# mikestir/webradio

Hardware: AMD Instinct MI355X
Metric: complex Msamples/sec (node), 256-ch DDC+NFM demod (higher is better)
Workload: dtype f32

## Files before the change

include/webradio_amd.h:

```cpp
#ifndef WEBRADIO_AMD_H_
#define WEBRADIO_AMD_H_

#include <stddef.h>
#include <stdint.h>

#ifdef __cplusplus
extern "C" {
#endif

#define WR_ABI_VERSION   6
#define WR_FIR_LENGTH    64
#define WR_TABLE_SIZE    65536

enum wr_status {
	WR_OK = 0,
	WR_ERR_ARG = 1,
	WR_ERR_HIP = 2,
	WR_ERR_STATE = 3,
	WR_ERR_NOMEM = 4,
	WR_ERR_NODEV = 5,
	WR_ERR_RATE = 6
};

enum wr_mode { WR_AM = 0, WR_FM = 1, WR_USB = 2, WR_LSB = 3 };

enum wr_stage {
	WR_STAGE_CHAN_IQ = 1,
	WR_STAGE_DEMOD   = 2,
	WR_STAGE_AUDIO   = 3
};

enum wr_nco {
	WR_NCO_SPLIT = 0,
	WR_NCO_EXACT = 1,
	WR_NCO_ROTATE = 2
};

enum wr_where { WR_HOST = 0, WR_DEVICE = 1 };

typedef struct wr_dev      wr_dev;
typedef struct wr_tuner    wr_tuner;
typedef struct wr_spectrum wr_spectrum;
typedef struct wr_ring     wr_ring;

int         wr_abi_version(void);
const char *wr_last_error(void);
int         wr_device_count(int *count);
enum wr_tunable {
	WR_TUNE_DDC_NG2_MIN_PASSES = 1
};
int         wr_tune(int key, long value, long *previous);

int wr_phase_step(int if_hz, unsigned int input_rate, int *phase_step);
int wr_sin_table(float *table_host);
int wr_lowpass_design(unsigned int passband, unsigned int input_rate,
                      float *coeff_host , unsigned int *maxbin_out);
#define WR_FIR_MAX 1024
#define WR_FIR_FUSED_MAX 256
int wr_lowpass_design_n(unsigned int fir_length, unsigned int passband, unsigned int input_rate,
                        float *coeff_host , unsigned int *maxbin_out);
int wr_spectrum_window(unsigned int fft_size, float *window_host);

int wr_dev_open(wr_dev **dev, int device_index, void *hip_stream);
int wr_dev_close(wr_dev *dev);
int wr_dev_sync(wr_dev *dev);
void *wr_dev_stream(wr_dev *dev);
int wr_dev_malloc(wr_dev *dev, size_t bytes, void **ptr_dev);
int wr_dev_free(wr_dev *dev, void *ptr_dev);
int wr_dev_upload(wr_dev *dev, void *dst_dev, const void *src_host, size_t bytes);
int wr_dev_download(wr_dev *dev, void *dst_host, const void *src_dev, size_t bytes);
int wr_dev_host_register(wr_dev *dev, void *host, size_t bytes);
int wr_dev_host_unregister(wr_dev *dev, void *host);
int wr_dev_upload_async(wr_dev *dev, void *dst_dev, const void *src_host, size_t bytes);
int wr_dev_wait_uploads(wr_dev *dev);
int wr_dev_wait_uploads_but(wr_dev *dev, unsigned int newest);
int wr_dev_upload_ahead(wr_dev *dev, void *dst_dev, const void *src_host, size_t bytes);

int wr_mix(wr_dev *dev, const float *in_dev, float *out_dev, size_t nframes,
           unsigned int *phase_io, int phase_step);

int wr_fir_decimate(wr_dev *dev, const float *in_dev, size_t nframes, unsigned int channels,
                    unsigned int decimation, const float *coeff_host ,
                    float *history_dev, float *out_dev);
int wr_fir_decimate_n(wr_dev *dev, const float *in_dev, size_t nframes, unsigned int channels,
                      unsigned int decimation, unsigned int fir_length, const float *coeff_host ,
                      float *history_dev, float *out_dev);
unsigned long long wr_block_kernel_calls(void);

int wr_demod(wr_dev *dev, int mode, const float *in_dev, size_t nframes,
             float *prev_io , float *out_dev);

int wr_u8_to_f32(wr_dev *dev, const uint8_t *in_dev, float *out_dev, size_t count);
int wr_u8_to_f32_from_host(wr_dev *dev, const uint8_t *in_host_registered, float *out_dev, size_t count);
int wr_stage_windows_from_host(wr_dev *dev, const void *in_host_registered, int is_u8, float *out_dev, size_t nframes,
                               unsigned int period, unsigned int length, size_t tail_frames);

#define WR_MAX_CHANNELS 4096
int wr_tuner_create(wr_tuner **tuner, wr_dev *dev, unsigned int input_rate,
                    unsigned int max_channels, size_t max_block_frames, int nco_mode);
int wr_tuner_destroy(wr_tuner *tuner);

int wr_chan_add(wr_tuner *tuner, int *chan);
int wr_chan_remove(wr_tuner *tuner, int chan);
int wr_chan_count(wr_tuner *tuner, int *count);

int wr_chan_set_if(wr_tuner *tuner, int chan, int if_hz);
int wr_chan_set_filter(wr_tuner *tuner, int chan, int stage, unsigned int passband,
                       unsigned int out_rate);
int wr_chan_set_taps(wr_tuner *tuner, int chan, int stage, const float *coeff_host ,
                     unsigned int decimation);
int wr_chan_set_filter_n(wr_tuner *tuner, int chan, int stage, unsigned int fir_length,
                         unsigned int passband, unsigned int out_rate);
int wr_chan_set_taps_n(wr_tuner *tuner, int chan, int stage, const float *coeff_host ,
                       unsigned int fir_length, unsigned int decimation);
#define WR_FILTER_CHANNEL  0
#define WR_FILTER_AUDIO    1
#define WR_FILTER_CHANNEL2 2
int wr_chan_set_af_gain(wr_tuner *tuner, int chan, float gain_db);
int wr_chan_set_squelch(wr_tuner *tuner, int chan, float threshold_dbfs, int enable);
int wr_chan_set_mode(wr_tuner *tuner, int chan, int mode);
int wr_tuner_keep_stages(wr_tuner *tuner, unsigned int stage_mask);

int wr_chan_get_state(wr_tuner *tuner, int chan, unsigned int *phase, float *prev_iq );
int wr_chan_set_state(wr_tuner *tuner, int chan, unsigned int phase, const float *prev_iq);

int wr_tuner_last_staging(wr_tuner *tuner, int *how);
int wr_tuner_submit(wr_tuner *tuner, const float *iq, size_t nframes, int where);
int wr_tuner_submit_u8(wr_tuner *tuner, const uint8_t *iq_u8, size_t nframes, int where);

int wr_tuner_flush(wr_tuner *tuner);

int wr_chan_fetch(wr_tuner *tuner, int chan, int stage, float *out_host, size_t out_capacity,
                  size_t *count);
int wr_tuner_audio_dev(wr_tuner *tuner, const float **audio_dev, size_t *chan_stride,
                       size_t *frames);
int wr_chan_slot(wr_tuner *tuner, int chan, int *slot);
int wr_tuner_fetch_audio_all(wr_tuner *tuner, float *out_host, size_t out_capacity,
                             size_t *chan_stride, size_t *frames, unsigned int *slots_used);
int wr_tuner_audio_ring(wr_tuner *tuner, unsigned int depth);
int wr_tuner_audio_ring_acquire(wr_tuner *tuner, const float **audio_host, size_t *chan_stride,
                                size_t *frames, unsigned int *slots_used, unsigned long long *seq);
int wr_tuner_audio_ring_release(wr_tuner *tuner);
int wr_tuner_audio_ring_ready(wr_tuner *tuner, int *ready);
int wr_tuner_audio_ring_stats(wr_tuner *tuner, unsigned int *queued, unsigned long long *overruns);
int wr_tuner_submit_count(wr_tuner *tuner, unsigned long long *submits);
int wr_chan_reset_history(wr_tuner *tuner, int chan);
int wr_tuner_seek(wr_tuner *tuner, unsigned long long frame);
int wr_ring_id_bytes(void);
int wr_ring_version(int *version);
int wr_ring_make_id(void *id_host, size_t nbytes);
int wr_ring_create(wr_ring **ring, wr_dev *dev, const void *id_host, size_t nbytes, int rank, int world);
int wr_ring_exchange(wr_ring *ring, const float *send_dev, float *recv_dev, size_t nfloats);
int wr_tuner_mark_launches(wr_tuner *tuner, int enable);
int wr_ring_exchange_after(wr_ring *ring, wr_tuner *tuner, const float *send_dev, float *recv_dev, size_t nfloats);
int wr_ring_wait(wr_ring *ring);
int wr_ring_info(wr_ring *ring, int *rank, int *world, unsigned long long *exchanges);
int wr_ring_destroy(wr_ring *ring);
int wr_tuner_set_audio_scale(wr_tuner *tuner, float scale);

int wr_tuner_set_blocks_per_launch(wr_tuner *tuner, unsigned int nblocks);

#define WR_STREAM_MAX_BLOCKS 512u
int wr_tuner_set_streaming(wr_tuner *tuner, int enable);
int wr_tuner_stream_info(wr_tuner *tuner, int *live, unsigned long long *launches, unsigned long long *blocks);
int wr_tuner_stream_host_blocks(wr_tuner *tuner, unsigned long long *blocks);
int wr_tuner_stream_long_blocks(wr_tuner *tuner, unsigned long long *blocks);

int wr_tuner_profile(wr_tuner *tuner, int enable);
int wr_tuner_profile_read(wr_tuner *tuner, unsigned int *launches, double *mean_ms);

int wr_spectrum_create(wr_spectrum **spec, wr_dev *dev, unsigned int fft_size, unsigned int hop);
int wr_spectrum_destroy(wr_spectrum *spec);
int wr_spectrum_push(wr_spectrum *spec, const float *iq, size_t nframes, int where);
int wr_spectrum_lazy_info(wr_spectrum *spec, unsigned long long *deferred_pushes, unsigned long long *resolves);
int wr_spectrum_get_db(wr_spectrum *spec, float *magnitudes_host );
int wr_spectrum_get_bins(wr_spectrum *spec, float *bins_host );
int wr_spectrum_frames_done(wr_spectrum *spec, unsigned long *frames);
int wr_spectrum_get_waterfall_row(wr_spectrum *spec, unsigned int width, int hold,
                                  float *db_row_host, uint8_t *palette_host);
int wr_spectrum_batch_db(wr_spectrum *spec, const float *iq_dev, size_t nframes_fft,
                         float *db_dev);

#ifdef __cplusplus
}
#endif
#endif
```

webradio_amd/capi.py:

```python
import ctypes as C
import os

_HERE = os.path.dirname(os.path.abspath(__file__))
LIB_PATH = os.path.join(_HERE, "lib", "libwebradio_amd.so")

WR_OK, WR_ERR_ARG, WR_ERR_HIP, WR_ERR_STATE, WR_ERR_NOMEM, WR_ERR_NODEV, WR_ERR_RATE = range(7)
WR_AM, WR_FM, WR_USB, WR_LSB = range(4)
WR_STAGE_CHAN_IQ, WR_STAGE_DEMOD, WR_STAGE_AUDIO = 1, 2, 3
WR_NCO_SPLIT, WR_NCO_EXACT, WR_NCO_ROTATE = 0, 1, 2
WR_HOST, WR_DEVICE = 0, 1
WR_ABI_VERSION = 6
WR_STREAM_MAX_BLOCKS = 512
WR_FIR_LENGTH = 64
WR_TABLE_SIZE = 65536

_fp = C.POINTER(C.c_float)
_vp = C.c_void_p
_u32 = C.c_uint
_sz = C.c_size_t

SIGNATURES = {
    "wr_abi_version": (C.c_int, []),
    "wr_last_error": (C.c_char_p, []),
    "wr_device_count": (C.c_int, [C.POINTER(C.c_int)]),
    "wr_tune": (C.c_int, [C.c_int, C.c_long, C.POINTER(C.c_long)]),
    "wr_phase_step": (C.c_int, [C.c_int, _u32, C.POINTER(C.c_int)]),
    "wr_sin_table": (C.c_int, [_vp]),
    "wr_lowpass_design": (C.c_int, [_u32, _u32, _vp, C.POINTER(_u32)]),
    "wr_lowpass_design_n": (C.c_int, [_u32, _u32, _u32, _vp, C.POINTER(_u32)]),
    "wr_spectrum_window": (C.c_int, [_u32, _vp]),
    "wr_dev_open": (C.c_int, [C.POINTER(_vp), C.c_int, _vp]),
    "wr_dev_close": (C.c_int, [_vp]),
    "wr_dev_sync": (C.c_int, [_vp]),
    "wr_dev_stream": (_vp, [_vp]),
    "wr_dev_malloc": (C.c_int, [_vp, _sz, C.POINTER(_vp)]),
    "wr_dev_free": (C.c_int, [_vp, _vp]),
    "wr_dev_upload": (C.c_int, [_vp, _vp, _vp, _sz]),
    "wr_dev_download": (C.c_int, [_vp, _vp, _vp, _sz]),
    "wr_dev_host_register": (C.c_int, [_vp, _vp, _sz]),
    "wr_dev_host_unregister": (C.c_int, [_vp, _vp]),
    "wr_dev_upload_async": (C.c_int, [_vp, _vp, _vp, _sz]),
    "wr_dev_wait_uploads": (C.c_int, [_vp]),
    "wr_dev_wait_uploads_but": (C.c_int, [_vp, C.c_uint]),
    "wr_dev_upload_ahead": (C.c_int, [_vp, _vp, _vp, _sz]),
    "wr_mix": (C.c_int, [_vp, _vp, _vp, _sz, C.POINTER(_u32), C.c_int]),
    "wr_fir_decimate": (C.c_int, [_vp, _vp, _sz, _u32, _u32, _vp, _vp, _vp]),
    "wr_fir_decimate_n": (C.c_int, [_vp, _vp, _sz, _u32, _u32, _u32, _vp, _vp, _vp]),
    "wr_demod": (C.c_int, [_vp, C.c_int, _vp, _sz, _vp, _vp]),
    "wr_u8_to_f32": (C.c_int, [_vp, _vp, _vp, _sz]),
    "wr_stage_windows_from_host": (C.c_int, [_vp, _vp, C.c_int, _vp, _sz, _u32, _u32, _sz]),
    "wr_u8_to_f32_from_host": (C.c_int, [_vp, _vp, _vp, _sz]),
    "wr_tuner_create": (C.c_int, [C.POINTER(_vp), _vp, _u32, _u32, _sz, C.c_int]),
    "wr_tuner_destroy": (C.c_int, [_vp]),
    "wr_chan_add": (C.c_int, [_vp, C.POINTER(C.c_int)]),
    "wr_chan_remove": (C.c_int, [_vp, C.c_int]),
    "wr_chan_count": (C.c_int, [_vp, C.POINTER(C.c_int)]),
    "wr_chan_set_if": (C.c_int, [_vp, C.c_int, C.c_int]),
    "wr_chan_set_filter": (C.c_int, [_vp, C.c_int, C.c_int, _u32, _u32]),
    "wr_chan_set_taps": (C.c_int, [_vp, C.c_int, C.c_int, _vp, _u32]),
    "wr_chan_set_filter_n": (C.c_int, [_vp, C.c_int, C.c_int, _u32, _u32, _u32]),
    "wr_chan_set_taps_n": (C.c_int, [_vp, C.c_int, C.c_int, _vp, _u32, _u32]),
    "wr_chan_set_mode": (C.c_int, [_vp, C.c_int, C.c_int]),
    "wr_chan_set_af_gain": (C.c_int, [_vp, C.c_int, C.c_float]),
    "wr_chan_set_squelch": (C.c_int, [_vp, C.c_int, C.c_float, C.c_int]),
    "wr_tuner_keep_stages": (C.c_int, [_vp, _u32]),
    "wr_tuner_flush": (C.c_int, [_vp]),
    "wr_tuner_set_blocks_per_launch": (C.c_int, [_vp, _u32]),
    "wr_tuner_set_streaming": (C.c_int, [_vp, C.c_int]),
    "wr_tuner_stream_info": (C.c_int, [_vp, C.POINTER(C.c_int), C.POINTER(C.c_ulonglong), C.POINTER(C.c_ulonglong)]),
    "wr_tuner_stream_host_blocks": (C.c_int, [_vp, C.POINTER(C.c_ulonglong)]),
    "wr_tuner_stream_long_blocks": (C.c_int, [_vp, C.POINTER(C.c_ulonglong)]),
    "wr_tuner_seek": (C.c_int, [_vp, C.c_ulonglong]),
    "wr_tuner_audio_ring": (C.c_int, [_vp, _u32]),
    "wr_tuner_audio_ring_acquire": (C.c_int, [_vp, C.POINTER(C.POINTER(C.c_float)), C.POINTER(C.c_size_t),
                                              C.POINTER(C.c_size_t), C.POINTER(_u32), C.POINTER(C.c_ulonglong)]),
    "wr_tuner_audio_ring_release": (C.c_int, [_vp]),
    "wr_tuner_audio_ring_ready": (C.c_int, [_vp, C.POINTER(C.c_int)]),
    "wr_tuner_audio_ring_stats": (C.c_int, [_vp, C.POINTER(_u32), C.POINTER(C.c_ulonglong)]),
    "wr_tuner_submit_count": (C.c_int, [_vp, C.POINTER(C.c_ulonglong)]),
    "wr_chan_get_state": (C.c_int, [_vp, C.c_int, C.POINTER(_u32), _vp]),
    "wr_chan_set_state": (C.c_int, [_vp, C.c_int, _u32, _vp]),
    "wr_tuner_submit": (C.c_int, [_vp, _vp, _sz, C.c_int]),
    "wr_tuner_last_staging": (C.c_int, [_vp, C.POINTER(C.c_int)]),
    "wr_block_kernel_calls": (C.c_ulonglong, []),
    "wr_tuner_submit_u8": (C.c_int, [_vp, _vp, _sz, C.c_int]),
    "wr_chan_fetch": (C.c_int, [_vp, C.c_int, C.c_int, _vp, _sz, C.POINTER(_sz)]),
    "wr_tuner_audio_dev": (C.c_int, [_vp, C.POINTER(_vp), C.POINTER(_sz), C.POINTER(_sz)]),
    "wr_chan_slot": (C.c_int, [_vp, C.c_int, C.POINTER(C.c_int)]),
    "wr_tuner_fetch_audio_all": (C.c_int, [_vp, _vp, _sz, C.POINTER(_sz), C.POINTER(_sz), C.POINTER(_u32)]),
    "wr_chan_reset_history": (C.c_int, [_vp, C.c_int]),
    "wr_ring_id_bytes": (C.c_int, []),
    "wr_ring_version": (C.c_int, [C.POINTER(C.c_int)]),
    "wr_ring_make_id": (C.c_int, [_vp, _sz]),
    "wr_ring_create": (C.c_int, [C.POINTER(_vp), _vp, _vp, _sz, C.c_int, C.c_int]),
    "wr_ring_exchange": (C.c_int, [_vp, _vp, _vp, _sz]),
    "wr_ring_exchange_after": (C.c_int, [_vp, _vp, _vp, _vp, _sz]),
    "wr_tuner_mark_launches": (C.c_int, [_vp, C.c_int]),
    "wr_ring_wait": (C.c_int, [_vp]),
    "wr_ring_info": (C.c_int, [_vp, C.POINTER(C.c_int), C.POINTER(C.c_int), C.POINTER(C.c_ulonglong)]),
    "wr_ring_destroy": (C.c_int, [_vp]),
    "wr_tuner_set_audio_scale": (C.c_int, [_vp, C.c_float]),
    "wr_spectrum_get_waterfall_row": (C.c_int, [_vp, _u32, C.c_int, _vp, _vp]),
    "wr_tuner_profile": (C.c_int, [_vp, C.c_int]),
    "wr_tuner_profile_read": (C.c_int, [_vp, C.POINTER(_u32), C.POINTER(C.c_double)]),
    "wr_spectrum_create": (C.c_int, [C.POINTER(_vp), _vp, _u32, _u32]),
    "wr_spectrum_destroy": (C.c_int, [_vp]),
    "wr_spectrum_push": (C.c_int, [_vp, _vp, _sz, C.c_int]),
    "wr_spectrum_lazy_info": (C.c_int, [_vp, C.POINTER(C.c_ulonglong), C.POINTER(C.c_ulonglong)]),
    "wr_spectrum_get_db": (C.c_int, [_vp, _vp]),
    "wr_spectrum_get_bins": (C.c_int, [_vp, _vp]),
    "wr_spectrum_frames_done": (C.c_int, [_vp, C.POINTER(C.c_ulong)]),
    "wr_spectrum_batch_db": (C.c_int, [_vp, _vp, _sz, _vp]),
}


class WrError(RuntimeError):
    def __init__(self, code, msg):
        super().__init__("webradio_amd error %d: %s" % (code, msg))
        self.code = code


_lib = None


def load():
    global _lib
    if _lib is not None:
        return _lib
    if not os.path.exists(LIB_PATH):
        raise RuntimeError(
            "%s is missing: build it with `python -c 'import __graft_entry__ as g; g.build()'` "
            "(there is no CPU fallback)" % LIB_PATH)
    try:
        import torch
    except Exception:
        pass
    lib = C.CDLL(LIB_PATH, mode=C.RTLD_GLOBAL)
    for name, (res, args) in SIGNATURES.items():
        fn = getattr(lib, name)
        fn.restype = res
        fn.argtypes = args
    _lib = lib
    return lib


def check(rc):
    if rc != WR_OK:
        raise WrError(rc, load().wr_last_error().decode(errors="replace"))
    return rc


def ptr(x):
    if x is None:
        return None
    if isinstance(x, int):
        return C.c_void_p(x)
    if hasattr(x, "data_ptr"):
        return C.c_void_p(x.data_ptr())
    return C.c_void_p(x.ctypes.data)
```

webradio_amd/csrc/wr_capi_internal.h:

```cpp
#ifndef WR_CAPI_INTERNAL_H
#define WR_CAPI_INTERNAL_H

#include "wr_internal.h"

#include <cstdarg>
#include <cstdio>
#include <cstdlib>
#include <cstring>
#include <new>
#include <atomic>
#include <chrono>
#include <map>
#include <mutex>
#include <vector>

#define HIP_TRY(expr)                                                                    \
	do {                                                                                 \
		hipError_t e_ = (expr);                                                          \
		if (e_ != hipSuccess)                                                            \
			return wrc_fail(WR_ERR_HIP, "%s: %s (%s:%d)", #expr, hipGetErrorString(e_),  \
			                __FILE__, __LINE__);                                         \
	} while (0)


#define WR_UPLOAD_RING 4

struct wr_dev {
	int device;
	hipStream_t stream;
	bool own_stream;
	int num_cus;
	float *table;
	float *table_turn;
	float *turn_host;
	float *hi_cs, *lo_cs;
	float *scratch;
	size_t scratch_floats;
	float *coeff;
	std::mutex *scratch_lock;
	hipEvent_t upload_ev[WR_UPLOAD_RING];
	std::atomic<unsigned long long> uploads_issued, uploads_done;
	std::mutex *upload_lock;
	hipStream_t up_stream;
	hipStream_t lazy_stream = nullptr;
	hipEvent_t up_tail[WR_UPLOAD_RING], up_done;
	void *up_out[WR_UPLOAD_RING];
	unsigned long long up_calls;
	uint8_t *up_raw[2];
	size_t up_raw_cap[2];
	std::map<void *, size_t> *registered;
	wr_tuner *streaming = nullptr;
	unsigned long long reg_gen = 1;
};
#define SCRATCH_GUARD(d) std::lock_guard<std::mutex> scratch_guard_(*(d)->scratch_lock)

struct Chan {
	bool in_use;
	int if_hz;
	unsigned int stepL;
	unsigned int phaseL;
	int mode;
	bool have[3];
	float taps[3][WR_FIR_LENGTH];
	unsigned int len1;
	float taps_long[WR_FIR_FUSED_MAX];
	unsigned int len2, len1b;
	float taps_long2[WR_FIR_FUSED_MAX], taps_long1b[WR_FIR_FUSED_MAX];
	unsigned int decim[3];
	float gain;
	float squelch;
	bool cs_hist_reset;
	int group;
	int slot;
	float prev_iq[2];
	bool prev_dirty;
	bool phase_dirty;
	bool dem_hist_reset;
};

struct Group {
	unsigned int d1, d2;
	unsigned int d1b = 0;
	unsigned int l1 = WR_FIR_LENGTH;
	unsigned int l2 = WR_FIR_LENGTH;
	unsigned int l1b = WR_FIR_LENGTH;
	int p2 = 0;
	bool use_gain = false, use_squelch = false;
	unsigned int slots;
	size_t k1max, k2max;
	WrGroupDev dev;
	int audio_cur = 0;
	int parity;
	int last_parity;
	bool last_demod_kept = false;
	bool post_pending = false;
	WrPostArgs post_args;
	bool seek_pending = false;
	unsigned long long seek_frame = 0;
	float *z_hist = nullptr, *z_prev = nullptr, *z_dem = nullptr;
	bool pend_direct = false;
	unsigned long long pend_seq = 0;
	size_t pend_k2 = 0;
	unsigned int pend_slots = 0;
	int sp;
	int cb;
	int last_cb;
	std::vector<int> owner;
	bool dirty;
	bool uniform_taps;
	unsigned long long uniform_mask = 0;
	unsigned long long uniform2_mask = 0;
	unsigned long long fewsets_mask = 0;
	unsigned char nsets[64] = {0};
	bool one_filter = false;
	bool long_uniform = false;
	bool long_one = false;
	size_t last_k1, last_k2;
	int active;
};

struct wr_tuner {
	wr_dev *dev;
	unsigned int input_rate;
	unsigned int max_channels;
	size_t max_block_frames;
	int nco_mode;
	unsigned int keep_mask;
	std::vector<Chan> chans;
	std::vector<Group *> groups;
	float *in_stage;
	int last_staging = 0;
	const void *probe_ptr = nullptr;
	unsigned long long probe_gen = 0;
	unsigned int probe_left = 0;
	float *in_hist[2];
	int in_par;
	bool submitted;
	float audio_scale;
	bool profiling;
	unsigned int prof_stride;
	unsigned int prof_tick;
	std::vector<unsigned int> ev_span;
	bool mark_launches = false;
	hipEvent_t launch_ev[4] = {nullptr, nullptr, nullptr, nullptr};
	unsigned long long launches_marked = 0;
	std::vector<hipEvent_t> ev;
	size_t ev_used;
	double prof_ms;
	unsigned int prof_n;
	struct RingSlot {
		float *host = nullptr;
		size_t cap = 0;
		hipEvent_t done = nullptr;
		size_t stride = 0, frames = 0;
		unsigned int slots = 0;
		unsigned long long seq = 0;
		unsigned int stream_wait = 0;
		unsigned long long stream_gen = 0;
	};
	std::vector<RingSlot> ring;
	unsigned int ring_head = 0, ring_count = 0;
	bool ring_held = false;
	unsigned long long ring_overruns = 0;
	unsigned long long submit_seq = 0;
	bool defer_post = true;
	unsigned int coalesce = 1;
	const float *held_base = nullptr;
	size_t held_frames = 0, held_each = 0;
	unsigned int held_count = 0;
	std::mutex ring_lock;
	struct Stream {
		bool enabled = false;
		bool host_bytes = false;
		bool live = false;
		bool unchecked = false;
		WrStreamCtl *ctl = nullptr;
		WrStreamDesc *desc = nullptr;
		WrStreamDev *sdev = nullptr;
		float *ring = nullptr;
		size_t ring_floats = 0;
		Group *g = nullptr;
		unsigned int count = 0;
		size_t nframes = 0;
		bool u8 = false;
		int parity0 = 0;
		size_t k1 = 0, k2 = 0;
		unsigned long long gen = 0;
		unsigned long long blocks = 0;
		std::chrono::steady_clock::time_point last_bell;
		const float *last_iq = nullptr;
		uint8_t *raw[4] = {nullptr, nullptr, nullptr, nullptr};
		size_t raw_cap = 0;
		unsigned long long raw_next = 0;
		unsigned long long raw_gen[4] = {0, 0, 0, 0};
		unsigned int raw_idx[4] = {0, 0, 0, 0};
		hipEvent_t raw_ev = nullptr;
		bool ext = false;
		bool up_pending = false;
		unsigned long long host_blocks = 0;
		unsigned long long long_blocks = 0;
	} stream;
};

struct wr_spectrum {
	wr_dev *dev;
	unsigned int n, hop;
	WrFftPlan plan;
	float *stage;
	size_t stage_cap;
	size_t pending;
	float *bins;
	unsigned long frames_done;
	bool deferred = false;
	float *keep_host = nullptr;
	size_t keep_cap = 0;
	size_t def_off = 0, def_keep = 0;
	size_t def_rest = 0;
	hipEvent_t def_ev = nullptr;
	unsigned long long deferred_pushes = 0, resolves = 0;
};


int        wrc_dev_bind(wr_dev *d);
int        wrc_dev_settle_stream(wr_dev *d);
hipError_t wrc_dev_stream_sync(wr_dev *d);
int        wrc_dev_scratch(wr_dev *d, size_t floats);
void      *wrc_host_mapped(const void *host, hipError_t *why = nullptr);
int        wrc_upload_mark_locked(wr_dev *d, hipStream_t st);
int        wrc_upload_mark(wr_dev *d, hipStream_t st);
int        wrc_dev_up_stream(wr_dev *d);

unsigned int  wrc_group_slots_used(const Group *g);
WrTunerLaunch wrc_group_launch(const wr_tuner *t, const Group *g, const float *cur, const uint8_t *cur_u8, size_t nframes);
Group        *wrc_single_group(wr_tuner *t, bool *several = nullptr);
int           wrc_group_upload(wr_tuner *t, Group *g);
int           wrc_settle_held(wr_tuner *t);
int           wrc_tuner_launch_held(wr_tuner *t);
int           wrc_tuner_flush(wr_tuner *t);
int           wrc_tuner_quiesce(wr_tuner *t);
int           wrc_tuner_submit_now(wr_tuner *t, const void *iq, size_t nframes, int where, bool u8);
void          wrc_advance_phases(wr_tuner *t, unsigned long long frames);
int           wrc_prof_pair_begin(wr_tuner *t, void **ev_start, void **ev_stop);
void          wrc_prof_pair_stamped(wr_tuner *t);

int  wrc_stream_close(wr_tuner *t);
int  wrc_stream_check(wr_tuner *t);
void wrc_stream_free(wr_tuner *t);
bool wrc_stream_follows(const wr_tuner *t, size_t nframes, int where, bool u8);
int  wrc_stream_bell(wr_tuner *t, const void *iq, bool behind_upload);
int  wrc_stream_open(wr_tuner *t, const void *iq, size_t nframes, bool u8, bool *took);
int  wrc_stream_host_u8(wr_tuner *t, const uint8_t *bytes, size_t nframes, bool *took);

float *wrc_ring_reserve(wr_tuner *t, Group *g, size_t k2, unsigned int used);
int    wrc_ring_push(wr_tuner *t, Group *g, unsigned long long seq, size_t k2, unsigned int used, bool direct);
float *wrc_stream_ring_entry(wr_tuner *t, Group *g, unsigned long long seq, size_t k2, unsigned int used, unsigned int idx);

#define DEV_SETTLE(d_) do { if (int rc_ = wrc_dev_settle_stream(d_)) return rc_; } while (0)
#define TUNER_SYNC_CHECKED(t_) do { HIP_TRY(wrc_dev_stream_sync((t_)->dev)); if (int rc_ = wrc_stream_check(t_)) return rc_; } while (0)

#define WR_STREAM_IDLE_MS   500
#define WR_STREAM_STALE_MS  100
#define WR_STREAM_WAIT_MS  2000
#define WR_STREAM_HOST_MIN_BYTES (16u << 10)

#endif
```

webradio_amd/csrc/wr_internal.h:

```cpp
#ifndef WR_INTERNAL_H_
#define WR_INTERNAL_H_

#include <hip/hip_runtime.h>
#include <stddef.h>
#include <stdint.h>

#include "webradio_amd.h"

#define WR_HIST      (WR_FIR_LENGTH - 1)
#define WR_LANES     64
#define WR_SPLIT_N   256
#define WR_MAX_DEVICES 64
#define WR_TAPSETS   4

int         wrc_fail(int code, const char *fmt, ...) __attribute__((format(printf, 2, 3)));
int         wrc_dev_index(const wr_dev *dev);
hipStream_t wrc_dev_stream(const wr_dev *dev);
int         wrc_tuner_launch_mark(wr_tuner *t, hipEvent_t *ev);

void     wrd_sin_table(float *table);
void     wrd_sin_table_rounded(float *table);
int      wrd_phase_step(int if_hz, unsigned int input_rate);
unsigned wrd_lowpass_maxbin(unsigned int fir_length, unsigned int passband, unsigned int input_rate);
void     wrd_lowpass_design(unsigned int fir_length, unsigned int passband, unsigned int input_rate, float *coeff);
void     wrd_spectrum_window(unsigned int n, float *window);
void     wrd_split_tables(float *hi_cs , float *lo_cs );
void     wrd_twiddles(unsigned int n, float *tw );

struct WrGroupDev {
	unsigned int *phase[2];
	unsigned int *step;
	float        *hist_cs[2];
	float        *hist_lo[2];
	int          *flags;
	int          *mode;
	float        *taps1;
	float        *taps2;
	float        *taps2u;
	float        *rot;
	float        *taps1u;
	int          *tapsel;
	float        *taps1b;
	float        *iq2_hist[2];
	float        *chan_iq2[2];
	float        *taps1L;
	float        *mixhist[2];
	float        *gain;
	float        *squelch;
	float        *prev_iq[2];
	float        *chan_iq[2];
	float        *dem[2];
	float        *audio;
	float        *audio_set[4];
	unsigned int  l2 = 64, l1b = 64;
};

struct WrTunerLaunch {
	const float *cur;
	const uint8_t *cur_u8;
	const float *hist;
	float       *hist_next;
	int          parity;
	int          sp;
	int          cb;
	size_t       nframes;
	unsigned int d1, d2;
	unsigned int slots;
	unsigned int slots_used;
	size_t       k1, k2;
	size_t       k2max;
	int          nco_mode;
	float        audio_scale;
	int          use_gain, use_squelch;
	unsigned long long uniform_mask;
	unsigned long long uniform2_mask;
	unsigned long long fewsets_mask;
	unsigned char nsets[64];
	int          one_filter;
	void        *ev_start, *ev_stop;
	bool         seeking = false;
	unsigned int seek_lo = 0;
};

hipError_t wrk_mix(hipStream_t st, const float *in, float *out, size_t nframes,
                   unsigned int phase, int step, const float *table_dev);
hipError_t wrk_fir(hipStream_t st, const float *in, size_t nframes, unsigned int channels,
                   unsigned int decim, unsigned int fir_length, const float *coeff_dev, const float *hist_dev,
                   float *out);
hipError_t wrk_hist_update(hipStream_t st, const float *in, size_t nframes, unsigned int channels,
                           unsigned int fir_length, float *hist_dev, float *scratch_dev);
hipError_t wrk_demod(hipStream_t st, int mode, const float *in, size_t nframes, float prev_i,
                     float prev_q, float *out);
hipError_t wrk_u8_to_f32(hipStream_t st, const uint8_t *in, float *out, size_t count);
hipError_t wrk_stage_windows(hipStream_t st, const void *src_mapped, bool u8, float *dst, size_t nframes, unsigned int period,
                             unsigned int len, size_t tail_frames);

struct WrPostArgs {
	const float *chan_iq;
	unsigned int k1, slots;
	const int   *mode;
	const float *prev_iq;
	float       *prev_next;
	const float *dem_hist;
	float       *dem_hist_next;
	size_t       k2;
	unsigned int tiles;
	unsigned int run;
	unsigned int ntiles;
	const float *taps2;
	const float *taps2u;
	unsigned long long uni2;
	float       *audio;
	size_t       k2max;
	float        scale;
	unsigned int d2;
	unsigned int groups;
	const float *gain;
	const float *squelch;
	float       *audio_host;
	size_t       host_stride;
	unsigned int nseg = 1;
	const float *chan_prev = nullptr;
};
long wrk_tune_ng2_min_passes(long value, bool set);
hipError_t wrk_tuner_ddc(hipStream_t st, const WrTunerLaunch &L, const WrGroupDev &G,
                         const float *table_dev, const float *hi_dev, const float *lo_dev,
                         int num_cus, const WrPostArgs *post = nullptr, bool *post_taken = nullptr);
hipError_t wrk_tuner_ddc_long(hipStream_t st, const WrTunerLaunch &L, const WrGroupDev &G, unsigned int len,
                              const float *table_dev, int num_cus, bool rotate, bool rotate_one_filter, const float *hi_dev,
                              const float *lo_dev, const WrPostArgs *post = nullptr, bool *post_taken = nullptr);
hipError_t wrk_tuner_demod(hipStream_t st, const WrTunerLaunch &L, const WrGroupDev &G);
hipError_t wrk_tuner_iq2(hipStream_t st, const WrGroupDev &G, unsigned int slots, unsigned int slots_used,
                         size_t k1a, unsigned int d1b, int cb, int p2);
hipError_t wrk_tuner_audio(hipStream_t st, const WrTunerLaunch &L, const WrGroupDev &G);
WrPostArgs wrk_post_args(const WrTunerLaunch &L, const WrGroupDev &G);
hipError_t wrk_tuner_post(hipStream_t st, const WrTunerLaunch &L, const WrGroupDev &G);
hipError_t wrk_tuner_post_args(hipStream_t st, const WrPostArgs &A);
bool wrk_tuner_post_supported(unsigned int d2);
hipError_t wrk_input_hist(hipStream_t st, const float *cur, const uint8_t *cur_u8, size_t nframes,
                          const float *hist, float *hist_next);
hipError_t wrk_seek(hipStream_t st, const WrGroupDev &G, unsigned int slots, int sp, int parity, int p2,
                    unsigned long long frame);
hipError_t wrk_gather_rows(hipStream_t st, const float *src, size_t rows, size_t row_stride_floats,
                           size_t col_offset_floats, unsigned int width_floats, float *dst);

#define WR_STREAM_MAXJ   WR_STREAM_MAX_BLOCKS
#define WR_STREAM_RING   6u
struct WrStreamDesc {
	unsigned long long cur;
	unsigned long long audio_host;
	unsigned int count;
	unsigned int pad;
};
struct WrStreamCtl {
	volatile unsigned int ready;
	volatile unsigned int stop;
	volatile unsigned int pad0[14];
	volatile unsigned int done;
	volatile unsigned int final_blocks;
	volatile unsigned int err;
	volatile unsigned int self_closed;
	volatile unsigned int long_blocks;
	volatile unsigned int pad1[11];
};
#define WR_STREAM_SHARDS 16u
struct WrStreamDev {
	unsigned int ready, stop;
	unsigned long long beat;
	unsigned int ready_up;
	unsigned int pad0[27];
	unsigned long long progress;
	unsigned int drain_from;
	unsigned int pad1[29];
	unsigned int post_done[WR_STREAM_MAXJ];
	unsigned int post_fine[WR_STREAM_MAXJ];
	unsigned int post_ticket[WR_STREAM_MAXJ];
	unsigned int ddc_done[WR_STREAM_MAXJ][WR_STREAM_SHARDS][32];
	WrStreamDesc desc[WR_STREAM_MAXJ];
	unsigned long long cur[WR_STREAM_MAXJ + 1u];
};
struct WrStreamArgs {
	WrStreamCtl        *ctl;
	const WrStreamDesc *desc_host;
	WrStreamDev        *sdev;
	unsigned long long  idle_ticks;
	unsigned long long  wait_ticks;
	unsigned int        n_ddc, n_post;
	unsigned long long *tl;
	unsigned long long  cur0, audio0;
	unsigned long long  nframes;
	unsigned int        k1, d1, is_u8;
	unsigned int        ext;
	unsigned int        slots, groups;
	unsigned long long  gmap0, gmap1;
	unsigned int        kslow;
	unsigned int        kmax;
	const float        *hist;
	float              *hist_next;
	const unsigned int *phase, *step;
	unsigned int       *phase_next;
	const float        *hist_cs, *hist_lo;
	float              *hist_cs_next, *hist_lo_next;
	const int          *flags;
	const float        *taps1, *rot, *taps1u;
	const int          *tapsel;
	const float        *table, *hi_cs, *lo_cs;
	float              *ring;
	float              *audio_bufs[4];
	WrPostArgs          post;
	unsigned int        drain_run, drain_ntiles;
	const float        *prev_iq[2];
	float              *dem[2];
	int                 parity0;
	unsigned int        one_filter;
};
#define WR_STREAM_ERR_WAIT   1u
hipError_t wrk_stream_geometry(unsigned int d2, unsigned int groups, unsigned int kmax, bool one_filter, int num_cus,
                               unsigned int *n_ddc, unsigned int *n_post);
hipError_t wrk_tuner_stream(hipStream_t st, const WrStreamArgs &A, void *ev_start, void *ev_stop);

struct WrFftPlan {
	unsigned int n;
	unsigned int n1, n2;
	float *tw_n;
	float *tw_sub;
	float *window;
	float *window_p1;
	float *work;
	size_t work_frames;
};
hipError_t wrk_fft_frames(hipStream_t st, const WrFftPlan &P, const float *iq, size_t hop,
                          size_t nframes_fft, float *bins_out , float *db_out );

hipError_t wrk_bins_to_db(hipStream_t st, const float *bins, unsigned int n, float *db);
hipError_t wrk_waterfall_row(hipStream_t st, const float *bins, unsigned int n, unsigned int width, int hold,
                             float *db_row, uint8_t *palette);

#endif
```

webradio_amd/csrc/wr_kernels.hip:

```cpp
#include "wr_internal.h"

#include <atomic>
#include <cstdlib>
#include <type_traits>

#include <hip/hip_ext.h>

typedef float v2f __attribute__((ext_vector_type(2)));
typedef __attribute__((address_space(3))) v2f lds_v2f;
typedef float v4f __attribute__((ext_vector_type(4)));
typedef __attribute__((address_space(3))) v4f lds_v4f;

#define PHASE_FLAG_ACTIVE   1

#define WR_CONSTANT __attribute__((address_space(4)))

#ifdef DDC_TIMELINE
#define TL_SLOTS 12
__device__ unsigned long long g_ddc_tl[16384 * TL_SLOTS];
extern "C" int wr_debug_timeline(unsigned long long *out, size_t n)
{
	return (int)hipMemcpyFromSymbol(out, HIP_SYMBOL(g_ddc_tl), n * sizeof(unsigned long long));
}
__device__ unsigned long long g_ddc_rt[16384 * 2];
// ... 49 lines not shown
		out[n] = y;
	}
}

__global__ void __launch_bounds__(256)
k_fir(const float *__restrict__ in, size_t outfloats, unsigned int channels, unsigned int decim,
      unsigned int L, const float *__restrict__ coeff, const float *__restrict__ hist, float *__restrict__ out)
{
	__shared__ float taps[WR_FIR_MAX];
	for (unsigned int j = threadIdx.x; j < L; j += blockDim.x)
		taps[j] = coeff[j];
	__syncthreads();
	const unsigned int nh = L - 1u;
	size_t stride = (size_t)gridDim.x * blockDim.x;
	for (size_t o = (size_t)blockIdx.x * blockDim.x + threadIdx.x; o < outfloats; o += stride) {
		size_t k = o / channels;
		unsigned int c = (unsigned int)(o - k * channels);
		size_t first = k * decim;
		float acc = 0.0f;
		for (unsigned int j = 0; j < L; ++j) {
			size_t f = first + j;
			float x = (f < nh) ? hist[f * channels + c] : in[(f - nh) * channels + c];
			acc = acc + taps[L - 1u - j] * x;
		}
		out[o] = acc;
	}
}

__global__ void k_hist_build(const float *__restrict__ in, size_t nframes, unsigned int channels, unsigned int nh,
                             const float *__restrict__ hist, float *__restrict__ scratch)
{
	unsigned int total = nh * channels;
	for (unsigned int e = blockIdx.x * blockDim.x + threadIdx.x; e < total; e += gridDim.x * blockDim.x) {
		size_t f = nframes + e / channels;
		unsigned int c = e % channels;
		scratch[e] = (f < nh) ? hist[f * channels + c] : in[(f - nh) * channels + c];
	}
}

__global__ void k_copy_f32(const float *__restrict__ src, float *__restrict__ dst, size_t n)
{
	size_t stride = (size_t)gridDim.x * blockDim.x;
	for (size_t i = (size_t)blockIdx.x * blockDim.x + threadIdx.x; i < n; i += stride)
		dst[i] = src[i];
}

__device__ __forceinline__ float fm_angle_cycles(float y, float x)
{
	const float ax = __builtin_fabsf(x), ay = __builtin_fabsf(y);
	const float mx = __builtin_fmaxf(ax, ay), mn = __builtin_fminf(ax, ay);
	const float sc = (mx < 0x1p-100f) ? 0x1p100f : 1.0f;
	const float r = (mx == 0.0f) ? 0.0f : (mn * sc) * __builtin_amdgcn_rcpf(mx * sc);
	const float t = r * r;
	float p = 0.002456712769344449f;
	p = __builtin_fmaf(p, t, -0.014401308260858059f);
	p = __builtin_fmaf(p, t, 0.03978113830089569f);
	p = __builtin_fmaf(p, t, -0.07234849780797958f);
	p = __builtin_fmaf(p, t, 0.1049894168972969f);
	p = __builtin_fmaf(p, t, -0.14161227643489838f);
	p = __builtin_fmaf(p, t, 0.19985906779766083f);
	p = __builtin_fmaf(p, t, -0.33332598209381104f);
	p = __builtin_fmaf(p, t, 0.9999998807907104f);
	float c = (p * r) * 0.15915494309189533577f;
	if (ay > ax)
		c = 0.25f - c;
	if (__builtin_signbitf(x))
		c = 0.5f - c;
	return __builtin_copysignf(c, y);
}

__device__ __forceinline__ float demod_one(int mode, float i, float q, float pi_, float pq_)
{
	switch (mode) {
	case WR_AM:
		return (float)sqrt((double)(i * i + q * q));
	case WR_FM: {
		float ii = i * pi_ + q * pq_;
		float qq = q * pi_ - i * pq_;
		return fm_angle_cycles(ii, qq);
	}
	case WR_USB:
		return i + q;
	default:
		return i - q;
	}
}

__global__ void __launch_bounds__(256)
k_demod(int mode, const float2 *__restrict__ in, size_t nframes, float prev_i, float prev_q,
        float *__restrict__ out)
{
	size_t stride = (size_t)gridDim.x * blockDim.x;
	for (size_t n = (size_t)blockIdx.x * blockDim.x + threadIdx.x; n < nframes; n += stride) {
		float2 z = in[n];
		float2 p = n ? in[n - 1] : make_float2(prev_i, prev_q);
		out[n] = demod_one(mode, z.x, z.y, p.x, p.y);
	}
}

__global__ void k_u8_to_f32(const uint8_t *__restrict__ in, float *__restrict__ out, size_t n)
{
	size_t stride = (size_t)gridDim.x * blockDim.x;
	for (size_t i = (size_t)blockIdx.x * blockDim.x + threadIdx.x; i < n; i += stride)
		out[i] = ((float)in[i] - 128.0f) / 128.0f;
}

#define U8_X16_WGS 128u
__global__ void __launch_bounds__(256) k_u8_to_f32_x16(const uint4 *__restrict__ in, float4 *__restrict__ out, size_t n16)
{
	const size_t stride = (size_t)gridDim.x * blockDim.x;
	for (size_t i0 = (size_t)blockIdx.x * blockDim.x + threadIdx.x; i0 < n16; i0 += 4 * stride) {
		uint4 v[4];
#pragma unroll
		for (int u = 0; u < 4; ++u)
			if (i0 + u * stride < n16)
				v[u] = in[i0 + u * stride];
#pragma unroll
		for (int u = 0; u < 4; ++u) {
			const size_t i = i0 + u * stride;
			if (i >= n16)
				break;
			const unsigned int w[4] = {v[u].x, v[u].y, v[u].z, v[u].w};
#pragma unroll
			for (int q = 0; q < 4; ++q) {
				float4 o;
				o.x = ((float)(w[q] & 255u) - 128.0f) / 128.0f;
				o.y = ((float)((w[q] >> 8) & 255u) - 128.0f) / 128.0f;
				o.z = ((float)((w[q] >> 16) & 255u) - 128.0f) / 128.0f;
				o.w = ((float)(w[q] >> 24) - 128.0f) / 128.0f;
				out[4 * i + q] = o;
			}
		}
	}
}


template <int NCO>
__device__ __forceinline__ v2f nco(unsigned int P, const float *__restrict__ table,
                                   const v2f *hi_l, const v2f *lo_l)
{
	if (NCO == WR_NCO_EXACT) {
		v2f cs;
		cs.y = table[P >> 16];
		cs.x = table[(P + 0x40000000u) >> 16];
		return cs;
	} else {
		constexpr unsigned int SH = (NCO == WR_NCO_SPLIT) ? 5u : 0u;
		const v2f a = hi_l[(P >> 24) << SH];
		const v2f b = lo_l[((P >> 16) & 255u) << SH];
		const v2f rot = {-a.y, a.x};
		return __builtin_elementwise_fma(rot, b.yy, a * b.xx);
	}
}

template <int NCO>
__device__ __forceinline__ void mac(v2f xs, v2f cs, float hj, v2f &acc)
{
	if (NCO == WR_NCO_EXACT) {
		const float mi = xs.x * cs.x + xs.y * cs.y;
		const float mq = xs.y * cs.x - xs.x * cs.y;
		float ti, tq;
		asm("v_mul_f32 %0, %1, %2" : "=v"(ti) : "v"(hj), "v"(mi));
		asm("v_mul_f32 %0, %1, %2" : "=v"(tq) : "v"(hj), "v"(mq));
		acc.x = acc.x + ti;
		acc.y = acc.y + tq;
	} else {
		const v2f xr = {xs.y, -xs.x};
		const v2f m = __builtin_elementwise_fma(xr, cs.yy, xs * cs.xx);
		asm("v_fmac_f32 %0, %1, %2" : "+v"(acc.x) : "v"(hj), "v"(m.x));
		asm("v_fmac_f32 %0, %1, %2" : "+v"(acc.y) : "v"(hj), "v"(m.y));
	}
}

__device__ __forceinline__ unsigned int rot_index(unsigned int p0, unsigned int st, unsigned int m)
{
	const unsigned int P = p0 + m * st;
	return (st >> 16) + (((P & 0xFFFFu) < (st & 0xFFFFu)) ? 1u : 0u);
}

__device__ __forceinline__ v2f rot_into(unsigned int p0, unsigned int st, unsigned int m,
                                        const float *__restrict__ table)
{
	const unsigned int idx = rot_index(p0, st, m);
	v2f r;
	r.y = table[idx & 0xFFFFu];
	r.x = table[(idx + 16384u) & 0xFFFFu];
	return r;
}

__device__ __forceinline__ void horner_step(v2f &A, float rc, float rs, v2f u)
{
	const float tr = __builtin_fmaf(-A.y, rs, u.x);
	const float ti = __builtin_fmaf(A.x, rs, u.y);
	const float ar = __builtin_fmaf(A.x, rc, tr);
	const float ai = __builtin_fmaf(A.y, rc, ti);
	A.x = ar;
	A.y = ai;
}

__device__ __forceinline__ void horner_close(v2f &y, v2f A, v2f cs)
{
	const float yr = __builtin_fmaf(A.y, cs.y, __builtin_fmaf(A.x, cs.x, y.x));
	const float yi = __builtin_fmaf(-A.x, cs.y, __builtin_fmaf(A.y, cs.x, y.y));
	y.x = yr;
	y.y = yi;
}

__device__ __forceinline__ void wave_prio(unsigned int level)
{
	if (level >= 3u)
		__builtin_amdgcn_s_setprio(3);
	else if (level == 2u)
		__builtin_amdgcn_s_setprio(2);
	else if (level == 1u)
		__builtin_amdgcn_s_setprio(1);
	else
		__builtin_amdgcn_s_setprio(0);
}

__device__ __forceinline__ void rot_tables_to_lds(v2f *lds, const float2 *hi_cs, const float2 *lo_cs)
{
	for (unsigned int e = threadIdx.x; e < WR_SPLIT_N; e += blockDim.x) {
		const float2 hv = hi_cs[e], lv = lo_cs[e];
		lds[e] = (v2f){hv.x, hv.y};
		lds[WR_SPLIT_N + e] = (v2f){lv.x, lv.y};
	}
	__syncthreads();
}

#define ROT_SEG 64
#define ROT_Q   (WR_FIR_LENGTH / ROT_SEG)
#define SLOW_CH 4

__device__ __forceinline__ void gather_split(unsigned int P, unsigned int &ah, unsigned int &al,
                                             v2f &a, v2f &b)
{
	asm("v_mov_b32_sdwa %0, %1 dst_sel:BYTE_1 dst_unused:UNUSED_PRESERVE src0_sel:BYTE_3"
	    : "+v"(ah) : "v"(P));
	asm("v_mov_b32_sdwa %0, %1 dst_sel:BYTE_1 dst_unused:UNUSED_PRESERVE src0_sel:BYTE_2"
	    : "+v"(al) : "v"(P));
	a = *(const lds_v2f *)(uintptr_t)ah;
	b = *(const lds_v2f *)(uintptr_t)al;
}

__device__ __forceinline__ float2 input_frame(const float2 *__restrict__ cur, const uchar2 *__restrict__ cur_u8,
                                              size_t n)
{
	if (cur_u8) {
		const uchar2 b = cur_u8[n];
		return make_float2(((float)b.x - 128.0f) / 128.0f, ((float)b.y - 128.0f) / 128.0f);
	}
	return cur[n];
}

#define POST_TK 16u
#define POST_B 4u
#define POST_LB 5u
#define POST_THREADS 512u
__device__ __forceinline__ float audio_out(float v, const float *__restrict__ gain, const float *__restrict__ squelch,
                                           const float2 *__restrict__ chan_iq, unsigned int slots, unsigned int so,
                                           size_t k, unsigned int d2, float scale)
{
	if (squelch) {
		const float thr = squelch[so];
		if (thr > 0.0f) {
			float p = 0.0f;
			for (unsigned int i = 0; i < d2; ++i) {
				const float2 z = chan_iq[(k * d2 + i) * slots + so];
				p = p + (z.x * z.x + z.y * z.y);
			}
			if (p / (float)d2 < thr)
				v = 0.0f;
		}
	}
	if (gain) {
		const float gn = gain[so];
		if (gn != 1.0f)
			v = v * gn;
	}
	return (scale == 1.0f) ? v : v * scale;
}

__device__ __forceinline__ float post_row(const float2 *__restrict__ chan_iq, unsigned int k1, unsigned int slots,
                                          unsigned int s, int m, const float2 *__restrict__ prev_iq,
                                          const float *__restrict__ dem_hist, size_t rr,
                                          const float2 *__restrict__ chan_prev = nullptr, unsigned int hist = WR_HIST)
{
	if (rr < hist) {
		if (!chan_prev)
			return dem_hist[rr * slots + s];
		const size_t kp = (size_t)k1 - hist + rr;
		const float2 z = chan_prev[kp * slots + s];
		const float2 zp = chan_prev[(kp - 1u) * slots + s];
		return demod_one(m, z.x, z.y, zp.x, zp.y);
	}
	const size_t kk = rr - hist;
	if (kk >= k1)
		return 0.0f;
	const float2 z = chan_iq[kk * slots + s];
	const float2 zp = kk ? chan_iq[(kk - 1u) * slots + s] : chan_prev ? chan_prev[((size_t)k1 - 1u) * slots + s] : prev_iq[s];
	return demod_one(m, z.x, z.y, zp.x, zp.y);
}

template <unsigned int D2, bool HREGS, unsigned int NSEG = 1u>
__device__ __forceinline__ void post_role(const WrPostArgs &A, unsigned int bx, unsigned int g,
                                          float *stage, float *tile, int *modes)
{
	constexpr unsigned int HIST = WR_FIR_LENGTH * NSEG - 1u;
	constexpr unsigned int NEED = (POST_TK - 1u) * D2 + WR_FIR_LENGTH * NSEG;
	constexpr unsigned int NROW = POST_THREADS / 64u;
	static_assert(NSEG == 1u || !HREGS, "the segmented filter reads its taps when their turn comes (measured at C2, 128 / 256 taps: "
	                                    "61 / 83 us per block; a segment's 64 taps fetched into registers first: 64 / 94)");
	const float2 *__restrict__ chan_iq = (const float2 *)A.chan_iq;
	const float2 *__restrict__ prev_iq = (const float2 *)A.prev_iq;
	const float2 *__restrict__ chan_prev = (const float2 *)A.chan_prev;
	const float *__restrict__ dem_hist = A.dem_hist;
	const float *__restrict__ taps2 = A.taps2;
	const unsigned int k1 = A.k1, slots = A.slots;
	const unsigned int lane = threadIdx.x & 63u;
	const unsigned int row = threadIdx.x >> 6;
	const unsigned int s = g * 64u + lane;
	const int m = A.mode[s];

	if (bx == A.ntiles) {
		if (m < 0)
			return;
		const size_t first = k1;
#pragma unroll
		for (unsigned int r = row; r < HIST; r += NROW)
			A.dem_hist_next[(size_t)r * slots + s] = post_row(chan_iq, k1, slots, s, m, prev_iq, dem_hist, first + r, chan_prev, HIST);
		if (row == 0)
			((float2 *)A.prev_next)[s] = k1 ? chan_iq[(size_t)(k1 - 1u) * slots + s] : prev_iq[s];
		return;
	}

	TLP(0);
	float h[HREGS ? WR_FIR_LENGTH : 1];
	if (HREGS && row < POST_TK / POST_B) {
#pragma unroll
		for (int j = 0; j < (HREGS ? WR_FIR_LENGTH : 1); ++j)
			h[j] = taps2[(size_t)j * slots + s];
	}
	if (row == 0)
		modes[lane] = m;
	constexpr unsigned int FRESH = POST_TK * D2;
	constexpr unsigned int CARRY = NEED - FRESH;
	constexpr unsigned int CARRY_PER = (CARRY * 64u + POST_THREADS - 1u) / POST_THREADS;
	for (unsigned int tt = 0; tt < A.run; ++tt) {
		const unsigned int tl = bx * A.run + tt;
		if (tl >= A.tiles)
			break;
		const size_t kbase = (size_t)tl * POST_TK;
		const size_t r0 = kbase * D2;
		unsigned int first = 0;
		if (tt) {
			float keep[CARRY_PER];
#pragma unroll
			for (unsigned int i = 0; i < CARRY_PER; ++i) {
				const unsigned int e = threadIdx.x + i * POST_THREADS;
				keep[i] = (e < CARRY * 64u) ? stage[FRESH * 64u + e] : 0.0f;
			}
			__syncthreads();
#pragma unroll
			for (unsigned int i = 0; i < CARRY_PER; ++i) {
				const unsigned int e = threadIdx.x + i * POST_THREADS;
				if (e < CARRY * 64u)
					stage[e] = keep[i];
			}
			first = CARRY;
		}
		{
			const unsigned int per = (NEED - first + NROW - 1u) / NROW;
			const unsigned int beg = first + row * per;
			const unsigned int end = (beg + per < NEED) ? beg + per : NEED;
			if (r0 > HIST && r0 + NEED <= (size_t)k1 + HIST) {
				const float2 *__restrict__ src = chan_iq + (r0 - HIST) * slots + s;
				for (unsigned int r = beg; r < end; r += POST_LB) {
					float2 z[POST_LB + 1u];
					z[0] = src[((size_t)r - 1u) * slots];
#pragma unroll
					for (unsigned int i = 0; i < POST_LB; ++i) {
						const unsigned int ri = (r + i < end) ? r + i : end - 1u;
						z[i + 1u] = src[(size_t)ri * slots];
					}
#pragma unroll
					for (unsigned int i = 0; i < POST_LB; ++i)
						if (r + i < end)
							stage[(r + i) * 64u + lane] = (m >= 0) ? demod_one(m, z[i + 1u].x, z[i + 1u].y, z[i].x, z[i].y) : 0.0f;
				}
			} else {
				float2 zp = make_float2(0.0f, 0.0f);
				if (m >= 0 && beg < end) {
					const size_t rr = r0 + beg;
					if (rr == HIST)
						zp = chan_prev ? chan_prev[((size_t)k1 - 1u) * slots + s] : prev_iq[s];
					else if (rr > HIST && rr - HIST - 1u < k1)
						zp = chan_iq[(rr - HIST - 1u) * slots + s];
					else if (rr < HIST && chan_prev)
						zp = chan_prev[((size_t)k1 - HIST - 1u + rr) * slots + s];
				}
#pragma unroll 6
				for (unsigned int r = beg; r < end; ++r) {
					const size_t rr = r0 + r;
					float v = 0.0f;
					if (m >= 0) {
						if (rr < HIST && chan_prev) {
							const float2 z = chan_prev[((size_t)k1 - HIST + rr) * slots + s];
							v = demod_one(m, z.x, z.y, zp.x, zp.y);
							zp = z;
						} else if (rr < HIST) {
							v = dem_hist[rr * slots + s];
							if (rr + 1u == HIST)
								zp = prev_iq[s];
						} else if (rr - HIST < k1) {
							const float2 z = chan_iq[(rr - HIST) * slots + s];
							v = demod_one(m, z.x, z.y, zp.x, zp.y);
							zp = z;
						}
					}
					stage[r * 64u + lane] = v;
				}
			}
		}
		__syncthreads();
		TLP(1);
		if (row < POST_TK / POST_B) {
			float acc[POST_B];
#pragma unroll
			for (unsigned int o = 0; o < POST_B; ++o)
				acc[o] = 0.0f;
			if (HREGS) {
				const float *x = stage + (row * POST_B * D2) * 64u + lane;
#pragma unroll
				for (unsigned int r = 0; r < (POST_B - 1u) * D2 + WR_FIR_LENGTH; ++r) {
					const float xv = x[r * 64u];
#pragma unroll
					for (unsigned int o = 0; o < POST_B; ++o) {
						if (r >= o * D2 && r - o * D2 < WR_FIR_LENGTH)
							acc[o] = acc[o] + h[HREGS ? WR_FIR_LENGTH - 1u - (r - o * D2) : 0] * xv;
					}
				}
			} else {
#pragma unroll 1
			for (unsigned int seg = 0; seg < NSEG; ++seg) {
				const float *x = stage + (row * POST_B * D2 + seg * WR_FIR_LENGTH) * 64u + lane;
				const unsigned int tap0 = (NSEG - 1u - seg) * WR_FIR_LENGTH;
				if (g < 64u && ((A.uni2 >> g) & 1ull)) {
					const WR_CONSTANT float *tu = (const WR_CONSTANT float *)(A.taps2u + (size_t)g * (WR_FIR_LENGTH * NSEG) + tap0);
#pragma unroll
					for (int j = WR_FIR_LENGTH - 1; j >= 0; --j) {
						const float hj = tu[j];
#pragma unroll
						for (unsigned int o = 0; o < POST_B; ++o)
							acc[o] = acc[o] + hj * x[(o * D2 + (WR_FIR_LENGTH - 1u - (unsigned int)j)) * 64u];
					}
				} else {
#pragma unroll 16
					for (int j = WR_FIR_LENGTH - 1; j >= 0; --j) {
						const float hj = taps2[((size_t)tap0 + j) * slots + s];
#pragma unroll
						for (unsigned int o = 0; o < POST_B; ++o)
							acc[o] = acc[o] + hj * x[(o * D2 + (WR_FIR_LENGTH - 1u - (unsigned int)j)) * 64u];
					}
				}
			}
			}
#pragma unroll
			for (unsigned int o = 0; o < POST_B; ++o)
				tile[(row * POST_B + o) * 65u + lane] = acc[o];
		}
		__syncthreads();
		TLP(2);
		for (unsigned int e = threadIdx.x; e < 64u * POST_TK; e += POST_THREADS) {
			const unsigned int sl = e / POST_TK, kk = e - sl * POST_TK;
			const unsigned int so = g * 64u + sl;
			const size_t k = kbase + kk;
			if (k < A.k2 && modes[sl] >= 0) {
				const float v = audio_out(tile[kk * 65u + sl], A.gain, A.squelch, chan_iq, slots, so, k, D2, A.scale);
				A.audio[(size_t)so * A.k2max + k] = v;
				if (A.audio_host)
					A.audio_host[(size_t)so * A.host_stride + k] = v;
			} else if (k < A.k2 && A.audio_host) {
				A.audio_host[(size_t)so * A.host_stride + k] = 0.0f;
			}
		}
		TLP(3);
	}
}

template <unsigned int D2, unsigned int NSEG = 1u>
__global__ void __launch_bounds__(POST_THREADS)
k_tuner_post(WrPostArgs A)
{
	constexpr unsigned int NEED = (POST_TK - 1u) * D2 + WR_FIR_LENGTH * NSEG;
	if constexpr (NSEG == 1u) {
		__shared__ float stage[NEED * 64u];
		__shared__ float tile[POST_TK * 65u];
		__shared__ int modes[64];
		post_role<D2, NSEG == 1u, NSEG>(A, blockIdx.x, blockIdx.y, stage, tile, modes);
	} else {
		extern __shared__ float post_lds[];
		float *stage = post_lds;
		float *tile = stage + NEED * 64u;
		int *modes = (int *)(tile + POST_TK * 65u);
		post_role<D2, NSEG == 1u, NSEG>(A, blockIdx.x, blockIdx.y, stage, tile, modes);
	}
}

#define DDC_TABLE_BYTES   (2u * WR_SPLIT_N * 32u * 8u)
#define DDC_WAVES         16u
#define DDC_ROTATE_WAVES      8u
#define DDC_ROTATE_WGS_PER_CU 4u
#define DDC_LDS_BYTES     (DDC_TABLE_BYTES + DDC_WAVES * 2u * 512u)
#define DDC_DEAL_WAYS 2u

#define DDC_PARAMS \
	const float2 *__restrict__ cur, const uchar2 *__restrict__ cur_u8, const float2 *__restrict__ hist, \
	float2 *__restrict__ hist_next, size_t nframes, size_t k1, unsigned int d1, unsigned int slots, unsigned int groups, \
	const unsigned int *__restrict__ phase, const unsigned int *__restrict__ step, \
	const float2 *__restrict__ hist_cs, const int *__restrict__ flags, \
	unsigned int *__restrict__ phase_next, float2 *__restrict__ hist_cs_next, \
	const float2 *__restrict__ hist_lo, float2 *__restrict__ hist_lo_next, \
	const float *__restrict__ taps1, const float4 *__restrict__ rot, const float *__restrict__ taps1u, \
	const int *__restrict__ tapsel, unsigned int kmax, float2 *__restrict__ chan_iq, \
	const float *__restrict__ table, const float2 *__restrict__ hi_cs, const float2 *__restrict__ lo_cs, \
	unsigned int n_ddc, const WrPostArgs &post, unsigned long long gmap0, unsigned long long gmap1, int whole, \
	unsigned int kslow, unsigned int n_bnd, unsigned int seek_on, unsigned int seek_lo
#define DDC_PASS \
	cur, cur_u8, hist, hist_next, nframes, k1, d1, slots, groups, phase, step, hist_cs, flags, phase_next, hist_cs_next, \
	hist_lo, hist_lo_next, taps1, rot, taps1u, tapsel, kmax, chan_iq, table, hi_cs, lo_cs, n_ddc, post, gmap0, gmap1, \
	whole, kslow, n_bnd, seek_on, seek_lo
#define DDC_PHASE(s_) (seek_on ? step[s_] * seek_lo : phase[s_])
#define DDC_ROLE_ALL      0
#define DDC_ROLE_BOUNDARY 1
#define DDC_ROLE_ROLL     2

template <int NCO, bool UTAPS, unsigned int PD2>
__device__ __forceinline__ void
ddc_body(DDC_PARAMS, v2f *lds, const int role)
{
	if (PD2 != 0u && role != DDC_ROLE_ROLL && blockIdx.x >= n_ddc + n_bnd) {
		wave_prio(3u);
		constexpr unsigned int NEED = (POST_TK - 1u) * (PD2 ? PD2 : 1u) + WR_FIR_LENGTH;
		const unsigned int idx = blockIdx.x - n_ddc - n_bnd;
		if (threadIdx.x >= POST_THREADS)
			return;
		float *stage = (float *)lds;
		post_role<(PD2 ? PD2 : 1u), false>(post, idx % (post.ntiles + 1u), idx / (post.ntiles + 1u), stage,
		                                    stage + NEED * 64u, (int *)(stage + NEED * 64u + POST_TK * 65u));
		return;
	}
	const unsigned int lane = threadIdx.x & 63u;
	const unsigned int wave = __builtin_amdgcn_readfirstlane(threadIdx.x >> 6);
	const unsigned int waves_per_wg = blockDim.x >> 6;
	const unsigned int wid = blockIdx.x * waves_per_wg + wave;
	TL(0);
	wave_prio(3u);

	if (NCO == WR_NCO_SPLIT) {
		for (unsigned int e = threadIdx.x; e < WR_SPLIT_N * 32u; e += blockDim.x) {
			const float2 hv = hi_cs[e >> 5], lv = lo_cs[e >> 5];
			lds[e] = (v2f){hv.x, hv.y};
			lds[WR_SPLIT_N * 32u + e] = (v2f){lv.x, lv.y};
		}
		__syncthreads();
	} else if (NCO == WR_NCO_ROTATE) {
		rot_tables_to_lds(lds, hi_cs, lo_cs);
	}
	const v2f *hi_l = (NCO == WR_NCO_ROTATE) ? lds : lds + (lane & 31u);
	const v2f *lo_l = (NCO == WR_NCO_ROTATE) ? lds + WR_SPLIT_N : lds + WR_SPLIT_N * 32u + (lane & 31u);
	const unsigned int a_hi = (unsigned int)(uintptr_t)hi_l;
	const unsigned int a_lo = (unsigned int)(uintptr_t)lo_l;
	const unsigned int nset = UTAPS ? kmax : 1u;
	v2f *win = lds + (NCO == WR_NCO_SPLIT ? DDC_TABLE_BYTES / 8u : NCO == WR_NCO_ROTATE ? 2u * WR_SPLIT_N : 0u)
	           + wave * (128u * nset);

	if (whole && role != DDC_ROLE_ROLL && blockIdx.x == 0 && wave == 0 && lane < WR_HIST) {
		const size_t f = nframes + lane;
		hist_next[lane] = (f < WR_HIST) ? hist[f] : input_frame(cur, cur_u8, f - WR_HIST);
	}

	const unsigned int k1u = (unsigned int)k1;
	const unsigned int nwaves = n_ddc * waves_per_wg;
	TL(1);
	constexpr bool LTAPS = (NCO == WR_NCO_ROTATE) && !UTAPS;
	unsigned int wpg = LTAPS ? (n_ddc / groups) * waves_per_wg : nwaves / groups;
	const bool bnd = role == DDC_ROLE_BOUNDARY;
	const unsigned int ub = bnd ? (blockIdx.x - n_ddc) * waves_per_wg + wave : 0u;
	const unsigned int gl = bnd ? ub % groups : LTAPS ? blockIdx.x % groups : wid % groups;
	const unsigned int g = (unsigned int)(((gl < 8u ? gmap0 : gmap1) >> ((gl & 7u) * 8u)) & 255u);
	unsigned int k = bnd ? ub / groups : LTAPS ? (blockIdx.x / groups) * waves_per_wg + wave : wid / groups;
	if (role == DDC_ROLE_ROLL) {
		k = k1u;
	} else if (bnd) {
		if (k >= kslow)
			k = k1u;
		wpg = k1u;
	} else if (k >= wpg) {
		k = k1u;
	} else if (!LTAPS) {
		const unsigned int r = k % DDC_DEAL_WAYS, q = k / DDC_DEAL_WAYS;
		const unsigned int fl_ = wpg / DDC_DEAL_WAYS, rem = wpg % DDC_DEAL_WAYS;
		k = r * fl_ + (r < rem ? r : rem) + q;
	}
	const float *ltaps = (const float *)(lds + (NCO == WR_NCO_ROTATE ? 2u * WR_SPLIT_N : 0u) + waves_per_wg * 128u * nset);
	if (LTAPS) {
		float *lt = (float *)(lds + 2u * WR_SPLIT_N + waves_per_wg * 128u * nset);
		for (unsigned int e = threadIdx.x; e < WR_FIR_LENGTH * 64u; e += blockDim.x)
			lt[e] = taps1[(size_t)(e >> 6) * slots + g * 64u + (e & 63u)];
		__syncthreads();
	}

	float h[(UTAPS || LTAPS) ? 1 : WR_FIR_LENGTH];
	float hlane[UTAPS ? WR_TAPSETS : 1];
	unsigned int mysel = 0;
#pragma unroll
	for (int q = 0; q < (UTAPS ? WR_TAPSETS : 1); ++q)
		hlane[q] = 0.0f;
	unsigned int p0 = 0, st = 0;
	int fl = 0;
	unsigned int buf = 0;
	v2f rot0 = {1.0f, 0.0f}, rot1 = {1.0f, 0.0f};

	auto window_sample = [&](unsigned int kk) -> float2 {
		const long long n = (long long)kk * d1 - WR_HIST + lane;
		return (n >= 0) ? input_frame(cur, cur_u8, (size_t)n) : hist[WR_HIST + n];
	};
	float2 xnext = make_float2(0.0f, 0.0f);
	float2 xnext2 = make_float2(0.0f, 0.0f);
	const unsigned int s = g * 64u + lane;
	if (k < k1u) {
		{
			p0 = DDC_PHASE(s);
			st = step[s];
			fl = flags[s];
			if (NCO == WR_NCO_ROTATE) {
				const float4 r = rot[s];
				rot0 = (v2f){r.x, r.y};
				rot1 = (v2f){r.z, r.w};
			}
			if (UTAPS) {
				mysel = (unsigned int)tapsel[s];
#pragma unroll
				for (int q = 0; q < (UTAPS ? WR_TAPSETS : 1); ++q)
					if ((unsigned int)q < nset)
						hlane[q] = taps1u[((size_t)g * WR_TAPSETS + q) * 64u + lane];
			} else {
#pragma unroll
				for (int j = 0; j < ((UTAPS || LTAPS) ? 1 : WR_FIR_LENGTH); ++j)
					h[j] = taps1[(size_t)j * slots + s];
			}
		}
		xnext = window_sample(k);
		if (k + wpg < k1u)
			xnext2 = window_sample(k + wpg);
	}

	TL(2);
	unsigned int tl_unit = 0;
	const unsigned int my_units = (k < k1u) ? (k1u - k + wpg - 1u) / wpg : 0u;
	for (; k < k1u; buf ^= 1u) {
		const unsigned int kn = k + wpg;
		{
			const unsigned int q = (4u * tl_unit) / (my_units ? my_units : 1u);
			wave_prio(q >= 3u ? 0u : 2u - q + 0u);
		}

		const long long n0 = (long long)k * d1 - WR_HIST;
		{
			const float2 xf = xnext;
			if (UTAPS) {
#pragma unroll
				for (int q = 0; q < (UTAPS ? WR_TAPSETS : 1); ++q)
					if ((unsigned int)q < nset)
						win[(buf * nset + q) * 64u + lane] = (v2f){hlane[q] * xf.x, hlane[q] * xf.y};
			} else {
				win[buf * 64u + lane] = (v2f){xf.x, xf.y};
			}
// ... 1634 lines not shown
```

webradio_amd/csrc/wr_stream_kernel.inc:

```

__device__ __forceinline__ unsigned int st_rfl(unsigned int v) { return __builtin_amdgcn_readfirstlane(v); }
__device__ __forceinline__ unsigned int st_ld(const unsigned int *p)
{
	return st_rfl(__hip_atomic_load(p, __ATOMIC_RELAXED, __HIP_MEMORY_SCOPE_AGENT));
}
__device__ __forceinline__ unsigned long long st_ld64(const unsigned long long *p)
{
	const unsigned long long v = __hip_atomic_load(p, __ATOMIC_RELAXED, __HIP_MEMORY_SCOPE_AGENT);
	return ((unsigned long long)st_rfl((unsigned int)(v >> 32)) << 32) | st_rfl((unsigned int)v);
}
__device__ __forceinline__ unsigned int st_ld_sys(const volatile unsigned int *p)
{
	return st_rfl(__hip_atomic_load((const unsigned int *)p, __ATOMIC_RELAXED, __HIP_MEMORY_SCOPE_SYSTEM));
}
__device__ __forceinline__ void st_st_sys(volatile unsigned int *p, unsigned int v)
{
	__hip_atomic_store((unsigned int *)p, v, __ATOMIC_RELAXED, __HIP_MEMORY_SCOPE_SYSTEM);
}

__device__ __forceinline__ unsigned int st_ddc_ready(const WrStreamArgs &S)
{
	return st_rfl((unsigned int)__hip_atomic_load(&S.sdev->progress, __ATOMIC_RELAXED, __HIP_MEMORY_SCOPE_AGENT));
}
__device__ __forceinline__ unsigned int st_post_ready(const WrStreamArgs &S)
{
	return st_rfl((unsigned int)(__hip_atomic_load(&S.sdev->progress, __ATOMIC_RELAXED, __HIP_MEMORY_SCOPE_AGENT) >> 32));
}

__device__ __forceinline__ void stream_fail(const WrStreamArgs &S)
{
	st_st_sys(&S.ctl->err, WR_STREAM_ERR_WAIT);
	__hip_atomic_store(&S.sdev->stop, 1u, __ATOMIC_RELAXED, __HIP_MEMORY_SCOPE_AGENT);
}

__device__ __forceinline__ bool stream_wait_ready(const WrStreamArgs &S, unsigned int need, unsigned int &known, bool &closed)
{
	if (need < known)
		return true;
	if (closed)
		return false;
	const unsigned long long t0 = __builtin_amdgcn_s_memrealtime();
	unsigned int spins = 0;
	for (;;) {
		const unsigned int r = st_ld(&S.sdev->ready);
		if (r > need) {
			known = r;
			return true;
		}
		if (st_ld(&S.sdev->stop)) {
			const unsigned int f = st_ld(&S.sdev->ready);
			if (f > known)
				known = f;
			closed = true;
			return known > need;
		}
		if ((++spins & 63u) == 0u) {
			const unsigned long long now = __builtin_amdgcn_s_memrealtime();
			const unsigned long long beat = __hip_atomic_load(&S.sdev->beat, __ATOMIC_RELAXED, __HIP_MEMORY_SCOPE_AGENT);
			if (now - t0 > S.wait_ticks && now >= beat && now - beat > S.wait_ticks) {
				stream_fail(S);
				if (r > known)
					known = r;
				closed = true;
				return false;
			}
		}
		__builtin_amdgcn_s_sleep(20);
	}
}

__device__ __forceinline__ bool stream_wait_count(const WrStreamArgs &S, const unsigned int *p, unsigned int target)
{
	if (st_ld(p) >= target)
		return true;
	const unsigned long long t0 = __builtin_amdgcn_s_memrealtime();
	unsigned int spins = 0;
	for (;;) {
		__builtin_amdgcn_s_sleep(20);
		if (st_ld(p) >= target)
			return true;
		if ((++spins & 63u) == 0u) {
			if (__builtin_amdgcn_s_memrealtime() - t0 > S.wait_ticks) {
				stream_fail(S);
				return false;
			}
			if (st_ld_sys(&S.ctl->err))
				return false;
		}
	}
}

#define STREAM_DRAIN_BLOCKS 2u
__device__ __forceinline__ void stream_watch(const WrStreamArgs &S)
{
	const unsigned int lane = threadIdx.x & 63u;
	__builtin_amdgcn_s_setprio(3);
	const unsigned int units = S.k1 * S.groups;
	unsigned int known = 1, jd = 0, jp = 0;
	unsigned int df = 0;
	unsigned int nlong = 0;
	bool closed = false;
	unsigned long long t_last = __builtin_amdgcn_s_memrealtime();
#ifdef STREAM_TL
	if ((threadIdx.x & 63u) == 0 && S.tl)
		S.tl[6999u * 8u + 0u] = t_last;
#endif
	for (;;) {
		bool moved = false;
		auto look = [&]() __attribute__((always_inline)) {
			const unsigned int r = st_ld(&S.sdev->ready);
			if (r > known)
				known = r;
			if (st_ld(&S.sdev->stop)) {
				const unsigned int f = st_ld(&S.sdev->ready);
				if (f > known)
					known = f;
				closed = true;
				const unsigned int from = known >= STREAM_DRAIN_BLOCKS ? known - STREAM_DRAIN_BLOCKS : 0u;
				df = (jd > from ? jd : from) + 1u;
				__hip_atomic_store(&S.sdev->drain_from, df, __ATOMIC_RELAXED, __HIP_MEMORY_SCOPE_AGENT);
				__builtin_amdgcn_fence(__ATOMIC_RELEASE, "agent");
			}
		};
		if (!closed && (jd >= known || jp >= known))
			look();
		if (jd < known && jd < WR_STREAM_MAXJ) {
			unsigned int v = 0;
			if (lane < WR_STREAM_SHARDS)
				v = __hip_atomic_load(&S.sdev->ddc_done[jd][lane][0], __ATOMIC_RELAXED, __HIP_MEMORY_SCOPE_AGENT);
#pragma unroll
			for (int o = 8; o >= 1; o >>= 1)
				v += __shfl_xor(v, o, 64);
			if (st_rfl(v) >= units) {
				{
					unsigned int fine = 1u;
					if (S.drain_run != S.post.run) {
						if (!closed)
							look();
						fine = (df && jd + 1u >= df) ? 1u : known >= jd + 3u ? 0u : 1u;
					}
					__hip_atomic_store(&S.sdev->post_fine[jd], fine, __ATOMIC_RELAXED, __HIP_MEMORY_SCOPE_AGENT);
					if (!fine && lane == 0)
						st_st_sys(&S.ctl->long_blocks, ++nlong);
					asm volatile("s_waitcnt vmcnt(0)" ::: "memory");
				}
				++jd;
				__hip_atomic_store(&S.sdev->progress, ((unsigned long long)jp << 32) | jd, __ATOMIC_RELAXED, __HIP_MEMORY_SCOPE_AGENT);
				moved = true;
#ifdef STREAM_TL
				if (lane == 0 && S.tl && jd <= 256u)
					S.tl[(7000u + jd - 1u) * 8u + 0u] = __builtin_amdgcn_s_memrealtime();
#endif
			}
		}
		if (jp < jd && st_ld(&S.sdev->post_done[jp]) >= (st_ld(&S.sdev->post_fine[jp]) ? S.drain_ntiles : S.post.ntiles) * S.post.groups) {
			++jp;
			__hip_atomic_store(&S.sdev->progress, ((unsigned long long)jp << 32) | jd, __ATOMIC_RELAXED, __HIP_MEMORY_SCOPE_AGENT);
			if (lane == 0)
				st_st_sys(&S.ctl->done, jp);
			moved = true;
#ifdef STREAM_TL
			if (lane == 0 && S.tl && jp <= 256u)
				S.tl[(7000u + jp - 1u) * 8u + 1u] = __builtin_amdgcn_s_memrealtime();
#endif
		}
		if (closed && jp >= known)
			return;
		const unsigned long long now = __builtin_amdgcn_s_memrealtime();
		if (moved) {
			t_last = now;
		} else {
			if ((jd < known || jp < jd) && now - t_last > S.wait_ticks) {
				stream_fail(S);
				return;
			}
			if (closed && st_ld_sys(&S.ctl->err))
				return;
			__builtin_amdgcn_s_sleep(4);
		}
	}
}

__device__ __forceinline__ void stream_bell(const WrStreamArgs &S)
{
	if (threadIdx.x >= 64u && threadIdx.x < 128u) {
		stream_watch(S);
		return;
	}
	if (threadIdx.x != 0)
		return;
	__builtin_amdgcn_s_setprio(3);
	unsigned int seen = 1;
	__hip_atomic_store(&S.sdev->desc[0].cur, S.cur0, __ATOMIC_RELAXED, __HIP_MEMORY_SCOPE_AGENT);
	__hip_atomic_store(&S.sdev->desc[0].audio_host, S.audio0, __ATOMIC_RELAXED, __HIP_MEMORY_SCOPE_AGENT);
	__hip_atomic_store(&S.sdev->cur[1], S.cur0, __ATOMIC_RELAXED, __HIP_MEMORY_SCOPE_AGENT);
	asm volatile("s_waitcnt vmcnt(0)" ::: "memory");
	unsigned long long t_last = __builtin_amdgcn_s_memrealtime();
	for (;;) {
		__hip_atomic_store(&S.sdev->beat, (unsigned long long)__builtin_amdgcn_s_memrealtime(), __ATOMIC_RELAXED,
		                   __HIP_MEMORY_SCOPE_AGENT);
		const unsigned int s = st_ld_sys(&S.ctl->stop);
		unsigned int r = st_ld_sys(&S.ctl->ready);
		{
			const unsigned int ru = st_ld(&S.sdev->ready_up);
			if (ru > r)
				r = ru;
		}
		if (r > WR_STREAM_MAXJ)
			r = WR_STREAM_MAXJ;
		if (r > seen) {
			for (unsigned int j = seen; j < r; ++j) {
				const unsigned long long c = __hip_atomic_load(&S.desc_host[j].cur, __ATOMIC_RELAXED, __HIP_MEMORY_SCOPE_SYSTEM);
				const unsigned long long a = __hip_atomic_load(&S.desc_host[j].audio_host, __ATOMIC_RELAXED, __HIP_MEMORY_SCOPE_SYSTEM);
				__hip_atomic_store(&S.sdev->desc[j].cur, c, __ATOMIC_RELAXED, __HIP_MEMORY_SCOPE_AGENT);
				__hip_atomic_store(&S.sdev->cur[j + 1u], c, __ATOMIC_RELAXED, __HIP_MEMORY_SCOPE_AGENT);
				__hip_atomic_store(&S.sdev->desc[j].audio_host, a, __ATOMIC_RELAXED, __HIP_MEMORY_SCOPE_AGENT);
			}
			asm volatile("s_waitcnt vmcnt(0)" ::: "memory");
			__hip_atomic_store(&S.sdev->ready, r, __ATOMIC_RELAXED, __HIP_MEMORY_SCOPE_AGENT);
			seen = r;
			t_last = __builtin_amdgcn_s_memrealtime();
		}
		if (s || st_ld(&S.sdev->stop)) {
			asm volatile("s_waitcnt vmcnt(0)" ::: "memory");
			__hip_atomic_store(&S.sdev->stop, 1u, __ATOMIC_RELAXED, __HIP_MEMORY_SCOPE_AGENT);
			return;
		}
		if (seen >= WR_STREAM_MAXJ || __builtin_amdgcn_s_memrealtime() - t_last > S.idle_ticks) {
			if (seen < WR_STREAM_MAXJ)
				st_st_sys(&S.ctl->self_closed, 1u);
			asm volatile("s_waitcnt vmcnt(0)" ::: "memory");
			__hip_atomic_store(&S.sdev->stop, 1u, __ATOMIC_RELAXED, __HIP_MEMORY_SCOPE_AGENT);
			return;
		}
		__builtin_amdgcn_s_sleep(40);
	}
}

template <unsigned int PD2, unsigned int TS>
__device__ __forceinline__ void stream_post(const WrStreamArgs &S, const unsigned int p, v2f *lds, const bool helper)
{
	constexpr unsigned int D2 = PD2 ? PD2 : 1u;
	constexpr unsigned int NEED = (POST_TK - 1u) * D2 + WR_FIR_LENGTH;
	wave_prio(3u);
	if (threadIdx.x >= POST_THREADS)
		return;
	const unsigned int wave = st_rfl(threadIdx.x >> 6);
	const unsigned int waves_per_wg = POST_THREADS / 64u;
#ifdef STREAM_TL
	if (threadIdx.x == 0 && S.tl && !helper)
		S.tl[(6000u + p) * 8u + 7u] = 12345ull;
#endif

	const unsigned int n_bnd = (S.kslow * S.groups + waves_per_wg - 1u) / waves_per_wg;
	if (!helper && p < n_bnd) {
		const unsigned long long c0 = S.cur0;
		ddc_body<WR_NCO_ROTATE, true, PD2>(S.is_u8 ? nullptr : (const float2 *)c0, S.is_u8 ? (const uchar2 *)c0 : nullptr,
		                                   (const float2 *)S.hist, (float2 *)S.hist_next, (size_t)S.nframes, (size_t)S.k1, S.d1,
		                                   S.slots, S.groups, S.phase, S.step, (const float2 *)S.hist_cs, S.flags, S.phase_next,
		                                   (float2 *)S.hist_cs_next, (const float2 *)S.hist_lo, (float2 *)S.hist_lo_next, S.taps1,
		                                   (const float4 *)S.rot, S.taps1u, S.tapsel, TS == 1u ? 1u : S.kmax, (float2 *)S.ring, S.table,
		                                   (const float2 *)S.hi_cs, (const float2 *)S.lo_cs, S.n_ddc, S.post, S.gmap0, S.gmap1, 0,
		                                   S.kslow, 0x40000000u, 0u, 0u, lds, DDC_ROLE_BOUNDARY);
		const unsigned int ub = p * waves_per_wg + wave;
		asm volatile("s_waitcnt vmcnt(0)" ::: "memory");
		if (ub / S.groups < S.kslow && (threadIdx.x & 63u) == 0u)
			__hip_atomic_fetch_add(&S.sdev->ddc_done[0][ub % WR_STREAM_SHARDS][0], 1u, __ATOMIC_RELAXED, __HIP_MEMORY_SCOPE_AGENT);
		wave_prio(3u);
		__syncthreads();
	}

	float *stage = (float *)lds;
	float *tile = stage + NEED * 64u;
	int *modes = (int *)(tile + POST_TK * 65u);
	unsigned int *sh = (unsigned int *)(modes + 64);
	const unsigned int tasks = S.post.ntiles * S.post.groups;
	unsigned int known = 1;
	bool closed = false;
	unsigned int j = 0;
	if (helper) {
		if (threadIdx.x == 0)
			sh[6] = st_ld(&S.sdev->drain_from);
		__syncthreads();
		const unsigned int df = sh[6];
		if (!df)
			return;
		j = df - 1u;
	}
#ifdef STREAM_TL
	unsigned long long pt_wait = 0, pt_work = 0, pt_sync = 0, pt_n = 0;
#endif
	for (;; ++j) {
#ifdef STREAM_TL
		const unsigned long long pt0 = __builtin_amdgcn_s_memtime();
#endif
		if (threadIdx.x == 0) {
			bool ok = j < WR_STREAM_MAXJ && stream_wait_ready(S, j, known, closed);
			if (ok) {
				const unsigned int need_hi = j >= 4u ? j - 3u : 0u;
				const unsigned long long t0 = __builtin_amdgcn_s_memrealtime();
				unsigned int spins = 0;
				for (;;) {
					const unsigned long long pg = st_ld64(&S.sdev->progress);
					if ((unsigned int)pg >= j + 1u && (unsigned int)(pg >> 32) >= need_hi)
						break;
					if ((++spins & 63u) == 0u) {
						if (__builtin_amdgcn_s_memrealtime() - t0 > S.wait_ticks) {
							stream_fail(S);
							ok = false;
							break;
						}
						if (st_ld_sys(&S.ctl->err)) {
							ok = false;
							break;
						}
					}
					__builtin_amdgcn_s_sleep(20);
				}
			}
			unsigned long long ah = 0;
			unsigned int drain = helper ? 1u : 0u;
			if (ok) {
				ah = j ? st_ld64(&S.sdev->desc[j].audio_host) : S.audio0;
				__builtin_amdgcn_fence(__ATOMIC_ACQUIRE, "agent");
				if (!helper) {
					const unsigned int df = st_ld(&S.sdev->drain_from);
					drain = (df && j + 1u >= df) ? 1u : 0u;
				}
				sh[7] = (helper || drain) ? 1u : st_ld(&S.sdev->post_fine[j]);
			}
			sh[5] = drain;
			sh[0] = ok ? 1u : 0u;
			sh[1] = (unsigned int)ah;
			sh[2] = (unsigned int)(ah >> 32);
			sh[3] = known;
		}
		__syncthreads();
		const bool go = sh[0] != 0u;
		const unsigned long long ah = ((unsigned long long)sh[2] << 32) | sh[1];
		known = sh[3];
		if (!go)
			break;
		WrPostArgs A = S.post;
		A.chan_iq = S.ring + (size_t)(j % WR_STREAM_RING) * S.k1 * S.slots * 2u;
		A.chan_prev = j ? S.ring + (size_t)((j - 1u) % WR_STREAM_RING) * S.k1 * S.slots * 2u : nullptr;
		A.prev_iq = S.prev_iq[S.parity0];
		A.dem_hist = S.dem[S.parity0];
		A.audio_host = (float *)ah;
		A.audio = S.audio_bufs[j & 3u];
#ifdef STREAM_TL
		const unsigned long long pt1 = __builtin_amdgcn_s_memtime();
		if (threadIdx.x == 0 && S.tl && !helper && p < 4u && j < 256u)
			S.tl[(7300u + j) * 8u + p * 2u] = __builtin_amdgcn_s_memrealtime();
#endif
		const bool drain = sh[5] != 0u;
		if (sh[7] != 0u) {
			A.run = S.drain_run;
			A.ntiles = S.drain_ntiles;
		}
		const unsigned int tasks_j = A.ntiles * A.groups;
		unsigned int mine = 0;
		const unsigned int rot = (unsigned int)(((unsigned long long)j * tasks) % S.n_post);
		for (unsigned int t = p >= rot ? p - rot : p + S.n_post - rot;; t += S.n_post) {
			if (drain) {
				if (threadIdx.x == 0)
					sh[4] = __hip_atomic_fetch_add(&S.sdev->post_ticket[j], 1u, __ATOMIC_RELAXED, __HIP_MEMORY_SCOPE_AGENT);
				__syncthreads();
				t = sh[4];
			}
			if (t >= tasks_j)
				break;
			post_role<D2, false>(A, t % A.ntiles, t / A.ntiles, stage, tile, modes);
			__syncthreads();
			++mine;
		}
		if (threadIdx.x == 0 && mine) {
			if (ah)
				__builtin_amdgcn_fence(__ATOMIC_RELEASE, "");
			else
				__builtin_amdgcn_fence(__ATOMIC_RELEASE, "agent");
			asm volatile("s_waitcnt vmcnt(0)" ::: "memory");
			__hip_atomic_fetch_add(&S.sdev->post_done[j], mine, __ATOMIC_RELAXED, __HIP_MEMORY_SCOPE_AGENT);
		}
#ifdef STREAM_TL
		if (threadIdx.x == 0 && S.tl && !helper && p < 4u && j < 256u)
			S.tl[(7300u + j) * 8u + p * 2u + 1u] = __builtin_amdgcn_s_memrealtime();
		if (threadIdx.x == 0) {
			const unsigned long long pt3 = __builtin_amdgcn_s_memtime();
			pt_wait += pt1 - pt0;
			pt_sync += pt3 - pt1;
			++pt_n;
		}
#endif
	}
#ifdef STREAM_TL
	if (threadIdx.x == 0 && S.tl && !helper) {
		S.tl[(6000u + p) * 8u + 0u] = pt_wait;
		S.tl[(6000u + p) * 8u + 1u] = pt_sync;
		S.tl[(6000u + p) * 8u + 2u] = pt_n;
	}
#endif
	if (!helper && p < S.post.groups && known && known <= WR_STREAM_MAXJ) {
		const unsigned int jl = known - 1u;
		WrPostArgs A = S.post;
		A.chan_iq = S.ring + (size_t)(jl % WR_STREAM_RING) * S.k1 * S.slots * 2u;
		A.chan_prev = jl ? S.ring + (size_t)((jl - 1u) % WR_STREAM_RING) * S.k1 * S.slots * 2u : nullptr;
		A.prev_iq = S.prev_iq[S.parity0];
		A.dem_hist = S.dem[S.parity0];
		A.prev_next = const_cast<float *>(S.prev_iq[S.parity0 ^ 1]);
		A.dem_hist_next = S.dem[S.parity0 ^ 1];
		post_role<D2, false>(A, A.ntiles, p, stage, tile, modes);
	}
}

template <unsigned int NG, unsigned int TS>
__device__ __forceinline__ void stream_ddc(const WrStreamArgs &S, v2f *lds)
{
	static_assert(TS == 1u || (TS == WR_TAPSETS && NG == 1u), "several channel filters: one lane group per wave");
	constexpr int NCO = WR_NCO_ROTATE;
	const unsigned int lane = threadIdx.x & 63u;
	const unsigned int wave = st_rfl(threadIdx.x >> 6);
	const unsigned int waves_per_wg = blockDim.x >> 6;
	const unsigned int wid = blockIdx.x * waves_per_wg + wave;
	wave_prio(3u);
	rot_tables_to_lds(lds, (const float2 *)S.hi_cs, (const float2 *)S.lo_cs);
	const v2f *hi_l = lds, *lo_l = lds + WR_SPLIT_N;
	const unsigned int nset = TS == 1u ? 1u : S.kmax;
	v2f *win = lds + 2u * WR_SPLIT_N + wave * (128u * nset);
	const unsigned int k1s = S.k1, d1 = S.d1;
	const unsigned int nwaves = S.n_ddc * waves_per_wg;
	const unsigned int gsets = S.groups / NG;
	const unsigned int wpg = nwaves / gsets;
	const unsigned int gs = wid % gsets;
	const unsigned int iw = wid / gsets;
	unsigned int known = 1;
	bool closed = false;
	if (iw < wpg) {
		const unsigned long long q0 = (unsigned long long)S.kslow + iw;
		LeanRec<NG> R = lean_rec<NG>([&](unsigned int s) { return S.phase[s]; }, S.step, S.flags, (const float4 *)S.rot,
		                             (float2 *)S.ring, S.gmap0, S.gmap1, gs, lane, (unsigned int)(q0 * d1 - WR_HIST), wpg, d1);
		const LeanWin<TS> W = lean_win<TS>(S.taps1u, S.tapsel, R.g0, lane, nset, win);
		unsigned int j = 0, k = (unsigned int)q0;
		while (k >= k1s) {
			k -= k1s;
			++j;
		}
		unsigned int jf = j, kf = k;
		unsigned int jb = 0xFFFFFFFFu;
		unsigned long long base_cur = 0, base_prev = 0;
		const bool u8 = S.is_u8 != 0u, ext = S.ext != 0u;
		unsigned int ahead = 0;
		bool drain = false;
		auto try_fetch = [&](float2 &dst) __attribute__((always_inline)) {
			if (drain)
				return;
			if (jf >= WR_STREAM_MAXJ) {
				drain = true;
				return;
			}
			if (jf >= known) {
				if (!closed) {
					const unsigned int r = st_ld(&S.sdev->ready);
					if (r > known)
						known = r;
					if (jf >= known && st_ld(&S.sdev->stop)) {
						const unsigned int f = st_ld(&S.sdev->ready);
						if (f > known)
							known = f;
						closed = true;
					}
				}
				if (jf >= known) {
					drain = true;
					return;
				}
			}
			if (jf != jb) {
				if (jf) {
					const unsigned long long a0 = __hip_atomic_load(&S.sdev->cur[jf], __ATOMIC_RELAXED, __HIP_MEMORY_SCOPE_AGENT);
					const unsigned long long a1 = __hip_atomic_load(&S.sdev->cur[jf + 1u], __ATOMIC_RELAXED, __HIP_MEMORY_SCOPE_AGENT);
					base_prev = ((unsigned long long)st_rfl((unsigned int)(a0 >> 32)) << 32) | st_rfl((unsigned int)a0);
					base_cur = ((unsigned long long)st_rfl((unsigned int)(a1 >> 32)) << 32) | st_rfl((unsigned int)a1);
				} else {
					base_prev = 0;
					base_cur = S.cur0;
				}
				jb = jf;
			}
			const long long n = (long long)kf * d1 - WR_HIST + lane;
			const unsigned long long base = (n >= 0) ? base_cur : base_prev;
			const unsigned long long idx = (n >= 0) ? (unsigned long long)n : (unsigned long long)((long long)S.nframes + n);
			if (ext) {
				if (u8) {
					const unsigned short b2 = __hip_atomic_load((const __attribute__((address_space(1))) unsigned short *)base + idx,
					                                            __ATOMIC_RELAXED, __HIP_MEMORY_SCOPE_AGENT);
					dst = make_float2(__builtin_bit_cast(float, (unsigned int)b2), 0.0f);
				} else {
					const unsigned long long x2 = __hip_atomic_load((const __attribute__((address_space(1))) unsigned long long *)base + idx,
					                                                __ATOMIC_RELAXED, __HIP_MEMORY_SCOPE_AGENT);
					dst = make_float2(__builtin_bit_cast(float, (unsigned int)x2), __builtin_bit_cast(float, (unsigned int)(x2 >> 32)));
				}
			} else if (u8) {
				const unsigned short b2 = ((const __attribute__((address_space(1))) unsigned short *)base)[idx];
				dst = make_float2(__builtin_bit_cast(float, (unsigned int)b2), 0.0f);
			} else {
				const v2f x2 = ((const __attribute__((address_space(1))) v2f *)base)[idx];
				dst = make_float2(x2.x, x2.y);
			}
			++ahead;
			kf += wpg;
			while (kf >= k1s) {
				kf -= k1s;
				++jf;
			}
		};
		unsigned int cnt = 0, pend_j = 0, pend_cnt = 0;
		unsigned int jring = 0xFFFFFFFFu;
		auto tell = [&]() __attribute__((always_inline)) {
			if (pend_cnt) {
				asm volatile("s_waitcnt vmcnt(0)" ::: "memory");
				if (lane == 0)
					__hip_atomic_fetch_add(&S.sdev->ddc_done[pend_j][wid % WR_STREAM_SHARDS][0], pend_cnt, __ATOMIC_RELAXED, __HIP_MEMORY_SCOPE_AGENT);
				pend_cnt = 0;
			}
		};
		static_assert(ROT_SEG == WR_FIR_LENGTH, "one recurrence over the whole window");
		float2 xa = make_float2(0.0f, 0.0f), xb = xa;
		unsigned long long tl_taps = 0, tl_rest = 0, tl_wait = 0, tl_units = 0, tl_ring = 0, tl_ringn = 0, tl_epochs = 0;
#ifdef STREAM_TL
		const bool tl_on = S.tl != nullptr;
#else
		constexpr bool tl_on = false;
#endif
		unsigned int lead = 0;
		auto unit = [&](float2 &xo, const int b) __attribute__((always_inline)) {
			const unsigned long long tl0 = tl_on ? __builtin_amdgcn_s_memtime() : 0ull;
			if (j != jring) {
				const unsigned long long pg = __hip_atomic_load(&S.sdev->progress, __ATOMIC_RELAXED, __HIP_MEMORY_SCOPE_AGENT);
				const unsigned int dr = st_rfl((unsigned int)pg), pr = st_rfl((unsigned int)(pg >> 32));
				lead = j > dr ? j - dr : 0u;
				if (j + 1u >= WR_STREAM_RING && pr < j - WR_STREAM_RING + 2u) {
					const unsigned long long tw0 = tl_on ? __builtin_amdgcn_s_memtime() : 0ull;
					tell();
					if (!stream_wait_count(S, (const unsigned int *)&S.sdev->progress + 1, j - WR_STREAM_RING + 2u)) {
						known = j;
						closed = true;
					}
					if (tl_on) {
						tl_ring += __builtin_amdgcn_s_memtime() - tw0;
						++tl_ringn;
#ifdef STREAM_TL
						if (lane == 0 && S.tl && (wid % 1000u) == 0u && j < 256u)
							S.tl[(7600u + j) * 8u + 4u + wid / 1000u] = __builtin_amdgcn_s_memrealtime();
#endif
					}
				}
				jring = j;
			}
			{
				wave_prio(lead <= 1u ? 2u : lead <= 3u ? 1u : 0u);
			}
			const AccN<NG> acc = rotate_unit<NG>(W.w4[b], R, S.table, hi_l, lo_l);
			const unsigned long long tl1 = tl_on ? __builtin_amdgcn_s_memtime() : 0ull;
			if (ahead >= 2u)
				W.to_lds(xo, b ^ 1, u8);
			unsigned long long tl2 = 0;
			if (tl_on) {
				asm volatile("s_waitcnt vmcnt(0) lgkmcnt(0)" ::: "memory");
				tl2 = __builtin_amdgcn_s_memtime();
			}
			tell();
			const size_t row = (size_t)(j % WR_STREAM_RING) * k1s + k;
#pragma unroll
			for (unsigned int c = 0; c < NG; ++c) {
				if (R.fl[c] & PHASE_FLAG_ACTIVE) {
					union { v2f f; unsigned long long u; } cv;
					cv.f = acc.v[c];
					__hip_atomic_store((unsigned long long *)&R.out[c][row * S.slots], cv.u, __ATOMIC_RELAXED,
					                   __HIP_MEMORY_SCOPE_AGENT);
				}
				R.Pk[c] += R.dP[c];
			}
			--ahead;
			cnt += NG;
			k += wpg;
			if (k >= k1s) {
				pend_j = j;
				pend_cnt = cnt;
				cnt = 0;
				do {
					k -= k1s;
					++j;
				} while (k >= k1s);
			}
			try_fetch(xo);
			if (tl_on) {
				const unsigned long long tl3 = __builtin_amdgcn_s_memtime();
				tl_taps += tl1 - tl0;
				tl_wait += tl2 - tl1;
				tl_rest += tl3 - tl2;
				++tl_units;
			}
		};
		for (;;) {
			if (j >= WR_STREAM_MAXJ || !stream_wait_ready(S, j, known, closed))
				break;
			drain = false;
			++tl_epochs;
			try_fetch(xa);
			try_fetch(xb);
			W.to_lds(xa, 0, u8);
			try_fetch(xa);
			wave_prio(2u);
			while (ahead) {
				unit(xb, 0);
				if (!ahead)
					break;
				unit(xa, 1);
			}
			wave_prio(3u);
			tell();
		}
		if (tl_on && lane == 0 && S.tl) {
			S.tl[wid * 8u + 0u] = tl_taps;
			S.tl[wid * 8u + 1u] = tl_wait;
			S.tl[wid * 8u + 2u] = tl_rest;
			S.tl[wid * 8u + 3u] = tl_units;
			S.tl[wid * 8u + 4u] = __builtin_amdgcn_s_getreg((31 << 11) | 4);
			S.tl[wid * 8u + 5u] = __builtin_amdgcn_s_getreg((31 << 11) | 20);
			S.tl[wid * 8u + 6u] = tl_ring;
			S.tl[wid * 8u + 7u] = (tl_ringn << 32) | tl_epochs;
		}
		asm volatile("s_waitcnt vmcnt(0)" ::: "memory");
		if (lane == 0) {
			if (pend_cnt)
				__hip_atomic_fetch_add(&S.sdev->ddc_done[pend_j][wid % WR_STREAM_SHARDS][0], pend_cnt, __ATOMIC_RELAXED, __HIP_MEMORY_SCOPE_AGENT);
			if (cnt && j < WR_STREAM_MAXJ)
				__hip_atomic_fetch_add(&S.sdev->ddc_done[j][wid % WR_STREAM_SHARDS][0], cnt, __ATOMIC_RELAXED, __HIP_MEMORY_SCOPE_AGENT);
		}
	}
	wave_prio(0u);
	(void)stream_wait_ready(S, 0xFFFFFFFEu, known, closed);
	const unsigned long long total = S.nframes * known;
	const unsigned int gtid = wid * 64u + lane, gsz = nwaves * 64u;
	const float *table = S.table;
	for (unsigned int s = gtid; s < S.slots; s += gsz) {
		const bool act = (S.flags[s] & PHASE_FLAG_ACTIVE) != 0;
		S.phase_next[s] = act ? S.phase[s] + (unsigned int)total * S.step[s] : S.phase[s];
	}
	for (unsigned int e = gtid; e < WR_HIST * S.slots; e += gsz) {
		const unsigned int r = e / S.slots, s = e - r * S.slots;
		const unsigned long long f = total + r;
		v2f cs = {0.0f, 0.0f}, lo = {0.0f, 0.0f};
		if (S.flags[s] & PHASE_FLAG_ACTIVE) {
			lo = nco<NCO>(S.phase[s] + (unsigned int)(f - WR_HIST) * S.step[s], table, hi_l, lo_l);
			cs = rot_into(S.phase[s], S.step[s], (unsigned int)(f - (WR_HIST - 1)), table);
		}
		((float2 *)S.hist_lo_next)[e] = make_float2(lo.x, lo.y);
		((float2 *)S.hist_cs_next)[e] = make_float2(cs.x, cs.y);
	}
	if (wid == 0 && known) {
		const unsigned long long c = known > 1u ? st_ld64(&S.sdev->desc[known - 1u].cur) : S.cur0;
		if (lane < WR_HIST) {
			const size_t n = (size_t)(S.nframes - WR_HIST + lane);
			float2 v;
			if (S.ext && S.is_u8) {
				const unsigned int b = __hip_atomic_load((const unsigned short *)c + n, __ATOMIC_RELAXED, __HIP_MEMORY_SCOPE_AGENT);
				v = make_float2(((float)(b & 255u) - 128.0f) / 128.0f, ((float)(b >> 8) - 128.0f) / 128.0f);
			} else if (S.ext) {
				const unsigned long long x = __hip_atomic_load((const unsigned long long *)c + n, __ATOMIC_RELAXED, __HIP_MEMORY_SCOPE_AGENT);
				v = make_float2(__builtin_bit_cast(float, (unsigned int)x), __builtin_bit_cast(float, (unsigned int)(x >> 32)));
			} else {
				v = input_frame(S.is_u8 ? nullptr : (const float2 *)c, S.is_u8 ? (const uchar2 *)c : nullptr, n);
			}
			((float2 *)S.hist_next)[lane] = v;
		}
		if (lane == 0)
			st_st_sys(&S.ctl->final_blocks, known);
	}
}

template <unsigned int PD2, unsigned int NG, unsigned int TS>
__global__ void __launch_bounds__(DDC_ROTATE_WAVES * 64u) __attribute__((amdgpu_waves_per_eu(DDC_NG2_WAVES_PER_EU)))
k_tuner_stream(const WrStreamArgs S)
{
	extern __shared__ v2f lds[];
	if (blockIdx.x >= S.n_ddc + S.n_post) {
		stream_bell(S);
		return;
	}
	const bool ddc = blockIdx.x < S.n_ddc;
	if (ddc) {
		stream_ddc<NG, TS>(S, lds);
		__syncthreads();
	}
	stream_post<PD2, TS>(S, ddc ? blockIdx.x : blockIdx.x - S.n_ddc, lds, ddc);
}

static unsigned int stream_post_run(unsigned int tiles, unsigned int groups, unsigned int max_post)
{
	unsigned int run = 1;
	while (run < tiles && ((tiles + run - 1u) / run) * groups > max_post)
		++run;
	return run;
}

static size_t stream_lds_bytes(unsigned int d2, unsigned int nset)
{
	const size_t post_lds = post_lds_bytes(d2, 1u) + 16u * sizeof(float);
	const size_t ddc_lds = (size_t)DDC_ROTATE_WAVES * 2u * 512u * nset + 2u * WR_SPLIT_N * 8u;
	return post_lds > ddc_lds ? post_lds : ddc_lds;
}

static void stream_shape(unsigned int groups, unsigned int kmax, bool one_filter, unsigned int *ng, unsigned int *ts)
{
	*ng = (one_filter && !(groups & 1u)) ? 2u : 1u;
	*ts = kmax > 1u ? WR_TAPSETS : 1u;
}

template <unsigned int PD2, unsigned int NG, unsigned int TS>
static hipError_t stream_occupancy(size_t lds, int *per_cu)
{
	static bool attr_done[WR_MAX_DEVICES];
	if (lds > 64 * 1024) {
		hipError_t e = allow_lds((const void *)k_tuner_stream<PD2, NG, TS>, lds, attr_done);
		if (e != hipSuccess)
			return e;
	}
	return hipOccupancyMaxActiveBlocksPerMultiprocessor(per_cu, k_tuner_stream<PD2, NG, TS>, (int)(DDC_ROTATE_WAVES * 64u), lds);
}

hipError_t wrk_stream_geometry(unsigned int d2, unsigned int groups, unsigned int kmax, bool one_filter, int num_cus,
                               unsigned int *n_ddc, unsigned int *n_post)
{
	*n_ddc = *n_post = 0;
	if (!wrk_tuner_post_supported(d2) || !groups || groups > 16u || !kmax || kmax > WR_TAPSETS)
		return hipSuccess;
	unsigned int ng, ts;
	stream_shape(groups, kmax, one_filter, &ng, &ts);
	const size_t lds = stream_lds_bytes(d2, ts == 1u ? 1u : kmax);
	int per_cu = 0;
	hipError_t e = with_post_d2(d2, [&](auto D2) {
		constexpr unsigned int PD2 = decltype(D2)::value;
		return ts != 1u ? stream_occupancy<PD2, 1, WR_TAPSETS>(lds, &per_cu)
		       : ng == 1u ? stream_occupancy<PD2, 1, 1>(lds, &per_cu) : stream_occupancy<PD2, 2, 1>(lds, &per_cu);
	});
	if (e != hipSuccess)
		return e;
	if (per_cu > 3)
		per_cu = 3;
	if (per_cu < 2)
		return hipSuccess;
	*n_ddc = (unsigned int)(per_cu - 1) * (unsigned int)num_cus;
	*n_post = (unsigned int)num_cus - 4u;
	return hipSuccess;
}

template <unsigned int PD2, unsigned int NG, unsigned int TS>
static hipError_t launch_stream(hipStream_t st, const WrStreamArgs &A, void *ev_start, void *ev_stop)
{
	const size_t lds = stream_lds_bytes(PD2, TS == 1u ? 1u : A.kmax);
	static bool attr_done[WR_MAX_DEVICES];
	if (lds > 64 * 1024) {
		hipError_t e = allow_lds((const void *)k_tuner_stream<PD2, NG, TS>, lds, attr_done);
		if (e != hipSuccess)
			return e;
	}
	const unsigned int grid = A.n_ddc + A.n_post + 1u;
	if (ev_start || ev_stop) {
		hipExtLaunchKernelGGL((k_tuner_stream<PD2, NG, TS>), dim3(grid), dim3(DDC_ROTATE_WAVES * 64u), (uint32_t)lds, st,
		                      (hipEvent_t)ev_start, (hipEvent_t)ev_stop, 0u, A);
		return hipGetLastError();
	}
	k_tuner_stream<PD2, NG, TS><<<grid, DDC_ROTATE_WAVES * 64u, lds, st>>>(A);
	return hipGetLastError();
}

hipError_t wrk_tuner_stream(hipStream_t st, const WrStreamArgs &A0, void *ev_start, void *ev_stop)
{
	WrStreamArgs A = A0;
	if (!A.n_ddc || !A.n_post || !A.groups || A.groups > 16u || !A.k1)
		return hipErrorInvalidValue;
	const unsigned int min_run = stream_post_run(A.post.tiles, A.post.groups, A.n_post);
	A.post.run = min_run;
	if (min_run >= 2u && A.n_post >= 8u)
		A.post.run = stream_post_run(A.post.tiles, A.post.groups, A.n_post / 2u);
	while (A.post.run < 4u && A.post.run < A.post.tiles &&
	       ((A.post.tiles + A.post.run - 1u) / A.post.run) * A.post.groups > A.n_post / 4u &&
	       ((A.post.tiles + A.post.run - 1u) / A.post.run) * A.post.groups <= A.n_post / 2u)
		++A.post.run;
	A.post.ntiles = (A.post.tiles + A.post.run - 1u) / A.post.run;
	A.drain_run = min_run < A.post.run ? min_run : A.post.run;
	A.drain_ntiles = (A.post.tiles + A.drain_run - 1u) / A.drain_run;
	const unsigned int tasks = A.post.ntiles * A.post.groups;
	(void)tasks;
	if (!A.kmax || A.kmax > WR_TAPSETS)
		return hipErrorInvalidValue;
	unsigned int ng, ts;
	stream_shape(A.groups, A.kmax, A.one_filter != 0u, &ng, &ts);
	if ((size_t)A.n_ddc * DDC_ROTATE_WAVES < A.groups / ng)
		return hipErrorInvalidValue;
	return with_post_d2(A.post.d2, [&](auto D2) {
		constexpr unsigned int PD2 = decltype(D2)::value;
		return ts != 1u ? launch_stream<PD2, 1, WR_TAPSETS>(st, A, ev_start, ev_stop)
		       : ng == 2u ? launch_stream<PD2, 2, 1>(st, A, ev_start, ev_stop)
		                  : launch_stream<PD2, 1, 1>(st, A, ev_start, ev_stop);
	});
}
```

webradio_amd/csrc/wr_tuner.hip:

```cpp
#include "wr_capi_internal.h"

static int dev_alloc_zero(void **p, size_t count, size_t elem)
{
	HIP_TRY(hipMalloc(p, (count ? count : 1) * elem));
	HIP_TRY(hipMemset(*p, 0, (count ? count : 1) * elem));
	HIP_TRY(hipStreamSynchronize(nullptr));
	return WR_OK;
}


unsigned int wrc_group_slots_used(const Group *g)
{
	unsigned int hi = 0;
	for (unsigned int s = 0; s < g->slots; ++s)
		if (g->owner[s] >= 0)
			hi = s + 1;
	return ((hi + WR_LANES - 1) / WR_LANES) * WR_LANES;
}

WrTunerLaunch wrc_group_launch(const wr_tuner *t, const Group *g, const float *cur, const uint8_t *cur_u8,
                               size_t nframes)
{
	WrTunerLaunch L;
	L.cur = cur;
// ... 445 lines not shown
	unsigned int *lens[3] = {&c->len1, &c->len2, &c->len1b};
	float *longs[3] = {c->taps_long, c->taps_long2, c->taps_long1b};
	*lens[stage] = len;
	if (len > WR_FIR_LENGTH)
		memcpy(longs[stage], coeff, sizeof(float) * len);
	if (len <= WR_FIR_LENGTH)
		memcpy(c->taps[stage], coeff, sizeof(float) * WR_FIR_LENGTH);
	c->decim[stage] = decim;
	c->have[stage] = true;
	return chan_seat(t, chan);
}

static bool fused_fir_length_ok(unsigned int n)
{
	return n >= 2 && n <= (unsigned int)WR_FIR_FUSED_MAX && (n & (n - 1)) == 0;
}

extern "C" int wr_chan_set_taps_n(wr_tuner *t, int chan, int stage, const float *coeff_host,
                                  unsigned int fir_length, unsigned int decimation)
{
	if (!t || !coeff_host)
		return wrc_fail(WR_ERR_ARG, "wr_chan_set_taps: bad argument");
	if (!fused_fir_length_ok(fir_length))
		return wrc_fail(WR_ERR_ARG, "wr_chan_set_taps_n: fir_length %u is not a power of two in [2, %d] (longer filters run "
		                        "block by block: wr_fir_decimate_n)", fir_length, WR_FIR_FUSED_MAX);
	float coeff[WR_FIR_FUSED_MAX] = {0.0f};
	memcpy(coeff, coeff_host, sizeof(float) * fir_length);
	return set_taps_common(t, chan, stage, coeff, decimation, fir_length > WR_FIR_LENGTH ? fir_length : (unsigned int)WR_FIR_LENGTH);
}

extern "C" int wr_chan_set_taps(wr_tuner *t, int chan, int stage, const float *coeff_host,
                                unsigned int decimation)
{
	return wr_chan_set_taps_n(t, chan, stage, coeff_host, WR_FIR_LENGTH, decimation);
}

extern "C" int wr_chan_set_filter_n(wr_tuner *t, int chan, int stage, unsigned int fir_length,
                                    unsigned int passband, unsigned int out_rate)
{
	Chan *c = chan_get(t, chan);
	if (!c)
		return g_settle_rc ? g_settle_rc : wrc_fail(WR_ERR_ARG, "wr_chan_set_filter: no channel %d", chan);
	if (stage < 0 || stage > 2)
		return wrc_fail(WR_ERR_ARG, "stage must be 0 (channel), 1 (audio) or 2 (second channel filter)");
	if (!fused_fir_length_ok(fir_length))
		return wrc_fail(WR_ERR_ARG, "wr_chan_set_filter_n: fir_length %u is not a power of two in [2, %d]", fir_length,
		                WR_FIR_FUSED_MAX);
	unsigned int in_rate;
	if (stage == 0) {
		in_rate = t->input_rate;
	} else {
		if (!c->have[0])
			return wrc_fail(WR_ERR_STATE, "set the channel filter (stage 0) before the %s", stage == 1 ? "audio filter"
			                : "second channel filter");
		in_rate = t->input_rate / c->decim[0];
		if (stage == 1 && c->have[2])
			in_rate /= c->decim[2];
	}
	if (!out_rate || out_rate > in_rate)
		return wrc_fail(WR_ERR_RATE, "output rate %u not a decimation of %u", out_rate, in_rate);
	unsigned int decim = in_rate / out_rate;
	if (in_rate / decim != out_rate || in_rate % out_rate)
		return wrc_fail(WR_ERR_RATE, "Sample rates must be integer related (%u -> %u)", in_rate, out_rate);
	float coeff[WR_FIR_FUSED_MAX] = {0.0f};
	wrd_lowpass_design(fir_length, passband, in_rate, coeff);
	return set_taps_common(t, chan, stage, coeff, decim, fir_length > WR_FIR_LENGTH ? fir_length : (unsigned int)WR_FIR_LENGTH);
}

extern "C" int wr_chan_set_filter(wr_tuner *t, int chan, int stage, unsigned int passband,
                                  unsigned int out_rate)
{
	return wr_chan_set_filter_n(t, chan, stage, WR_FIR_LENGTH, passband, out_rate);
}

extern "C" int wr_chan_set_mode(wr_tuner *t, int chan, int mode)
{
	Chan *c = chan_get(t, chan);
	if (!c)
		return g_settle_rc ? g_settle_rc : wrc_fail(WR_ERR_ARG, "wr_chan_set_mode: no channel %d", chan);
	if (mode < WR_AM || mode > WR_LSB)
		return wrc_fail(WR_ERR_ARG, "wr_chan_set_mode: bad mode %d", mode);
	c->mode = mode;
	chan_mark_dirty(t, c);
	return WR_OK;
}

extern "C" int wr_chan_set_af_gain(wr_tuner *t, int chan, float gain_db)
{
	Chan *c = chan_get(t, chan);
	if (!c)
		return g_settle_rc ? g_settle_rc : wrc_fail(WR_ERR_ARG, "wr_chan_set_af_gain: no channel %d", chan);
	if (!(gain_db == gain_db) || gain_db < -200.0f || gain_db > 200.0f)
		return wrc_fail(WR_ERR_ARG, "wr_chan_set_af_gain: %g dB", (double)gain_db);
	c->gain = (float)pow(10.0, (double)gain_db / 20.0);
	chan_mark_dirty(t, c);
	return WR_OK;
}

extern "C" int wr_chan_set_squelch(wr_tuner *t, int chan, float threshold_dbfs, int enable)
{
	Chan *c = chan_get(t, chan);
	if (!c)
		return g_settle_rc ? g_settle_rc : wrc_fail(WR_ERR_ARG, "wr_chan_set_squelch: no channel %d", chan);
	if (enable && (!(threshold_dbfs == threshold_dbfs) || threshold_dbfs < -300.0f || threshold_dbfs > 100.0f))
		return wrc_fail(WR_ERR_ARG, "wr_chan_set_squelch: %g dBFS", (double)threshold_dbfs);
	c->squelch = enable ? (float)pow(10.0, (double)threshold_dbfs / 10.0) : 0.0f;
	chan_mark_dirty(t, c);
	return WR_OK;
}

extern "C" int wr_tuner_keep_stages(wr_tuner *t, unsigned int stage_mask)
{
	if (!t)
		return wrc_fail(WR_ERR_ARG, "tuner is NULL");
	if (int rc = wrc_settle_held(t))
		return rc;
	t->keep_mask = stage_mask;
	return WR_OK;
}

extern "C" int wr_chan_get_state(wr_tuner *t, int chan, unsigned int *phase, float *prev_iq)
{
	Chan *c = chan_get(t, chan);
	if (!c)
		return g_settle_rc ? g_settle_rc : wrc_fail(WR_ERR_ARG, "wr_chan_get_state: no channel %d", chan);
	if (phase)
		*phase = c->phaseL >> 1;
	if (prev_iq) {
		if (c->group >= 0 && !c->prev_dirty) {
			Group *g = t->groups[c->group];
			if (wrc_dev_bind(t->dev))
				return WR_ERR_HIP;
			{
				int rc = wrc_tuner_quiesce(t);
				if (rc)
					return rc;
			}
			HIP_TRY(hipMemcpy(prev_iq, g->dev.prev_iq[g->parity] + 2 * c->slot, 2 * sizeof(float),
			                  hipMemcpyDeviceToHost));
		} else {
			prev_iq[0] = c->prev_iq[0];
			prev_iq[1] = c->prev_iq[1];
		}
	}
	return WR_OK;
}

extern "C" int wr_chan_set_state(wr_tuner *t, int chan, unsigned int phase, const float *prev_iq)
{
	Chan *c = chan_get(t, chan);
	if (!c)
		return g_settle_rc ? g_settle_rc : wrc_fail(WR_ERR_ARG, "wr_chan_set_state: no channel %d", chan);
	c->phaseL = phase << 1;
	c->phase_dirty = true;
	if (prev_iq) {
		c->prev_iq[0] = prev_iq[0];
		c->prev_iq[1] = prev_iq[1];
		c->prev_dirty = true;
	}
	chan_mark_dirty(t, c);
	return WR_OK;
}

extern "C" int wr_chan_slot(wr_tuner *t, int chan, int *slot)
{
	Chan *c = chan_get(t, chan);
	if (!c || !slot)
		return g_settle_rc ? g_settle_rc : wrc_fail(WR_ERR_ARG, "wr_chan_slot: bad argument");
	if (c->group < 0)
		return wrc_fail(WR_ERR_STATE, "channel %d has no filters yet", chan);
	*slot = c->slot;
	return WR_OK;
}

namespace {
struct GroupFilters {
	std::vector<float> taps1u;
	std::vector<float> taps2u;
	std::vector<int> tapsel;
};
}

template <typename Taps>
static int lane_group_rep(const wr_tuner *t, const Group *g, size_t base, Taps taps, unsigned int len, bool *same)
{
	int rep = -1;
	*same = true;
	for (size_t s = base; s < base + WR_LANES && *same; ++s) {
		const int ci = g->owner[s];
		if (ci < 0)
			continue;
		if (rep < 0)
			rep = ci;
		else
			*same = !memcmp(taps(t->chans[ci]), taps(t->chans[rep]), sizeof(float) * len);
	}
	return rep;
}

static void group_classify(const wr_tuner *t, Group *g, GroupFilters &F)
{
	const size_t S = g->slots;
	int first_rep = -1;
	g->uniform_taps = g->one_filter = true;
	g->uniform_mask = g->fewsets_mask = g->uniform2_mask = 0;
	memset(g->nsets, 0, sizeof(g->nsets));
	F.taps1u.assign(S * WR_TAPSETS, 0.0f);
	F.tapsel.assign(S, 0);
	for (size_t base = 0; base < S; base += WR_LANES) {
		const size_t grp = base / WR_LANES;
		int reps[WR_TAPSETS];
		unsigned int nrep = 0;
		bool few = true;
		for (size_t s = base; s < base + WR_LANES; ++s) {
			int ci = g->owner[s];
			if (ci < 0)
				continue;
			unsigned int q = 0;
			for (; q < nrep; ++q)
				if (!memcmp(t->chans[ci].taps[0], t->chans[reps[q]].taps[0], sizeof(float) * WR_FIR_LENGTH))
					break;
			if (q == nrep) {
				if (nrep == WR_TAPSETS) {
					few = false;
					break;
				}
				reps[nrep++] = ci;
			}
			F.tapsel[s] = (int)q;
		}
		if (nrep) {
			if (first_rep < 0)
				first_rep = reps[0];
			if (nrep > 1 || !few ||
			    memcmp(t->chans[reps[0]].taps[0], t->chans[first_rep].taps[0], sizeof(float) * WR_FIR_LENGTH))
				g->one_filter = false;
		}
		if (!few || grp >= 64) {
			for (size_t s = base; s < base + WR_LANES; ++s)
				F.tapsel[s] = 0;
			if (nrep)
				g->uniform_taps = false;
			continue;
		}
		for (unsigned int q = 0; q < nrep; ++q)
			for (size_t j = 0; j < WR_LANES; ++j)
				F.taps1u[(grp * WR_TAPSETS + q) * WR_LANES + j] = t->chans[reps[q]].taps[0][WR_FIR_LENGTH - 1 - j];
		g->nsets[grp] = (unsigned char)(nrep ? nrep : 1);
		g->fewsets_mask |= 1ull << grp;
		if (nrep <= 1)
			g->uniform_mask |= 1ull << grp;
		else
			g->uniform_taps = false;
	}
	g->one_filter = g->one_filter && first_rep >= 0;
	const unsigned int l2 = g->l2;
	const auto audio_taps = [l2](const Chan &c) { return l2 > WR_FIR_LENGTH ? c.taps_long2 : c.taps[1]; };
	F.taps2u.assign(S / WR_LANES * l2, 0.0f);
	for (size_t base = 0; base < S && base / WR_LANES < 64; base += WR_LANES) {
		bool same = true;
		const int rep = lane_group_rep(t, g, base, audio_taps, l2, &same);
		if (!same || rep < 0)
			continue;
		memcpy(&F.taps2u[base / WR_LANES * l2], audio_taps(t->chans[rep]), sizeof(float) * l2);
		g->uniform2_mask |= 1ull << (base / WR_LANES);
	}
	g->long_uniform = g->long_one = false;
	if (g->l1 > WR_FIR_LENGTH) {
		const auto long_taps = [](const Chan &c) { return c.taps_long; };
		g->long_uniform = g->long_one = true;
		int rep_all = -1;
		for (size_t base = 0; base < S && g->long_uniform; base += WR_LANES) {
			const int rep = lane_group_rep(t, g, base, long_taps, g->l1, &g->long_uniform);
			if (rep >= 0) {
				if (rep_all < 0)
					rep_all = rep;
				else if (memcmp(t->chans[rep].taps_long, t->chans[rep_all].taps_long, sizeof(float) * g->l1))
					g->long_one = false;
			}
		}
		g->long_one = g->long_one && g->long_uniform;
	}
	if (g->one_filter)
		for (size_t grp = 0; grp < S / WR_LANES; ++grp)
			for (size_t j = 0; j < WR_LANES; ++j)
				F.taps1u[(grp * WR_TAPSETS) * WR_LANES + j] = t->chans[first_rep].taps[0][WR_FIR_LENGTH - 1 - j];
}

int wrc_group_upload(wr_tuner *t, Group *g)
{
	const size_t S = g->slots;
	hipStream_t st = t->dev->stream;
	{
		int rc = wrc_tuner_quiesce(t);
		if (rc)
			return rc;
	}
	std::vector<unsigned int> step(S, 0);
	std::vector<int> flags(S, 0), mode(S, -1);
	std::vector<float> taps1(S * WR_FIR_LENGTH, 0.0f), taps2(S * g->l2, 0.0f);
	std::vector<float> taps1b(g->d1b ? S * g->l1b : 0, 0.0f), gain(S, 1.0f), squelch(S, 0.0f);
	std::vector<float> taps1L(g->l1 > WR_FIR_LENGTH ? S * g->l1 : 0, 0.0f);
	g->use_gain = g->use_squelch = false;
	for (size_t s = 0; s < S; ++s) {
		int ci = g->owner[s];
		if (ci < 0)
			continue;
		Chan &c = t->chans[ci];
		step[s] = c.stepL;
		mode[s] = c.mode;
		flags[s] = 1;
		for (int j = 0; j < WR_FIR_LENGTH; ++j)
			taps1[(size_t)j * S + s] = c.taps[0][j];
		for (unsigned int j = 0; j < g->l2; ++j)
			taps2[(size_t)j * S + s] = g->l2 > WR_FIR_LENGTH ? c.taps_long2[j] : c.taps[1][j];
		if (g->d1b)
			for (unsigned int j = 0; j < g->l1b; ++j)
				taps1b[(size_t)j * S + s] = g->l1b > WR_FIR_LENGTH ? c.taps_long1b[j] : c.taps[2][j];
		if (g->l1 > WR_FIR_LENGTH)
			for (unsigned int j = 0; j < g->l1; ++j)
				taps1L[(size_t)j * S + s] = c.taps_long[j];
		gain[s] = c.gain;
		squelch[s] = c.squelch;
		g->use_gain = g->use_gain || c.gain != 1.0f;
		g->use_squelch = g->use_squelch || c.squelch > 0.0f;
	}
	GroupFilters F;
	group_classify(t, g, F);
	std::vector<float> rot(S * 4, 0.0f);
	{
		const float *turn = t->dev->turn_host;
		for (size_t s = 0; s < S; ++s) {
			const unsigned int Sx = step[s] >> 16;
			rot[4 * s + 0] = turn[(Sx + 16384u) & 0xFFFFu];
			rot[4 * s + 1] = turn[Sx & 0xFFFFu];
			rot[4 * s + 2] = turn[(Sx + 16385u) & 0xFFFFu];
			rot[4 * s + 3] = turn[(Sx + 1u) & 0xFFFFu];
		}
	}
	HIP_TRY(hipMemcpyAsync(g->dev.step, step.data(), S * sizeof(unsigned int), hipMemcpyHostToDevice, st));
	HIP_TRY(hipMemcpyAsync(g->dev.flags, flags.data(), S * sizeof(int), hipMemcpyHostToDevice, st));
	HIP_TRY(hipMemcpyAsync(g->dev.mode, mode.data(), S * sizeof(int), hipMemcpyHostToDevice, st));
	HIP_TRY(hipMemcpyAsync(g->dev.taps1, taps1.data(), taps1.size() * sizeof(float), hipMemcpyHostToDevice, st));
	if (g->l1 > WR_FIR_LENGTH)
		HIP_TRY(hipMemcpyAsync(g->dev.taps1L, taps1L.data(), taps1L.size() * sizeof(float), hipMemcpyHostToDevice, st));
	HIP_TRY(hipMemcpyAsync(g->dev.taps2, taps2.data(), taps2.size() * sizeof(float), hipMemcpyHostToDevice, st));
	HIP_TRY(hipMemcpyAsync(g->dev.rot, rot.data(), rot.size() * sizeof(float), hipMemcpyHostToDevice, st));
	HIP_TRY(hipMemcpyAsync(g->dev.taps1u, F.taps1u.data(), F.taps1u.size() * sizeof(float), hipMemcpyHostToDevice, st));
	HIP_TRY(hipMemcpyAsync(g->dev.taps2u, F.taps2u.data(), F.taps2u.size() * sizeof(float), hipMemcpyHostToDevice, st));
	HIP_TRY(hipMemcpyAsync(g->dev.tapsel, F.tapsel.data(), F.tapsel.size() * sizeof(int), hipMemcpyHostToDevice, st));
	HIP_TRY(hipMemcpyAsync(g->dev.gain, gain.data(), S * sizeof(float), hipMemcpyHostToDevice, st));
	HIP_TRY(hipMemcpyAsync(g->dev.squelch, squelch.data(), S * sizeof(float), hipMemcpyHostToDevice, st));
	if (g->d1b)
		HIP_TRY(hipMemcpyAsync(g->dev.taps1b, taps1b.data(), taps1b.size() * sizeof(float), hipMemcpyHostToDevice, st));
	for (size_t s = 0; s < S; ++s) {
		int ci = g->owner[s];
		if (ci < 0)
			continue;
		Chan &c = t->chans[ci];
		if (c.phase_dirty) {
			HIP_TRY(hipMemcpyAsync(g->dev.phase[g->sp] + s, &c.phaseL, sizeof(unsigned int), hipMemcpyHostToDevice, st));
			c.phase_dirty = false;
			if (t->nco_mode == WR_NCO_ROTATE)
				c.cs_hist_reset = true;
		}
		if (c.prev_dirty) {
			HIP_TRY(hipMemcpyAsync(g->dev.prev_iq[g->parity] + 2 * s, c.prev_iq, 2 * sizeof(float), hipMemcpyHostToDevice, st));
			c.prev_dirty = false;
		}
		if (c.cs_hist_reset) {
			HIP_TRY(hipMemset2DAsync(g->dev.hist_cs[g->sp] + 2 * s, S * 2 * sizeof(float), 0, 2 * sizeof(float),
			                         WR_HIST, st));
			HIP_TRY(hipMemset2DAsync(g->dev.hist_lo[g->sp] + 2 * s, S * 2 * sizeof(float), 0, 2 * sizeof(float),
			                         WR_HIST, st));
			HIP_TRY(hipMemset2DAsync(g->dev.iq2_hist[g->p2] + 2 * s, S * 2 * sizeof(float), 0, 2 * sizeof(float),
			                         g->l1b - 1, st));
			if (g->l1 > WR_FIR_LENGTH)
				HIP_TRY(hipMemset2DAsync(g->dev.mixhist[g->sp] + 2 * s, S * 2 * sizeof(float), 0, 2 * sizeof(float),
				                         g->l1 - 1, st));
			c.cs_hist_reset = false;
		}
		if (c.dem_hist_reset) {
			HIP_TRY(hipMemset2DAsync(g->dev.dem[g->parity] + s, S * sizeof(float), 0, sizeof(float), g->l2 - 1, st));
			c.dem_hist_reset = false;
		}
	}
	HIP_TRY(hipStreamSynchronize(st));
	g->dirty = false;
	return WR_OK;
}

static int prof_drain(wr_tuner *t, size_t keep)
{
	if (t->ev_used / 2 <= keep)
		return WR_OK;
	HIP_TRY(wrc_dev_stream_sync(t->dev));
	for (size_t i = 0; i + 1 < t->ev_used; i += 2) {
		float ms = 0.0f;
		HIP_TRY(hipEventElapsedTime(&ms, t->ev[i], t->ev[i + 1]));
		const unsigned int span = (i / 2 < t->ev_span.size() && t->ev_span[i / 2]) ? t->ev_span[i / 2] : 1u;
		t->prof_ms += ms;
		t->prof_n += span;
	}
	t->ev_used = 0;
	t->ev_span.clear();
	return WR_OK;
}

static int prof_reserve_pair(wr_tuner *t)
{
	if (int rc = (t->ev_used & 1) ? WR_OK : prof_drain(t, 64))
		return rc;
	while (t->ev.size() < t->ev_used + 2) {
		hipEvent_t e;
		HIP_TRY(hipEventCreate(&e));
		t->ev.push_back(e);
	}
	return WR_OK;
}

int wrc_prof_pair_begin(wr_tuner *t, void **ev_start, void **ev_stop)
{
	if (int rc = prof_reserve_pair(t))
		return rc;
	*ev_start = t->ev[t->ev_used];
	*ev_stop = t->ev[t->ev_used + 1];
	return WR_OK;
}

void wrc_prof_pair_stamped(wr_tuner *t)
{
	t->ev_span.resize(t->ev_used / 2 + 1, 1u);
	t->ev_used += 2;
}

extern "C" int wr_tuner_profile(wr_tuner *t, int enable)
{
	if (!t)
		return wrc_fail(WR_ERR_ARG, "tuner is NULL");
	if (int rc = wrc_settle_held(t))
		return rc;
	if (t->ev_used & 1)
		t->ev_used--;
	t->profiling = enable != 0;
	t->prof_stride = enable > 1 ? (unsigned int)enable : 1u;
	t->prof_tick = 0;
	return WR_OK;
}

extern "C" int wr_tuner_profile_read(wr_tuner *t, unsigned int *launches, double *mean_ms)
{
	if (!t || !launches || !mean_ms)
		return wrc_fail(WR_ERR_ARG, "wr_tuner_profile_read: bad argument");
	if (wrc_dev_bind(t->dev))
		return WR_ERR_HIP;
	if (int rc = wrc_settle_held(t))
		return rc;
	int rc = prof_drain(t, 0);
	if (rc)
		return rc;
	*launches = t->prof_n;
	*mean_ms = t->prof_n ? t->prof_ms / t->prof_n : 0.0;
	t->prof_ms = 0.0;
	t->prof_n = 0;
	return WR_OK;
}

static bool block_can_be_held(const wr_tuner *t, size_t nframes)
{
	for (const Group *g : t->groups) {
		if (g->active <= 0)
			continue;
		const size_t q = (size_t)g->d1 * (g->d1b ? g->d1b : 1u) * g->d2;
		if (!q || nframes % q)
			return false;
	}
	return true;
}

static int submit_precheck(const wr_tuner *t, size_t nframes, int where)
{
	if (nframes > t->max_block_frames)
		return wrc_fail(WR_ERR_ARG, "wr_tuner_submit: %zu frames exceeds max_block_frames %zu", nframes,
		                t->max_block_frames);
	if (where != WR_HOST && where != WR_DEVICE)
		return wrc_fail(WR_ERR_ARG, "wr_tuner_submit: bad `where`");
	for (const Chan &c : t->chans)
		if (c.in_use && c.group < 0)
			return wrc_fail(WR_ERR_STATE, "a channel has no filters (LowPass::init: \"Must specify either "
			                          "decimation or output rate\")");
	return WR_OK;
}

void wrc_advance_phases(wr_tuner *t, unsigned long long frames)
{
	for (Chan &c : t->chans) {
		if (!c.in_use || c.group < 0)
			continue;
		c.phaseL += (unsigned int)frames * c.stepL;
	}
}

struct Submit {
	const float *cur;
	const uint8_t *cur_u8;
	size_t nframes;
	unsigned long long seq;
	bool prof_now, group_first, group_last;
	bool hist_written = false;
	bool marked = false, unmarked = false;
};

static int submit_stage_host(wr_tuner *t, const void *iq, size_t nframes, bool *u8)
{
	wr_dev *d = t->dev;
	hipStream_t st = d->stream;
	if (!t->in_stage)
		HIP_TRY(hipMalloc((void **)&t->in_stage, t->max_block_frames * 2 * sizeof(float)));
	bool sparse = false;
	if (nframes && !(((uintptr_t)iq | (uintptr_t)t->in_stage) & 15u)) {
		unsigned int sd = 0, sl = 0;
		bool same = true;
		for (const Group *g : t->groups) {
			if (g->active <= 0)
				continue;
			if (!sd) {
				sd = g->d1;
				sl = g->l1;
			} else if (g->d1 != sd || g->l1 != sl) {
				same = false;
			}
		}
		void *mapped = nullptr;
		if (same && sd && sd >= 2u * sl && nframes >= 4u * (size_t)sd) {
			if (iq != t->probe_ptr || t->probe_gen != d->reg_gen || !t->probe_left--) {
				mapped = wrc_host_mapped(iq);
				if (!mapped) {
					t->probe_ptr = iq;
					t->probe_gen = d->reg_gen;
					t->probe_left = 64;
				}
			}
		}
		if (mapped) {
			HIP_TRY(wrk_stage_windows(st, mapped, *u8, t->in_stage, nframes, sd, sl, sl - 1u));
			if (int rc = wrc_upload_mark(d, st))
				return rc;
			sparse = true;
		}
	}
	if (nframes && !sparse)
		HIP_TRY(hipMemcpyAsync(t->in_stage, iq, nframes * 2 * (*u8 ? sizeof(uint8_t) : sizeof(float)),
		                       hipMemcpyHostToDevice, st));
	t->last_staging = sparse ? 2 : 1;
	if (sparse)
		*u8 = false;
	return WR_OK;
}

static int submit_post(wr_tuner *t, Group *g, const Submit &S, const WrTunerLaunch &L, const WrTunerLaunch &Lp,
                       const WrGroupDev &Gp, bool two_kernels)
{
	hipStream_t st = t->dev->stream;
	const bool long_rides = g->l1 > WR_FIR_LENGTH && g->long_uniform;
	const bool defer = !two_kernels && (g->l1 <= WR_FIR_LENGTH || long_rides) && Lp.k1 && t->defer_post &&
	                   t->nco_mode == WR_NCO_ROTATE && g->l2 == WR_FIR_LENGTH;
	if (two_kernels) {
		HIP_TRY(wrk_tuner_demod(st, Lp, Gp));
		HIP_TRY(wrk_tuner_audio(st, Lp, Gp));
	} else if (defer) {
		g->post_pending = true;
		g->post_args = wrk_post_args(Lp, Gp);
		g->pend_seq = S.seq;
		g->pend_k2 = Lp.k2;
		g->pend_slots = L.slots_used;
		g->post_args.audio_host = wrc_ring_reserve(t, g, Lp.k2, L.slots_used);
		g->post_args.host_stride = Lp.k2;
		g->pend_direct = g->post_args.audio_host != nullptr;
	} else {
		HIP_TRY(wrk_tuner_post(st, Lp, Gp));
	}
	if (!defer)
		return wrc_ring_push(t, g, S.seq, Lp.k2, L.slots_used, false);
	return WR_OK;
}

static int submit_group(wr_tuner *t, Group *g, Submit &S)
{
	wr_dev *d = t->dev;
	hipStream_t st = d->stream;
	if (g->dirty)
		if (int rc = wrc_group_upload(t, g))
			return rc;
	WrTunerLaunch L = wrc_group_launch(t, g, S.cur, S.cur_u8, S.nframes);
	if (S.group_first)
		if (int rc = prof_reserve_pair(t))
			return rc;
	if (S.prof_now) {
		if (int rc = wrc_prof_pair_begin(t, &L.ev_start, &L.ev_stop))
			return rc;
		if (t->mark_launches)
			S.unmarked = true;
	} else if (t->mark_launches && g->l1 <= WR_FIR_LENGTH) {
		L.ev_start = nullptr;
		L.ev_stop = t->launch_ev[(t->launches_marked + 1) % 4];
		S.marked = true;
	} else if (t->mark_launches) {
		S.unmarked = true;
	}
	if (S.group_first && !(t->ev_used & 1)) {
		HIP_TRY(hipEventRecord(t->ev[t->ev_used], st));
		t->ev_used += 1;
	}
	const bool two_kernels = (t->keep_mask & (1u << WR_STAGE_DEMOD)) != 0 || !wrk_tuner_post_supported(L.d2);
	WrGroupDev Gs = g->dev;
	if (g->seek_pending) {
		if (two_kernels || g->d1b || g->l1 > WR_FIR_LENGTH) {
			if (g->post_pending)
				if (int rc = post_send_pending(t, g, false))
					return rc;
			int rc = seek_materialize(t, g);
			if (rc)
				return rc;
		} else {
			L.seeking = true;
			L.seek_lo = (unsigned int)g->seek_frame;
			Gs.hist_cs[g->sp] = g->z_hist;
			Gs.hist_lo[g->sp] = g->z_hist;
// ... 459 lines not shown
```

webradio_amd/csrc/wr_tuner_stream.hip:

```cpp
#include "wr_capi_internal.h"


static unsigned long long *g_stream_tl = nullptr;
extern "C" int wr_debug_stream_tl(unsigned long long *out, size_t n)
{
	if (!g_stream_tl)
		return 1;
	memcpy(out, g_stream_tl, n * sizeof(unsigned long long));
	return 0;
}

static std::mutex g_stream_mu;
static wr_tuner *g_stream_on[WR_MAX_DEVICES];

static void stream_raw_free(wr_tuner::Stream &s)
{
	for (uint8_t *&r : s.raw) {
		(void)hipFree(r);
		r = nullptr;
	}
	s.raw_cap = 0;
}

void wrc_stream_free(wr_tuner *t)
{
	wr_tuner::Stream &s = t->stream;
	(void)hipHostFree(s.ctl);
	(void)hipHostFree(s.desc);
	(void)hipFree(s.sdev);
	(void)hipFree(s.ring);
	stream_raw_free(s);
	if (s.raw_ev)
		(void)hipEventDestroy(s.raw_ev);
	s.raw_ev = nullptr;
	s.ctl = nullptr;
	s.desc = nullptr;
	s.sdev = nullptr;
	s.ring = nullptr;
	s.ring_floats = 0;
}

int wrc_stream_check(wr_tuner *t)
{
	wr_tuner::Stream &s = t->stream;
	if (!s.unchecked)
		return WR_OK;
	s.unchecked = false;
	s.long_blocks += s.ctl->long_blocks;
	s.ctl->long_blocks = 0;
	if (s.ctl->err)
		return wrc_fail(WR_ERR_HIP, "streaming launch: a wait inside the launch ran into its deadline (code %u)", s.ctl->err);
	if (s.ctl->final_blocks != s.count)
		return wrc_fail(WR_ERR_STATE, "streaming launch: %u blocks rung, %u processed%s", s.count, s.ctl->final_blocks,
		                s.ctl->self_closed ? " (the launch had closed itself: the doorbell was silent too long)" : "");
	return WR_OK;
}

bool wrc_stream_follows(const wr_tuner *t, size_t nframes, int where, bool u8)
{
	const wr_tuner::Stream &s = t->stream;
	if (!s.live || !s.enabled || where != WR_DEVICE || nframes != s.nframes || u8 != s.u8 || s.count >= WR_STREAM_MAXJ)
		return false;
	if (s.g->dirty)
		return false;
	const auto idle = std::chrono::steady_clock::now() - s.last_bell;
	return idle < std::chrono::milliseconds(WR_STREAM_STALE_MS);
}

int wrc_stream_bell(wr_tuner *t, const void *iq, bool behind_upload)
{
	wr_tuner::Stream &s = t->stream;
	const unsigned int j = s.count;
	const unsigned long long seq = t->submit_seq++;
	float *slot = wrc_stream_ring_entry(t, s.g, seq, s.k2, wrc_group_slots_used(s.g), j);
	s.desc[j].cur = (unsigned long long)(uintptr_t)iq;
	s.desc[j].audio_host = (unsigned long long)(uintptr_t)slot;
	s.desc[j].count = j + 1u;
	std::atomic_thread_fence(std::memory_order_release);
	if (behind_upload) {
		HIP_TRY(hipStreamWriteValue32(t->dev->up_stream, &s.sdev->ready_up, j + 1u, 0));
		s.up_pending = true;
	} else {
		if (s.up_pending) {
			HIP_TRY(hipStreamSynchronize(t->dev->up_stream));
			s.up_pending = false;
		}
		s.ctl->ready = j + 1u;
	}
	std::atomic_thread_fence(std::memory_order_seq_cst);
	s.count = j + 1u;
	++s.blocks;
	s.last_bell = std::chrono::steady_clock::now();
	return WR_OK;
}

int wrc_stream_open(wr_tuner *t, const void *iq, size_t nframes, bool u8, bool *took)
{
	*took = false;
	wr_tuner::Stream &s = t->stream;
	wr_dev *d = t->dev;
	if (t->nco_mode != WR_NCO_ROTATE || !t->defer_post || t->mark_launches || (t->keep_mask & (1u << WR_STAGE_DEMOD)))
		return WR_OK;
	Group *g = wrc_single_group(t);
	if (!g || g->l1 != WR_FIR_LENGTH || g->l2 != WR_FIR_LENGTH || g->d1b || g->seek_pending || !wrk_tuner_post_supported(g->d2))
		return WR_OK;
	if (nframes < (size_t)WR_FIR_LENGTH * g->d1 || nframes % ((size_t)g->d1 * g->d2) || nframes / g->d1 > 0x3FFFFFFFu)
		return WR_OK;
	if (wrc_dev_bind(d))
		return WR_ERR_HIP;
	if (int rc = wrc_tuner_launch_held(t))
		return rc;
	if (g->dirty)
		if (int rc = wrc_group_upload(t, g))
			return rc;
	const unsigned int used = wrc_group_slots_used(g), groups = used / 64u;
	if (!groups || groups > 16u)
		return WR_OK;
	const unsigned long long used_mask = (1ull << groups) - 1ull;
	if ((g->fewsets_mask & used_mask) != used_mask)
		return WR_OK;
	unsigned int kmax = 1;
	for (unsigned int gi = 0; gi < groups; ++gi)
		if (g->nsets[gi] > kmax)
			kmax = g->nsets[gi];
	if (int rc = wrc_dev_settle_stream(d))
		return rc;
	{
		std::lock_guard<std::mutex> lk(g_stream_mu);
		if (d->device < 0 || d->device >= WR_MAX_DEVICES || (g_stream_on[d->device] && g_stream_on[d->device] != t))
			return WR_OK;
	}
	if (s.unchecked) {
		HIP_TRY(wrc_dev_stream_sync(d));
		if (int rc = wrc_stream_check(t))
			return rc;
	}
	if (g->post_pending)
		if (int rc = wrc_tuner_flush(t))
			return rc;
	const size_t k1 = nframes / g->d1, k2 = k1 / g->d2;
	unsigned int n_ddc = 0, n_post = 0;
	HIP_TRY(wrk_stream_geometry(g->d2, groups, kmax, g->one_filter, d->num_cus, &n_ddc, &n_post));
	if (!n_ddc || !n_post)
		return WR_OK;
	if (!s.ctl)
		HIP_TRY(hipHostMalloc((void **)&s.ctl, sizeof(WrStreamCtl), hipHostMallocMapped | hipHostMallocCoherent));
	if (!s.desc)
		HIP_TRY(hipHostMalloc((void **)&s.desc, sizeof(WrStreamDesc) * WR_STREAM_MAXJ, hipHostMallocMapped | hipHostMallocCoherent));
	if (!s.sdev)
		HIP_TRY(hipMalloc((void **)&s.sdev, sizeof(WrStreamDev)));
	const size_t ring_floats = (size_t)WR_STREAM_RING * k1 * g->slots * 2u;
	if (ring_floats > s.ring_floats) {
		HIP_TRY(wrc_dev_stream_sync(d));
		(void)hipFree(s.ring);
		s.ring = nullptr;
		s.ring_floats = 0;
		HIP_TRY(hipMalloc((void **)&s.ring, ring_floats * sizeof(float)));
		s.ring_floats = ring_floats;
	}
	void *ctl_dev = nullptr, *desc_dev = nullptr;
	HIP_TRY(hipHostGetDevicePointer(&ctl_dev, s.ctl, 0));
	HIP_TRY(hipHostGetDevicePointer(&desc_dev, s.desc, 0));
	hipStream_t st = d->stream;

	const WrTunerLaunch L = wrc_group_launch(t, g, u8 ? nullptr : (const float *)iq, u8 ? (const uint8_t *)iq : nullptr, nframes);

	WrStreamArgs A;
	memset(&A, 0, sizeof(A));
	A.ctl = (WrStreamCtl *)ctl_dev;
	A.desc_host = (const WrStreamDesc *)desc_dev;
	A.sdev = s.sdev;
	A.idle_ticks = (unsigned long long)WR_STREAM_IDLE_MS * 100000ull;
	A.wait_ticks = (unsigned long long)WR_STREAM_WAIT_MS * 100000ull;
	A.n_ddc = n_ddc;
	A.n_post = n_post;
	if (getenv("WR_STREAM_TL") && atoi(getenv("WR_STREAM_TL"))) {
		static unsigned long long *tlbuf = nullptr;
		if (!tlbuf)
			HIP_TRY(hipHostMalloc((void **)&tlbuf, 8192 * 8 * sizeof(unsigned long long), hipHostMallocMapped | hipHostMallocCoherent));
		memset(tlbuf, 0, 8192 * 8 * sizeof(unsigned long long));
		void *tld = nullptr;
		HIP_TRY(hipHostGetDevicePointer(&tld, tlbuf, 0));
		A.tl = (unsigned long long *)tld;
		g_stream_tl = tlbuf;
	}
	A.nframes = nframes;
	A.k1 = (unsigned int)k1;
	A.d1 = g->d1;
	A.is_u8 = u8 ? 1u : 0u;
	A.ext = s.ext ? 1u : 0u;
	A.slots = g->slots;
	A.groups = groups;
	for (unsigned int gi = 0; gi < groups; ++gi)
		(gi < 8u ? A.gmap0 : A.gmap1) |= (unsigned long long)gi << ((gi & 7u) * 8u);
	A.kslow = (WR_HIST + g->d1 - 1u) / g->d1;
	if (A.kslow > k1)
		A.kslow = (unsigned int)k1;
	A.hist = L.hist;
	A.hist_next = L.hist_next;
	A.phase = g->dev.phase[g->sp];
	A.step = g->dev.step;
	A.phase_next = g->dev.phase[g->sp ^ 1];
	A.hist_cs = g->dev.hist_cs[g->sp];
	A.hist_lo = g->dev.hist_lo[g->sp];
	A.hist_cs_next = g->dev.hist_cs[g->sp ^ 1];
	A.hist_lo_next = g->dev.hist_lo[g->sp ^ 1];
	A.flags = g->dev.flags;
	A.taps1 = g->dev.taps1;
	A.rot = g->dev.rot;
	A.taps1u = g->dev.taps1u;
	A.tapsel = g->dev.tapsel;
	A.table = d->table_turn;
	A.hi_cs = d->hi_cs;
	A.lo_cs = d->lo_cs;
	A.ring = s.ring;
	for (int i = 0; i < 4; ++i)
		A.audio_bufs[i] = g->dev.audio_set[(g->audio_cur + i) & 3];
	A.post = wrk_post_args(L, g->dev);
	A.post.host_stride = k2;
	A.prev_iq[0] = g->dev.prev_iq[0];
	A.prev_iq[1] = g->dev.prev_iq[1];
	A.dem[0] = g->dev.dem[0];
	A.dem[1] = g->dev.dem[1];
	A.parity0 = g->parity;
	A.kmax = kmax;
	A.one_filter = g->one_filter ? 1u : 0u;

	++s.gen;
	s.g = g;
	s.count = 0;
	s.nframes = nframes;
	s.u8 = u8;
	s.parity0 = g->parity;
	s.k1 = k1;
	s.k2 = k2;
	s.last_iq = nullptr;
	const unsigned long long seq = t->submit_seq++;
	float *slot = wrc_stream_ring_entry(t, g, seq, k2, used, 0);
	s.ctl->ready = 1;
	s.ctl->stop = 0;
	s.ctl->done = 0;
	s.ctl->final_blocks = 0;
	s.ctl->long_blocks = 0;
	s.ctl->err = 0;
	s.ctl->self_closed = 0;
	s.desc[0].cur = (unsigned long long)(uintptr_t)iq;
	s.desc[0].audio_host = (unsigned long long)(uintptr_t)slot;
	std::atomic_thread_fence(std::memory_order_seq_cst);
	if (s.ext) {
		HIP_TRY(hipMemsetAsync(s.sdev, 0, offsetof(WrStreamDev, ready_up), st));
		const size_t after = offsetof(WrStreamDev, ready_up) + sizeof(unsigned int);
		HIP_TRY(hipMemsetAsync((char *)s.sdev + after, 0, offsetof(WrStreamDev, desc) - after, st));
	} else {
		HIP_TRY(hipMemsetAsync(s.sdev, 0, offsetof(WrStreamDev, desc), st));
	}
	A.cur0 = s.desc[0].cur;
	A.audio0 = s.desc[0].audio_host;

	void *ev0 = nullptr, *ev1 = nullptr;
	if (t->profiling && !(t->ev_used & 1))
		if (int rc = wrc_prof_pair_begin(t, &ev0, &ev1))
			return rc;
	HIP_TRY(wrk_tuner_stream(st, A, ev0, ev1));
	if (ev0)
		wrc_prof_pair_stamped(t);
	s.live = true;
	s.count = 1;
	++s.blocks;
	s.last_bell = std::chrono::steady_clock::now();
	d->streaming = t;
	{
		std::lock_guard<std::mutex> lk(g_stream_mu);
		g_stream_on[d->device] = t;
	}
	*took = true;
	return WR_OK;
}

int wrc_stream_host_u8(wr_tuner *t, const uint8_t *bytes, size_t nframes, bool *took)
{
	*took = false;
	wr_tuner::Stream &s = t->stream;
	wr_dev *d = t->dev;
	if (wrc_dev_bind(d))
		return WR_ERR_HIP;
	if (!wrc_host_mapped(bytes))
		return WR_OK;
	const size_t need = nframes * 2;
	if (need <= WR_STREAM_HOST_MIN_BYTES)
		return WR_OK;
	const bool follows = s.live && s.ext && wrc_stream_follows(t, nframes, WR_DEVICE, true);
	if (need > s.raw_cap) {
		if (int rc = wrc_stream_close(t))
			return rc;
		HIP_TRY(wrc_dev_stream_sync(d));
		if (d->up_stream)
			HIP_TRY(hipStreamSynchronize(d->up_stream));
		stream_raw_free(s);
		for (uint8_t *&r : s.raw)
			HIP_TRY(hipMalloc((void **)&r, need));
		s.raw_cap = need;
	}
	const unsigned int slot = (unsigned int)(s.raw_next & 3u);
	const unsigned int through = s.raw_idx[slot] + 2u < s.count ? s.raw_idx[slot] + 2u : s.count;
	if ((s.live || s.unchecked) && s.raw_gen[slot] == s.gen && s.ctl->done < through) {
		const auto t0 = std::chrono::steady_clock::now();
		while (s.ctl->done < through && !s.ctl->err)
			if (std::chrono::steady_clock::now() - t0 > std::chrono::milliseconds(4 * WR_STREAM_WAIT_MS))
				return wrc_fail(WR_ERR_HIP, "streaming launch: block %u did not finish", s.raw_idx[slot] + 1u);
	}
	{
		std::lock_guard<std::mutex> up_guard(*d->upload_lock);
		if (int rc = wrc_dev_up_stream(d))
			return rc;
		HIP_TRY(hipMemcpyAsync(s.raw[slot], bytes, need, hipMemcpyHostToDevice, d->up_stream));
		if (int rc = wrc_upload_mark_locked(d, d->up_stream))
			return rc;
	}
	if (follows) {
		s.raw_gen[slot] = s.gen;
		s.raw_idx[slot] = s.count;
		++s.raw_next;
		++s.host_blocks;
		t->last_staging = 3;
		*took = true;
		return wrc_stream_bell(t, s.raw[slot], true);
	}
	if (int rc = wrc_stream_close(t))
		return rc;
	if (!s.raw_ev)
		HIP_TRY(hipEventCreateWithFlags(&s.raw_ev, hipEventDisableTiming));
	if (!s.sdev)
		HIP_TRY(hipMalloc((void **)&s.sdev, sizeof(WrStreamDev)));
	HIP_TRY(hipStreamWriteValue32(d->up_stream, &s.sdev->ready_up, 0u, 0));
	HIP_TRY(hipEventRecord(s.raw_ev, d->up_stream));
	HIP_TRY(hipStreamWaitEvent(d->stream, s.raw_ev, 0));
	s.ext = true;
	bool opened = false;
	if (int rc = wrc_stream_open(t, s.raw[slot], nframes, true, &opened))
		return rc;
	s.raw_gen[slot] = opened ? s.gen : 0;
	s.raw_idx[slot] = 0;
	++s.raw_next;
	*took = true;
	if (opened) {
		++s.host_blocks;
		t->last_staging = 3;
		return WR_OK;
	}
	s.ext = false;
	t->last_staging = 1;
	return wrc_tuner_submit_now(t, s.raw[slot], nframes, WR_DEVICE, true);
}

int wrc_stream_close(wr_tuner *t)
{
	wr_tuner::Stream &s = t->stream;
	if (!s.live)
		return WR_OK;
	if (s.up_pending) {
		HIP_TRY(hipStreamSynchronize(t->dev->up_stream));
		s.ctl->ready = s.count;
		s.up_pending = false;
	}
	std::atomic_thread_fence(std::memory_order_seq_cst);
	s.ctl->stop = 1;
	std::atomic_thread_fence(std::memory_order_seq_cst);
	s.live = false;
	s.unchecked = true;
	if (t->dev->streaming == t)
		t->dev->streaming = nullptr;
	{
		std::lock_guard<std::mutex> lk(g_stream_mu);
		if (g_stream_on[t->dev->device] == t)
			g_stream_on[t->dev->device] = nullptr;
	}
	Group *g = s.g;
	const unsigned int J = s.count;
	for (Group *x : t->groups)
		if (x != g)
			x->last_k1 = x->last_k2 = 0;
	g->sp ^= 1;
	g->last_parity = s.parity0;
	g->parity = s.parity0 ^ 1;
	g->last_k1 = s.k1;
	g->last_k2 = s.k2;
	g->last_demod_kept = false;
	s.last_iq = s.ring + (size_t)((J - 1u) % WR_STREAM_RING) * s.k1 * g->slots * 2u;
	g->audio_cur = (int)((g->audio_cur + (J - 1u)) & 3u);
	g->dev.audio = g->dev.audio_set[g->audio_cur];
	t->in_par ^= 1;
	wrc_advance_phases(t, (unsigned long long)s.nframes * J);
	t->submitted = true;
	return WR_OK;
}

extern "C" int wr_tuner_set_streaming(wr_tuner *t, int enable)
{
	if (!t)
		return wrc_fail(WR_ERR_ARG, "tuner is NULL");
	if (wrc_dev_bind(t->dev))
		return WR_ERR_HIP;
	if (int rc = wrc_tuner_launch_held(t))
		return rc;
	t->stream.enabled = enable != 0;
	t->stream.host_bytes = enable >= 2;
	return WR_OK;
}

extern "C" int wr_tuner_stream_info(wr_tuner *t, int *live, unsigned long long *launches, unsigned long long *blocks)
{
	if (!t)
		return wrc_fail(WR_ERR_ARG, "tuner is NULL");
	if (live)
		*live = t->stream.live ? 1 : 0;
	if (launches)
		*launches = t->stream.gen;
	if (blocks)
		*blocks = t->stream.blocks;
	return WR_OK;
}

extern "C" int wr_tuner_stream_long_blocks(wr_tuner *t, unsigned long long *blocks)
{
	if (!t || !blocks)
		return wrc_fail(WR_ERR_ARG, "wr_tuner_stream_long_blocks: bad argument");
	*blocks = t->stream.long_blocks;
	return WR_OK;
}

extern "C" int wr_tuner_stream_host_blocks(wr_tuner *t, unsigned long long *blocks)
{
	if (!t || !blocks)
		return wrc_fail(WR_ERR_ARG, "wr_tuner_stream_host_blocks: bad argument");
	*blocks = t->stream.host_blocks;
	return WR_OK;
}
```

webradio_amd/device.py:

```python
import ctypes as C

import numpy as np

from . import capi
from .capi import check, ptr


class Device:

    def __init__(self, index=0, stream=None):
        self.lib = capi.load()
        h = C.c_void_p()
        check(self.lib.wr_dev_open(C.byref(h), index, ptr(stream) if stream else None))
        self.h = h
        self.index = index

    def close(self):
        if self.h:
            self.lib.wr_dev_close(self.h)
            self.h = None

    def sync(self):
        check(self.lib.wr_dev_sync(self.h))

    def malloc(self, nbytes):
        p = C.c_void_p()
        check(self.lib.wr_dev_malloc(self.h, nbytes, C.byref(p)))
        return p.value

    def free(self, p):
        check(self.lib.wr_dev_free(self.h, C.c_void_p(p)))

    def upload(self, arr):
        arr = np.ascontiguousarray(arr)
        p = self.malloc(max(arr.nbytes, 4))
        check(self.lib.wr_dev_upload(self.h, C.c_void_p(p), ptr(arr), arr.nbytes))
        return p

    def download(self, p, count, dtype=np.float32):
        out = np.empty(count, dtype=dtype)
        check(self.lib.wr_dev_download(self.h, ptr(out), C.c_void_p(p), out.nbytes))
        return out

    def mix(self, iq, phase, phase_step):
        iq = np.ascontiguousarray(iq, dtype=np.float32)
        n = iq.size // 2
        din = self.upload(iq)
        dout = self.malloc(max(iq.nbytes, 4))
        ph = C.c_uint(phase)
        check(self.lib.wr_mix(self.h, C.c_void_p(din), C.c_void_p(dout), n, C.byref(ph), phase_step))
        out = self.download(dout, 2 * n)
        self.free(din)
        self.free(dout)
        return out, ph.value

    def fir_decimate(self, x, channels, decimation, coeff, history_dev):
        x = np.ascontiguousarray(x, dtype=np.float32)
        nframes = x.size // channels
        nout = (nframes // decimation) * channels
        din = self.upload(x)
        dout = self.malloc(max(nout * 4, 4))
        coeff = np.ascontiguousarray(coeff, dtype=np.float32)
        check(self.lib.wr_fir_decimate_n(self.h, C.c_void_p(din), nframes, channels, decimation, coeff.size,
                                         ptr(coeff), C.c_void_p(history_dev), C.c_void_p(dout)))
        out = self.download(dout, nout)
        self.free(din)
        self.free(dout)
        return out

    def demod(self, mode, iq, prev):
        iq = np.ascontiguousarray(iq, dtype=np.float32)
        n = iq.size // 2
        din = self.upload(iq)
        dout = self.malloc(max(n * 4, 4))
        prev = np.array(prev, dtype=np.float32)
        check(self.lib.wr_demod(self.h, mode, C.c_void_p(din), n, ptr(prev), C.c_void_p(dout)))
        out = self.download(dout, n)
        self.free(din)
        self.free(dout)
        return out, prev


class Tuner:

    def __init__(self, dev, input_rate, max_channels, max_block_frames, nco=capi.WR_NCO_ROTATE):
        self.dev = dev
        self.lib = dev.lib
        h = C.c_void_p()
        check(self.lib.wr_tuner_create(C.byref(h), dev.h, input_rate, max_channels, max_block_frames, nco))
        self.h = h
        self.input_rate = input_rate

    def destroy(self):
        if self.h:
            self.lib.wr_tuner_destroy(self.h)
            self.h = None

    def add_receiver(self, if_hz, chan_passband, chan_rate, mode, audio_passband, audio_rate, fir_lengths=None,
                     stage2=None):
        c = C.c_int()
        check(self.lib.wr_chan_add(self.h, C.byref(c)))
        ch = c.value
        check(self.lib.wr_chan_set_if(self.h, ch, if_hz))
        l1, l2 = fir_lengths if fir_lengths else (capi.WR_FIR_LENGTH, capi.WR_FIR_LENGTH)
        check(self.lib.wr_chan_set_filter_n(self.h, ch, 0, l1, chan_passband, chan_rate))
        if stage2:
            check(self.lib.wr_chan_set_filter_n(self.h, ch, 2, stage2[0], stage2[1], stage2[2]))
        check(self.lib.wr_chan_set_filter_n(self.h, ch, 1, l2, audio_passband, audio_rate))
        check(self.lib.wr_chan_set_mode(self.h, ch, mode))
        return ch

    def keep_stages(self, *stages):
        mask = 0
        for st in stages:
            mask |= 1 << st
        check(self.lib.wr_tuner_keep_stages(self.h, mask))

    def flush(self):
        check(self.lib.wr_tuner_flush(self.h))

    def blocks_per_launch(self, n):
        check(self.lib.wr_tuner_set_blocks_per_launch(self.h, n))

    def streaming(self, enable=True):
        check(self.lib.wr_tuner_set_streaming(self.h, int(enable) if enable is not True else 1))

    def stream_info(self):
        live, launches, blocks = C.c_int(), C.c_ulonglong(), C.c_ulonglong()
        check(self.lib.wr_tuner_stream_info(self.h, C.byref(live), C.byref(launches), C.byref(blocks)))
        return bool(live.value), launches.value, blocks.value

    def stream_host_blocks(self):
        n = C.c_ulonglong()
        check(self.lib.wr_tuner_stream_host_blocks(self.h, C.byref(n)))
        return n.value

    def stream_long_blocks(self):
        n = C.c_ulonglong()
        check(self.lib.wr_tuner_stream_long_blocks(self.h, C.byref(n)))
        return n.value

    def mark_launches(self, enable=True):
        check(self.lib.wr_tuner_mark_launches(self.h, 1 if enable else 0))

    def seek(self, frame):
        check(self.lib.wr_tuner_seek(self.h, C.c_ulonglong(frame)))

    def fetch_audio_all(self):
        stride, frames, slots = C.c_size_t(), C.c_size_t(), C.c_uint()
        self.lib.wr_tuner_fetch_audio_all(self.h, None, 0, C.byref(stride), C.byref(frames), C.byref(slots))
        out = np.empty(max(1, slots.value * frames.value), dtype=np.float32)
        check(self.lib.wr_tuner_fetch_audio_all(self.h, ptr(out), out.size, C.byref(stride), C.byref(frames),
                                                C.byref(slots)))
        return out[: slots.value * frames.value].reshape(slots.value, frames.value)

    def slot(self, ch):
        s = C.c_int()
        check(self.lib.wr_chan_slot(self.h, ch, C.byref(s)))
        return s.value

    def audio_ring(self, depth):
        check(self.lib.wr_tuner_audio_ring(self.h, depth))

    def ring_acquire(self):
        p = C.POINTER(C.c_float)()
        stride, frames, slots, seq = C.c_size_t(), C.c_size_t(), C.c_uint(), C.c_ulonglong()
        check(self.lib.wr_tuner_audio_ring_acquire(self.h, C.byref(p), C.byref(stride), C.byref(frames),
                                                   C.byref(slots), C.byref(seq)))
        n = slots.value * stride.value
        a = np.ctypeslib.as_array(p, shape=(n,)).copy() if n else np.zeros(0, np.float32)
        return a.reshape(slots.value, stride.value)[:, : frames.value], seq.value

    def ring_release(self):
        check(self.lib.wr_tuner_audio_ring_release(self.h))

    def ring_stats(self):
        q, o = C.c_uint(), C.c_ulonglong()
        check(self.lib.wr_tuner_audio_ring_stats(self.h, C.byref(q), C.byref(o)))
        return q.value, o.value

    def submit_count(self):
        n = C.c_ulonglong()
        check(self.lib.wr_tuner_submit_count(self.h, C.byref(n)))
        return n.value

    def remove_receiver(self, ch):
        check(self.lib.wr_chan_remove(self.h, ch))

    def set_if(self, ch, if_hz):
        check(self.lib.wr_chan_set_if(self.h, ch, if_hz))

    def set_af_gain(self, ch, gain_db):
        check(self.lib.wr_chan_set_af_gain(self.h, ch, C.c_float(gain_db)))

    def set_squelch(self, ch, threshold_dbfs, enable=True):
        check(self.lib.wr_chan_set_squelch(self.h, ch, C.c_float(threshold_dbfs), 1 if enable else 0))

    def set_mode(self, ch, mode):
        check(self.lib.wr_chan_set_mode(self.h, ch, mode))

    def set_filter(self, ch, stage, passband, out_rate):
        check(self.lib.wr_chan_set_filter(self.h, ch, stage, passband, out_rate))

    def submit_host(self, iq):
        iq = np.ascontiguousarray(iq, dtype=np.float32)
        check(self.lib.wr_tuner_submit(self.h, ptr(iq), iq.size // 2, capi.WR_HOST))
        self.dev.sync()

    def submit_device(self, dev_ptr, nframes):
        check(self.lib.wr_tuner_submit(self.h, ptr(dev_ptr), nframes, capi.WR_DEVICE))

    def submit_u8_host(self, raw):
        check(self.lib.wr_tuner_submit_u8(self.h, raw.ctypes.data_as(C.c_void_p), raw.size // 2, capi.WR_HOST))

    def last_staging(self):
        how = C.c_int()
        check(self.lib.wr_tuner_last_staging(self.h, C.byref(how)))
        return how.value

    def submit_u8_device(self, dev_ptr, nframes):
        check(self.lib.wr_tuner_submit_u8(self.h, ptr(dev_ptr), nframes, capi.WR_DEVICE))

    def fetch(self, ch, stage, capacity):
        out = np.empty(max(capacity, 1), dtype=np.float32)
        n = C.c_size_t()
        check(self.lib.wr_chan_fetch(self.h, ch, stage, ptr(out), capacity, C.byref(n)))
        return out[: n.value].copy()

    def state(self, ch):
        ph = C.c_uint()
        prev = np.zeros(2, dtype=np.float32)
        check(self.lib.wr_chan_get_state(self.h, ch, C.byref(ph), ptr(prev)))
        return ph.value, prev

    def set_state(self, ch, phase, prev=None):
        p = None if prev is None else np.ascontiguousarray(prev, dtype=np.float32)
        check(self.lib.wr_chan_set_state(self.h, ch, phase, ptr(p)))

    def profile(self, enable):
        check(self.lib.wr_tuner_profile(self.h, int(enable)))

    def profile_read(self):
        n = C.c_uint()
        ms = C.c_double()
        check(self.lib.wr_tuner_profile_read(self.h, C.byref(n), C.byref(ms)))
        return n.value, ms.value

    def audio_dev(self):
        a = C.c_void_p()
        stride = C.c_size_t()
        frames = C.c_size_t()
        check(self.lib.wr_tuner_audio_dev(self.h, C.byref(a), C.byref(stride), C.byref(frames)))
        return a.value, stride.value, frames.value


class Spectrum:

    def __init__(self, dev, fft_size, hop=0):
        self.dev = dev
        self.lib = dev.lib
        self.n = fft_size
        h = C.c_void_p()
        check(self.lib.wr_spectrum_create(C.byref(h), dev.h, fft_size, hop))
        self.h = h

    def destroy(self):
        if self.h:
            self.lib.wr_spectrum_destroy(self.h)
            self.h = None

    def push_host(self, iq):
        iq = np.ascontiguousarray(iq, dtype=np.float32)
        check(self.lib.wr_spectrum_push(self.h, ptr(iq), iq.size // 2, capi.WR_HOST))

    def push_device(self, dev_ptr, nframes):
        check(self.lib.wr_spectrum_push(self.h, ptr(dev_ptr), nframes, capi.WR_DEVICE))

    def get_db(self):
        out = np.empty(self.n, dtype=np.float32)
        check(self.lib.wr_spectrum_get_db(self.h, ptr(out)))
        return out

    def get_bins(self):
        out = np.empty(2 * self.n, dtype=np.float32)
        check(self.lib.wr_spectrum_get_bins(self.h, ptr(out)))
        return out

    def waterfall_row(self, width, hold=0):
        db = np.empty(width, dtype=np.float32)
        pal = np.empty(width, dtype=np.uint8)
        check(self.lib.wr_spectrum_get_waterfall_row(self.h, width, hold, ptr(db), ptr(pal)))
        return db, pal

    def frames_done(self):
        n = C.c_ulong()
        check(self.lib.wr_spectrum_frames_done(self.h, C.byref(n)))
        return n.value

    def lazy_info(self):
        a, b = C.c_ulonglong(), C.c_ulonglong()
        check(self.lib.wr_spectrum_lazy_info(self.h, C.byref(a), C.byref(b)))
        return a.value, b.value

    def batch_db(self, iq_dev, nframes_fft, db_dev):
        check(self.lib.wr_spectrum_batch_db(self.h, ptr(iq_dev), nframes_fft, ptr(db_dev)))


class Ring:

    @staticmethod
    def make_id():
        lib = capi.load()
        buf = (C.c_ubyte * lib.wr_ring_id_bytes())()
        check(lib.wr_ring_make_id(buf, len(buf)))
        return bytes(buf)

    @staticmethod
    def rccl_version():
        v = C.c_int()
        check(capi.load().wr_ring_version(C.byref(v)))
        return v.value

    def __init__(self, dev, id_bytes, rank, world):
        self.lib = capi.load()
        h = C.c_void_p()
        buf = (C.c_ubyte * len(id_bytes)).from_buffer_copy(id_bytes)
        check(self.lib.wr_ring_create(C.byref(h), dev.h, buf, len(id_bytes), rank, world))
        self.h, self.rank, self.world = h, rank, world

    def exchange(self, send_dev, recv_dev, nfloats):
        check(self.lib.wr_ring_exchange(self.h, ptr(send_dev), ptr(recv_dev), nfloats))

    def exchange_after(self, tuner, send_dev, recv_dev, nfloats):
        check(self.lib.wr_ring_exchange_after(self.h, tuner.h, ptr(send_dev), ptr(recv_dev), nfloats))

    def wait(self):
        check(self.lib.wr_ring_wait(self.h))

    def exchanges(self):
        n = C.c_ulonglong()
        check(self.lib.wr_ring_info(self.h, None, None, C.byref(n)))
        return n.value

    def destroy(self):
        if self.h:
            self.lib.wr_ring_destroy(self.h)
            self.h = None
```

Baseline: 117,600.

## Fuse FM demod into DDC stage for runs of consecutive output rows

In the streaming kernel, when every channel is FM with no squelch, one filter and paired groups, each DDC wave now computes runs of consecutive decimated rows instead of strided rows. Within a run it computes the FM discriminator directly from the previous sample carried in LDS, and writes one float per row to a new demod ring instead of writing complex IQ. The post stage reads the precomputed demod values for inner rows and still demodulates run boundaries from IQ. This is meant to cut IQ ring traffic and the post-stage demod work, at the cost of extra LDS, a lean flag per block, and more complex indexing.

```diff
diff --git a/include/webradio_amd.h b/include/webradio_amd.h
--- a/include/webradio_amd.h
+++ b/include/webradio_amd.h
@@ -161,10 +161,12 @@
 int wr_tuner_set_blocks_per_launch(wr_tuner *tuner, unsigned int nblocks);
 
 #define WR_STREAM_MAX_BLOCKS 512u
+#define WR_STREAM_RUN 5u
 int wr_tuner_set_streaming(wr_tuner *tuner, int enable);
 int wr_tuner_stream_info(wr_tuner *tuner, int *live, unsigned long long *launches, unsigned long long *blocks);
 int wr_tuner_stream_host_blocks(wr_tuner *tuner, unsigned long long *blocks);
 int wr_tuner_stream_long_blocks(wr_tuner *tuner, unsigned long long *blocks);
+int wr_tuner_stream_lean_blocks(wr_tuner *tuner, unsigned long long *blocks);
 
 int wr_tuner_profile(wr_tuner *tuner, int enable);
 int wr_tuner_profile_read(wr_tuner *tuner, unsigned int *launches, double *mean_ms);
diff --git a/webradio_amd/capi.py b/webradio_amd/capi.py
--- a/webradio_amd/capi.py
+++ b/webradio_amd/capi.py
@@ -11,6 +11,7 @@
 WR_HOST, WR_DEVICE = 0, 1
 WR_ABI_VERSION = 6
 WR_STREAM_MAX_BLOCKS = 512
+WR_STREAM_RUN = 5
 WR_FIR_LENGTH = 64
 WR_TABLE_SIZE = 65536
 
@@ -70,6 +71,7 @@
     "wr_tuner_stream_info": (C.c_int, [_vp, C.POINTER(C.c_int), C.POINTER(C.c_ulonglong), C.POINTER(C.c_ulonglong)]),
     "wr_tuner_stream_host_blocks": (C.c_int, [_vp, C.POINTER(C.c_ulonglong)]),
     "wr_tuner_stream_long_blocks": (C.c_int, [_vp, C.POINTER(C.c_ulonglong)]),
+    "wr_tuner_stream_lean_blocks": (C.c_int, [_vp, C.POINTER(C.c_ulonglong)]),
     "wr_tuner_seek": (C.c_int, [_vp, C.c_ulonglong]),
     "wr_tuner_audio_ring": (C.c_int, [_vp, _u32]),
     "wr_tuner_audio_ring_acquire": (C.c_int, [_vp, C.POINTER(C.POINTER(C.c_float)), C.POINTER(C.c_size_t),
diff --git a/webradio_amd/csrc/wr_capi_internal.h b/webradio_amd/csrc/wr_capi_internal.h
--- a/webradio_amd/csrc/wr_capi_internal.h
+++ b/webradio_amd/csrc/wr_capi_internal.h
@@ -86,6 +86,7 @@
 	unsigned int l1b = WR_FIR_LENGTH;
 	int p2 = 0;
 	bool use_gain = false, use_squelch = false;
+	bool all_fm = false;
 	unsigned int slots;
 	size_t k1max, k2max;
 	WrGroupDev dev;
@@ -179,6 +180,8 @@
 		WrStreamDev *sdev = nullptr;
 		float *ring = nullptr;
 		size_t ring_floats = 0;
+		float *dem_ring = nullptr;
+		size_t dem_ring_floats = 0;
 		Group *g = nullptr;
 		unsigned int count = 0;
 		size_t nframes = 0;
@@ -199,6 +202,7 @@
 		bool up_pending = false;
 		unsigned long long host_blocks = 0;
 		unsigned long long long_blocks = 0;
+		unsigned long long lean_blocks = 0;
 	} stream;
 };
 
diff --git a/webradio_amd/csrc/wr_internal.h b/webradio_amd/csrc/wr_internal.h
--- a/webradio_amd/csrc/wr_internal.h
+++ b/webradio_amd/csrc/wr_internal.h
@@ -120,6 +120,10 @@
 	float       *audio_host;
 	size_t       host_stride;
 	unsigned int nseg = 1;
+	const float *dem_rows = nullptr;
+	const float *dem_rows_prev = nullptr;
+	unsigned int lean_cur = 0, lean_prev = 0;
+	unsigned int off_cur = 0, off_prev = 0;
 	const float *chan_prev = nullptr;
 };
 long wrk_tune_ng2_min_passes(long value, bool set);
@@ -161,7 +165,8 @@
 	volatile unsigned int err;
 	volatile unsigned int self_closed;
 	volatile unsigned int long_blocks;
-	volatile unsigned int pad1[11];
+	volatile unsigned int lean_blocks;
+	volatile unsigned int pad1[10];
 };
 #define WR_STREAM_SHARDS 16u
 struct WrStreamDev {
@@ -174,6 +179,7 @@
 	unsigned int pad1[29];
 	unsigned int post_done[WR_STREAM_MAXJ];
 	unsigned int post_fine[WR_STREAM_MAXJ];
+	unsigned int lean[WR_STREAM_MAXJ];
 	unsigned int post_ticket[WR_STREAM_MAXJ];
 	unsigned int ddc_done[WR_STREAM_MAXJ][WR_STREAM_SHARDS][32];
 	WrStreamDesc desc[WR_STREAM_MAXJ];
@@ -206,6 +212,7 @@
 	const int          *tapsel;
 	const float        *table, *hi_cs, *lo_cs;
 	float              *ring;
+	float              *dem_ring;
 	float              *audio_bufs[4];
 	WrPostArgs          post;
 	unsigned int        drain_run, drain_ntiles;
@@ -213,6 +220,7 @@
 	float              *dem[2];
 	int                 parity0;
 	unsigned int        one_filter;
+	unsigned int        lean;
 };
 #define WR_STREAM_ERR_WAIT   1u
 hipError_t wrk_stream_geometry(unsigned int d2, unsigned int groups, unsigned int kmax, bool one_filter, int num_cus,
diff --git a/webradio_amd/csrc/wr_kernels.hip b/webradio_amd/csrc/wr_kernels.hip
--- a/webradio_amd/csrc/wr_kernels.hip
+++ b/webradio_amd/csrc/wr_kernels.hip
@@ -375,7 +375,35 @@
 	return demod_one(m, z.x, z.y, zp.x, zp.y);
 }
 
-template <unsigned int D2, bool HREGS, unsigned int NSEG = 1u>
+__device__ __forceinline__ bool lean_inner(unsigned int k, unsigned int off, unsigned int k1)
+{
+	const unsigned int pos = (k + off) % WR_STREAM_RUN;
+	return pos != 0u && k >= pos && k - pos + WR_STREAM_RUN <= k1;
+}
+
+__device__ __forceinline__ float post_row_lean(const WrPostArgs &A, const float2 *__restrict__ chan_iq,
+                                               const float2 *__restrict__ chan_prev, unsigned int s, int m, size_t rr)
+{
+	const unsigned int k1 = A.k1, slots = A.slots;
+	if (rr < WR_HIST) {
+		const unsigned int kp = k1 - WR_HIST + (unsigned int)rr;
+		if (A.lean_prev && lean_inner(kp, A.off_prev, k1))
+			return A.dem_rows_prev[(size_t)kp * slots + s];
+		const float2 z = chan_prev[(size_t)kp * slots + s];
+		const float2 zp = chan_prev[(size_t)(kp - 1u) * slots + s];
+		return demod_one(m, z.x, z.y, zp.x, zp.y);
+	}
+	const size_t kk = rr - WR_HIST;
+	if (kk >= k1)
+		return 0.0f;
+	if (A.lean_cur && lean_inner((unsigned int)kk, A.off_cur, k1))
+		return A.dem_rows[kk * slots + s];
+	const float2 z = chan_iq[kk * slots + s];
+	const float2 zp = kk ? chan_iq[(kk - 1u) * slots + s] : chan_prev[((size_t)k1 - 1u) * slots + s];
+	return demod_one(m, z.x, z.y, zp.x, zp.y);
+}
+
+template <unsigned int D2, bool HREGS, unsigned int NSEG = 1u, bool LEAN = false>
 __device__ __forceinline__ void post_role(const WrPostArgs &A, unsigned int bx, unsigned int g,
                                           float *stage, float *tile, int *modes)
 {
@@ -446,7 +474,46 @@
 			const unsigned int per = (NEED - first + NROW - 1u) / NROW;
 			const unsigned int beg = first + row * per;
 			const unsigned int end = (beg + per < NEED) ? beg + per : NEED;
-			if (r0 > HIST && r0 + NEED <= (size_t)k1 + HIST) {
+			bool staged = false;
+			if constexpr (LEAN && NSEG == 1u) {
+				const bool inside = r0 > HIST && r0 + NEED <= (size_t)k1 + HIST;
+				if (A.lean_cur && inside) {
+					const unsigned int ub = __builtin_amdgcn_readfirstlane(beg), ue = __builtin_amdgcn_readfirstlane(end);
+					const unsigned int k0 = (unsigned int)(r0 - HIST);
+					const float2 *__restrict__ src = chan_iq + (size_t)k0 * slots + s;
+					const float *__restrict__ dsrc = A.dem_rows + (size_t)k0 * slots + s;
+					for (unsigned int r = ub; r < ue; r += POST_LB) {
+						float v[POST_LB];
+#pragma unroll
+						for (unsigned int i = 0; i < POST_LB; ++i) {
+							const unsigned int ri = (r + i < ue) ? r + i : ue - 1u;
+							v[i] = 0.0f;
+							if (m >= 0 && lean_inner(k0 + ri, A.off_cur, k1))
+								v[i] = dsrc[(size_t)ri * slots];
+						}
+#pragma unroll
+						for (unsigned int i = 0; i < POST_LB; ++i) {
+							const unsigned int ri = (r + i < ue) ? r + i : ue - 1u;
+							if (m >= 0 && !lean_inner(k0 + ri, A.off_cur, k1)) {
+								const float2 z = src[(size_t)ri * slots];
+								const float2 zp = src[((size_t)ri - 1u) * slots];
+								v[i] = demod_one(m, z.x, z.y, zp.x, zp.y);
+							}
+						}
+#pragma unroll
+						for (unsigned int i = 0; i < POST_LB; ++i)
+							if (r + i < ue)
+								stage[(r + i) * 64u + lane] = v[i];
+					}
+					staged = true;
+				} else if ((A.lean_cur | A.lean_prev) && !inside) {
+					for (unsigned int r = beg; r < end; ++r)
+						stage[r * 64u + lane] = (m >= 0) ? post_row_lean(A, chan_iq, chan_prev, s, m, r0 + r) : 0.0f;
+					staged = true;
+				}
+			}
+			if (staged) {
+			} else if (r0 > HIST && r0 + NEED <= (size_t)k1 + HIST) {
 				const float2 *__restrict__ src = chan_iq + (r0 - HIST) * slots + s;
 				for (unsigned int r = beg; r < end; r += POST_LB) {
 					float2 z[POST_LB + 1u];
diff --git a/webradio_amd/csrc/wr_stream_kernel.inc b/webradio_amd/csrc/wr_stream_kernel.inc
--- a/webradio_amd/csrc/wr_stream_kernel.inc
+++ b/webradio_amd/csrc/wr_stream_kernel.inc
@@ -191,6 +191,7 @@
 		return;
 	__builtin_amdgcn_s_setprio(3);
 	unsigned int seen = 1;
+	unsigned int nlean = 0;
 	__hip_atomic_store(&S.sdev->desc[0].cur, S.cur0, __ATOMIC_RELAXED, __HIP_MEMORY_SCOPE_AGENT);
 	__hip_atomic_store(&S.sdev->desc[0].audio_host, S.audio0, __ATOMIC_RELAXED, __HIP_MEMORY_SCOPE_AGENT);
 	__hip_atomic_store(&S.sdev->cur[1], S.cur0, __ATOMIC_RELAXED, __HIP_MEMORY_SCOPE_AGENT);
@@ -209,6 +210,7 @@
 		if (r > WR_STREAM_MAXJ)
 			r = WR_STREAM_MAXJ;
 		if (r > seen) {
+			const unsigned int again = S.lean ? __hip_atomic_load((const unsigned int *)&S.ctl->ready, __ATOMIC_RELAXED, __HIP_MEMORY_SCOPE_SYSTEM) : 0u;
 			for (unsigned int j = seen; j < r; ++j) {
 				const unsigned long long c = __hip_atomic_load(&S.desc_host[j].cur, __ATOMIC_RELAXED, __HIP_MEMORY_SCOPE_SYSTEM);
 				const unsigned long long a = __hip_atomic_load(&S.desc_host[j].audio_host, __ATOMIC_RELAXED, __HIP_MEMORY_SCOPE_SYSTEM);
@@ -216,6 +218,18 @@
 				__hip_atomic_store(&S.sdev->cur[j + 1u], c, __ATOMIC_RELAXED, __HIP_MEMORY_SCOPE_AGENT);
 				__hip_atomic_store(&S.sdev->desc[j].audio_host, a, __ATOMIC_RELAXED, __HIP_MEMORY_SCOPE_AGENT);
 			}
+			if (S.lean) {
+				unsigned int r2 = st_rfl(again);
+				if (r2 > WR_STREAM_MAXJ)
+					r2 = WR_STREAM_MAXJ;
+				if (r2 < r)
+					r2 = r;
+				for (unsigned int j = seen; j < r && j + 1u < r2; ++j) {
+					__hip_atomic_store(&S.sdev->lean[j], 1u, __ATOMIC_RELAXED, __HIP_MEMORY_SCOPE_AGENT);
+					++nlean;
+				}
+				st_st_sys(&S.ctl->lean_blocks, nlean);
+			}
 			asm volatile("s_waitcnt vmcnt(0)" ::: "memory");
 			__hip_atomic_store(&S.sdev->ready, r, __ATOMIC_RELAXED, __HIP_MEMORY_SCOPE_AGENT);
 			seen = r;
@@ -237,11 +251,12 @@
 	}
 }
 
-template <unsigned int PD2, unsigned int TS>
+template <unsigned int PD2, unsigned int NG, unsigned int TS>
 __device__ __forceinline__ void stream_post(const WrStreamArgs &S, const unsigned int p, v2f *lds, const bool helper)
 {
 	constexpr unsigned int D2 = PD2 ? PD2 : 1u;
 	constexpr unsigned int NEED = (POST_TK - 1u) * D2 + WR_FIR_LENGTH;
+	constexpr bool LEAN = NG == 2u && TS == 1u;
 	wave_prio(3u);
 	if (threadIdx.x >= POST_THREADS)
 		return;
@@ -328,6 +343,8 @@
 					drain = (df && j + 1u >= df) ? 1u : 0u;
 				}
 				sh[7] = (helper || drain) ? 1u : st_ld(&S.sdev->post_fine[j]);
+				sh[8] = (LEAN && S.lean) ? st_ld(&S.sdev->lean[j]) : 0u;
+				sh[9] = (LEAN && S.lean && j) ? st_ld(&S.sdev->lean[j - 1u]) : 0u;
 			}
 			sh[5] = drain;
 			sh[0] = ok ? 1u : 0u;
@@ -348,6 +365,14 @@
 		A.dem_hist = S.dem[S.parity0];
 		A.audio_host = (float *)ah;
 		A.audio = S.audio_bufs[j & 3u];
+		if (LEAN && (sh[8] | sh[9])) {
+			A.lean_cur = sh[8];
+			A.lean_prev = sh[9];
+			A.dem_rows = S.dem_ring + (size_t)(j % WR_STREAM_RING) * S.k1 * S.slots;
+			A.dem_rows_prev = S.dem_ring + (size_t)((j - 1u) % WR_STREAM_RING) * S.k1 * S.slots;
+			A.off_cur = (unsigned int)(((unsigned long long)j * S.k1) % WR_STREAM_RUN);
+			A.off_prev = (unsigned int)(((unsigned long long)(j - 1u) * S.k1) % WR_STREAM_RUN);
+		}
 #ifdef STREAM_TL
 		const unsigned long long pt1 = __builtin_amdgcn_s_memtime();
 		if (threadIdx.x == 0 && S.tl && !helper && p < 4u && j < 256u)
@@ -370,7 +395,7 @@
 			}
 			if (t >= tasks_j)
 				break;
-			post_role<D2, false>(A, t % A.ntiles, t / A.ntiles, stage, tile, modes);
+			post_role<D2, false, 1u, LEAN>(A, t % A.ntiles, t / A.ntiles, stage, tile, modes);
 			__syncthreads();
 			++mine;
 		}
@@ -418,6 +443,7 @@
 {
 	static_assert(TS == 1u || (TS == WR_TAPSETS && NG == 1u), "several channel filters: one lane group per wave");
 	constexpr int NCO = WR_NCO_ROTATE;
+	constexpr unsigned int RUN = (NG == 2u && TS == 1u) ? WR_STREAM_RUN : 1u;
 	const unsigned int lane = threadIdx.x & 63u;
 	const unsigned int wave = st_rfl(threadIdx.x >> 6);
 	const unsigned int waves_per_wg = blockDim.x >> 6;
@@ -436,10 +462,26 @@
 	unsigned int known = 1;
 	bool closed = false;
 	if (iw < wpg) {
-		const unsigned long long q0 = (unsigned long long)S.kslow + iw;
+		const unsigned int hop = (wpg - 1u) * RUN + 1u;
+		unsigned long long q0 = RUN == 1u ? (unsigned long long)S.kslow + iw : (unsigned long long)iw * RUN;
+		unsigned int ri = 0;
+		while (q0 < S.kslow) {
+			const bool last = ri + 1u == RUN;
+			q0 += last ? hop : 1u;
+			ri = last ? 0u : ri + 1u;
+		}
+		unsigned int rif = ri;
 		LeanRec<NG> R = lean_rec<NG>([&](unsigned int s) { return S.phase[s]; }, S.step, S.flags, (const float4 *)S.rot,
 		                             (float2 *)S.ring, S.gmap0, S.gmap1, gs, lane, (unsigned int)(q0 * d1 - WR_HIST), wpg, d1);
 		const LeanWin<TS> W = lean_win<TS>(S.taps1u, S.tapsel, R.g0, lane, nset, win);
+		v2f *carry = lds + 2u * WR_SPLIT_N + waves_per_wg * 128u * nset + wave * (NG * 64u) + lane;
+		unsigned int dem_g[NG];
+#pragma unroll
+		for (unsigned int c = 0; c < NG; ++c) {
+			const unsigned int gl = gs * NG + c;
+			dem_g[c] = (unsigned int)(((gl < 8u ? S.gmap0 : S.gmap1) >> ((gl & 7u) * 8u)) & 255u) * 64u;
+		}
+		bool lean_blk = false, lean_run = false;
 		unsigned int j = 0, k = (unsigned int)q0;
 		while (k >= k1s) {
 			k -= k1s;
@@ -508,7 +550,13 @@
 				dst = make_float2(x2.x, x2.y);
 			}
 			++ahead;
-			kf += wpg;
+			if (RUN == 1u) {
+				kf += wpg;
+			} else {
+				const bool last = rif + 1u == RUN;
+				kf += last ? hop : 1u;
+				rif = last ? 0u : rif + 1u;
+			}
 			while (kf >= k1s) {
 				kf -= k1s;
 				++jf;
@@ -537,6 +585,8 @@
 			const unsigned long long tl0 = tl_on ? __builtin_amdgcn_s_memtime() : 0ull;
 			if (j != jring) {
 				const unsigned long long pg = __hip_atomic_load(&S.sdev->progress, __ATOMIC_RELAXED, __HIP_MEMORY_SCOPE_AGENT);
+				if (RUN > 1u && S.lean)
+					lean_blk = st_ld(&S.sdev->lean[j]) != 0u;
 				const unsigned int dr = st_rfl((unsigned int)pg), pr = st_rfl((unsigned int)(pg >> 32));
 				lead = j > dr ? j - dr : 0u;
 				if (j + 1u >= WR_STREAM_RING && pr < j - WR_STREAM_RING + 2u) {
@@ -571,19 +621,39 @@
 			}
 			tell();
 			const size_t row = (size_t)(j % WR_STREAM_RING) * k1s + k;
+			if (RUN > 1u && ri == 0u)
+				lean_run = lean_blk && k + RUN <= k1s;
+			const bool last = ri + 1u == RUN;
+			const bool inner = RUN > 1u && lean_run && ri != 0u;
+			const unsigned int dq = RUN == 1u ? wpg : last ? hop : 1u;
 #pragma unroll
 			for (unsigned int c = 0; c < NG; ++c) {
 				if (R.fl[c] & PHASE_FLAG_ACTIVE) {
-					union { v2f f; unsigned long long u; } cv;
-					cv.f = acc.v[c];
-					__hip_atomic_store((unsigned long long *)&R.out[c][row * S.slots], cv.u, __ATOMIC_RELAXED,
-					                   __HIP_MEMORY_SCOPE_AGENT);
-				}
-				R.Pk[c] += R.dP[c];
+					if (inner) {
+						const v2f zp = carry[c * 64u];
+						const float dv = demod_one(WR_FM, acc.v[c].x, acc.v[c].y, zp.x, zp.y);
+						float *drow = S.dem_ring + (row * S.slots + dem_g[c]);
+						__hip_atomic_store((unsigned int *)&drow[lane], __builtin_bit_cast(unsigned int, dv),
+						                   __ATOMIC_RELAXED, __HIP_MEMORY_SCOPE_AGENT);
+					}
+					if (RUN > 1u && lean_run && !last)
+						carry[c * 64u] = acc.v[c];
+					if (!inner || last) {
+						union { v2f f; unsigned long long u; } cv;
+						cv.f = acc.v[c];
+						__hip_atomic_store((unsigned long long *)&R.out[c][row * S.slots], cv.u, __ATOMIC_RELAXED,
+						                   __HIP_MEMORY_SCOPE_AGENT);
+					}
+				}
+				if (RUN == 1u)
+					R.Pk[c] += R.dP[c];
+				else
+					R.Pk[c] += (dq * d1) * R.stv[c];
 			}
 			--ahead;
 			cnt += NG;
-			k += wpg;
+			k += dq;
+			ri = last ? 0u : ri + 1u;
 			if (k >= k1s) {
 				pend_j = j;
 				pend_cnt = cnt;
@@ -694,7 +764,7 @@
 		stream_ddc<NG, TS>(S, lds);
 		__syncthreads();
 	}
-	stream_post<PD2, TS>(S, ddc ? blockIdx.x : blockIdx.x - S.n_ddc, lds, ddc);
+	stream_post<PD2, NG, TS>(S, ddc ? blockIdx.x : blockIdx.x - S.n_ddc, lds, ddc);
 }
 
 static unsigned int stream_post_run(unsigned int tiles, unsigned int groups, unsigned int max_post)
@@ -708,7 +778,7 @@
 static size_t stream_lds_bytes(unsigned int d2, unsigned int nset)
 {
 	const size_t post_lds = post_lds_bytes(d2, 1u) + 16u * sizeof(float);
-	const size_t ddc_lds = (size_t)DDC_ROTATE_WAVES * 2u * 512u * nset + 2u * WR_SPLIT_N * 8u;
+	const size_t ddc_lds = (size_t)DDC_ROTATE_WAVES * 2u * 512u * nset + 2u * WR_SPLIT_N * 8u + (nset == 1u ? DDC_ROTATE_WAVES * 1024u : 0u);
 	return post_lds > ddc_lds ? post_lds : ddc_lds;
 }
 
@@ -800,6 +870,8 @@
 	stream_shape(A.groups, A.kmax, A.one_filter != 0u, &ng, &ts);
 	if ((size_t)A.n_ddc * DDC_ROTATE_WAVES < A.groups / ng)
 		return hipErrorInvalidValue;
+	if (ng != 2u || ts != 1u || !A.dem_ring || A.k1 < 2u * WR_STREAM_RUN)
+		A.lean = 0;
 	return with_post_d2(A.post.d2, [&](auto D2) {
 		constexpr unsigned int PD2 = decltype(D2)::value;
 		return ts != 1u ? launch_stream<PD2, 1, WR_TAPSETS>(st, A, ev_start, ev_stop)
diff --git a/webradio_amd/csrc/wr_tuner.hip b/webradio_amd/csrc/wr_tuner.hip
--- a/webradio_amd/csrc/wr_tuner.hip
+++ b/webradio_amd/csrc/wr_tuner.hip
@@ -771,6 +771,7 @@
 	std::vector<float> taps1b(g->d1b ? S * g->l1b : 0, 0.0f), gain(S, 1.0f), squelch(S, 0.0f);
 	std::vector<float> taps1L(g->l1 > WR_FIR_LENGTH ? S * g->l1 : 0, 0.0f);
 	g->use_gain = g->use_squelch = false;
+	g->all_fm = true;
 	for (size_t s = 0; s < S; ++s) {
 		int ci = g->owner[s];
 		if (ci < 0)
@@ -793,6 +794,7 @@
 		squelch[s] = c.squelch;
 		g->use_gain = g->use_gain || c.gain != 1.0f;
 		g->use_squelch = g->use_squelch || c.squelch > 0.0f;
+		g->all_fm = g->all_fm && c.mode == WR_FM;
 	}
 	GroupFilters F;
 	group_classify(t, g, F);
diff --git a/webradio_amd/csrc/wr_tuner_stream.hip b/webradio_amd/csrc/wr_tuner_stream.hip
--- a/webradio_amd/csrc/wr_tuner_stream.hip
+++ b/webradio_amd/csrc/wr_tuner_stream.hip
@@ -29,6 +29,7 @@
 	(void)hipHostFree(s.desc);
 	(void)hipFree(s.sdev);
 	(void)hipFree(s.ring);
+	(void)hipFree(s.dem_ring);
 	stream_raw_free(s);
 	if (s.raw_ev)
 		(void)hipEventDestroy(s.raw_ev);
@@ -38,6 +39,8 @@
 	s.sdev = nullptr;
 	s.ring = nullptr;
 	s.ring_floats = 0;
+	s.dem_ring = nullptr;
+	s.dem_ring_floats = 0;
 }
 
 int wrc_stream_check(wr_tuner *t)
@@ -48,6 +51,8 @@
 	s.unchecked = false;
 	s.long_blocks += s.ctl->long_blocks;
 	s.ctl->long_blocks = 0;
+	s.lean_blocks += s.ctl->lean_blocks;
+	s.ctl->lean_blocks = 0;
 	if (s.ctl->err)
 		return wrc_fail(WR_ERR_HIP, "streaming launch: a wait inside the launch ran into its deadline (code %u)", s.ctl->err);
 	if (s.ctl->final_blocks != s.count)
@@ -157,6 +162,15 @@
 		s.ring_floats = 0;
 		HIP_TRY(hipMalloc((void **)&s.ring, ring_floats * sizeof(float)));
 		s.ring_floats = ring_floats;
+	}
+	const bool lean = g->all_fm && !g->use_squelch && g->one_filter && !(groups & 1u) && kmax == 1u && k1 >= 2u * WR_STREAM_RUN;
+	if (lean && ring_floats / 2u > s.dem_ring_floats) {
+		HIP_TRY(wrc_dev_stream_sync(d));
+		(void)hipFree(s.dem_ring);
+		s.dem_ring = nullptr;
+		s.dem_ring_floats = 0;
+		HIP_TRY(hipMalloc((void **)&s.dem_ring, ring_floats / 2u * sizeof(float)));
+		s.dem_ring_floats = ring_floats / 2u;
 	}
 	void *ctl_dev = nullptr, *desc_dev = nullptr;
 	HIP_TRY(hipHostGetDevicePointer(&ctl_dev, s.ctl, 0));
@@ -214,6 +228,8 @@
 	A.hi_cs = d->hi_cs;
 	A.lo_cs = d->lo_cs;
 	A.ring = s.ring;
+	A.dem_ring = lean ? s.dem_ring : nullptr;
+	A.lean = lean ? 1u : 0u;
 	for (int i = 0; i < 4; ++i)
 		A.audio_bufs[i] = g->dev.audio_set[(g->audio_cur + i) & 3];
 	A.post = wrk_post_args(L, g->dev);
@@ -242,6 +258,7 @@
 	s.ctl->done = 0;
 	s.ctl->final_blocks = 0;
 	s.ctl->long_blocks = 0;
+	s.ctl->lean_blocks = 0;
 	s.ctl->err = 0;
 	s.ctl->self_closed = 0;
 	s.desc[0].cur = (unsigned long long)(uintptr_t)iq;
@@ -429,6 +446,14 @@
 	return WR_OK;
 }
 
+extern "C" int wr_tuner_stream_lean_blocks(wr_tuner *t, unsigned long long *blocks)
+{
+	if (!t || !blocks)
+		return wrc_fail(WR_ERR_ARG, "wr_tuner_stream_lean_blocks: bad argument");
+	*blocks = t->stream.lean_blocks;
+	return WR_OK;
+}
+
 extern "C" int wr_tuner_stream_host_blocks(wr_tuner *t, unsigned long long *blocks)
 {
 	if (!t || !blocks)
diff --git a/webradio_amd/device.py b/webradio_amd/device.py
--- a/webradio_amd/device.py
+++ b/webradio_amd/device.py
@@ -140,6 +140,11 @@
         check(self.lib.wr_tuner_stream_long_blocks(self.h, C.byref(n)))
         return n.value
 
+    def stream_lean_blocks(self):
+        n = C.c_ulonglong()
+        check(self.lib.wr_tuner_stream_lean_blocks(self.h, C.byref(n)))
+        return n.value
+
     def mark_launches(self, enable=True):
         check(self.lib.wr_tuner_mark_launches(self.h, 1 if enable else 0))
 
```

After: 114,900. 2.3% lower.
